# uthree/tinyvc

Hardware: AMD Instinct MI355X
Metric: audio-samples/sec (16 kHz) end-to-end VC (higher is better)
Workload: dtype f32 (fp32 in / out / accumulate; channel contractions as two-term fp16 splits on v_mfma_f32_32x32x16_f16: 22-bit significands, three part-products per fp32 product)

## Files before the change

tinyvc_amd/csrc/conv3s.h:

```cpp
#pragma once
#include <type_traits>
#include "conv_epi.h"
#include "small_kernels.h"
#include "split_fp16.h"
#include "tvc_common.h"

namespace tvc {

constexpr int S_WPE = 3;
constexpr int S_WPE_G = 4;
constexpr int S_WPE_F = 3;
constexpr int TVC_S_KG = 2;
constexpr int S_BPC = 1;
constexpr int S_FB = 2;
constexpr int S_FB_G = 1;
constexpr int S_FB_F = 1;
constexpr int S_FB_FW = 2;
constexpr int S_PF = 2;


template <class E, class = void>
struct wants_res_conv : std::false_type {};
template <class E>
struct wants_res_conv<E, std::void_t<decltype(E::kResConv)>> : std::bool_constant<E::kResConv> {};

template <int MTB_, int WM_, int NWV_, int WN_ = 1, int KG_ = 1, int MAXD_ = 27>
struct SplitTile {
    static constexpr int MTB = MTB_, WM = WM_, NWV = NWV_, WN = WN_;
    static constexpr int KG = KG_;
    static constexpr int MW = MTB / WM, NW = MW * NWV, NTHR = NW * 64;
    static_assert(MTB % WM == 0, "wave rows must tile the workgroup");
    static constexpr int BM = MTB * 32, BN = NWV * WN * 32;
    static constexpr int MAXD = MAXD_, XROW = BN + 2 * MAXD;
    static constexpr int XG_U4 = kParts * 2 * XROW;
    static constexpr int X_U4 = KG * XG_U4;
    static constexpr int X_PER = (KG * 2 * XROW + NTHR - 1) / NTHR;
    static constexpr int a_u4(int taps) { return taps * KG * MTB * kPU4; }
    static constexpr int stage_u4(int taps) { return a_u4(taps) + X_U4; }
    static constexpr int KS_MAX = 2 * 768;
    static constexpr int OS = BN + 4;
    static constexpr int lds_bytes(int taps) {
        const int stage = stage_u4(taps) * 16, out = BM * OS * 4;
        return (stage > out ? stage : out) + 2 * 6 * BM * 4 + KS_MAX * 4 + 64;
    }
    static constexpr int bias_off(int taps) {
        const int stage = stage_u4(taps) * 16, out = BM * OS * 4;
        return (stage > out ? stage : out) / 4;
    }
};

struct ConvSArgs {
    const uint4* A6;
    const float* wsc;
    int MT;
    const float* x;
    long xstride;
    int Cin, len, dil, tiles_per_utt, ntiles;
    int lin = 0;
    float lscale = 0.f;
    int cmax = 0;
    int flatT = 0;
    const float* kscale = nullptr;
    const uint4* sc6 = nullptr;
    const float* fsc = nullptr;
    const float* cond = nullptr;
    int Ccond = 0;
    const float* amax_x = nullptr;
    const float* amax_c = nullptr;
    float* amax_y = nullptr;
    RagDev rag;
};


template <class TL>
struct SlabRegs {
    static constexpr int A_MAX = (3 * TL::KG * TL::MTB * kParts + TL::NW - 1) / TL::NW;
    u32x4 ar[A_MAX];
    float xr[TL::X_PER][8];
    float xr2[TL::X_PER][8];
};
template <class TL>
struct SlabMap {
    unsigned xo[TL::X_PER];
    int xdst[TL::X_PER];
    int xg8[TL::X_PER];
    int xk[TL::X_PER];
    unsigned xo1[TL::X_PER];
    float w0[TL::X_PER], w1[TL::X_PER];
    float xs[TL::X_PER];
};
template <class TL, bool LERP = false>
__device__ __forceinline__ void make_map(SlabMap<TL>& m, int len, int dil, int t0, int fT = 0, unsigned fstride = 0, int kcin = 0, int lin = 0,
                                         float lscale = 0.f, float xs = 1.f, const float* amax = nullptr, int rs_ = 0, const int* __restrict__ c2b = nullptr, int cmult = 1) {
    const int rs = rs_ ? rs_ : len;
    const int xw = TL::BN + 2 * dil;
    int tid0 = threadIdx.x;
    asm volatile("" : "+v"(tid0));
    __builtin_assume(tid0 >= 0 && tid0 < TL::NTHR);
#pragma unroll
    for (int i = 0; i < TL::X_PER; ++i) {
        int idx = tid0 + i * TL::NTHR;
        int gk = idx / xw, c = idx - gk * xw;
        int p = t0 - dil + c;
        p = p < 0 ? 0 : (p > len - 1 ? len - 1 : p);
        const bool live = gk < 2 * TL::KG;
        gk = live ? gk : 2 * TL::KG - 1;
        const int ks = gk >> 1, g = gk & 1;
        m.xdst[i] = live ? ks * TL::XG_U4 + g * TL::XROW + c : -1;
        m.xg8[i] = ks * 16 + 8 * g;
        m.xs[i] = xs;
        if (fT > 0) {
            const int b = p / fT, t = p - b * fT;
            m.xo[i] = (unsigned)b * fstride + (unsigned)(m.xg8[i] * fT + t);
            m.xk[i] = (b - t0 / fT) * kcin;
            m.xs[i] = bfp_load(amax, b).s;
        } else if (LERP) {
            const Lerp lc = lerp_coord(p, lscale, lin);
            m.xo[i] = (unsigned)(m.xg8[i] * lin + lc.i0);
            m.xo1[i] = (unsigned)(m.xg8[i] * lin + lc.i1);
            m.w0[i] = lc.w0;
            m.w1[i] = lc.w1;
            m.xk[i] = 0;
        } else {
            m.xo[i] = (unsigned)(m.xg8[i] * rs + p);
            m.xk[i] = 0;
            if (c2b) m.xs[i] = bfp_load(amax, c2b[p / cmult]).s;
        }
    }
}
template <class TL, int TAPS, bool LERP = false, bool CLAMP = false>
__device__ __forceinline__ void slab_load(SlabRegs<TL>& r, const SlabMap<TL>& m, const uint4* __restrict__ A6, int MT, int mt0,
                                          const float* __restrict__ xb, int Cin, int len, int s, int fT = 0, int cmax = 0, int lin = 0, int rs_ = 0, int tid_ = -1) {
    constexpr int MTB = TL::MTB, NW = TL::NW, X_PER = TL::X_PER, STEPS = TAPS * TL::KG;
    const int cs = LERP ? lin : (fT > 0 ? fT : (rs_ ? rs_ : len));
    constexpr int PIECES = STEPS * MTB * kParts, A_PER = (PIECES + NW - 1) / NW;
    static_assert(A_PER <= SlabRegs<TL>::A_MAX, "weight pieces must fit the staging registers");
    const int tid = tid_ >= 0 ? tid_ : (int)threadIdx.x;
    __builtin_assume(tid >= 0 && tid < TL::NTHR);
    const int lane = tid & 63, wave = __builtin_amdgcn_readfirstlane(tid >> 6);
    __builtin_assume(wave >= 0 && wave < NW);
    const int ci0 = s * 16 * TL::KG;
    {
        const uint4* a_src = A6 + (long)mt0 * kPU4;
#pragma unroll
        for (int i = 0; i < A_PER; ++i) {
            int q = wave + i * NW;
            q = q < PIECES ? q : PIECES - 1;
            const int tap = q / (MTB * kParts), rem = q - tap * (MTB * kParts);
            r.ar[i] = ldg_so4(a_src + (long)s * STEPS * MT * kPU4, 16u * (unsigned)(tap * MT * kPU4 + rem * 64 + lane));
        }
    }
    const float* xc = xb + (long)ci0 * cs;
    if (LERP) {
#pragma unroll
        for (int i = 0; i < X_PER; ++i)
#pragma unroll
            for (int j = 0; j < 8; ++j) {
                r.xr[i][j] = ldg_so(xc + (long)j * cs, 4u * m.xo[i]);
                r.xr2[i][j] = ldg_so(xc + (long)j * cs, 4u * m.xo1[i]);
            }
        return;
    }
    if constexpr (CLAMP) {
#pragma unroll
        for (int i = 0; i < X_PER; ++i)
#pragma unroll
            for (int j = 0; j < 8; ++j) {
                int cj = ci0 + m.xg8[i] + j;
                cj = cj < cmax ? cj : cmax;
                r.xr[i][j] = xb[m.xo[i] + (unsigned)((cj - m.xg8[i]) * cs)];
            }
        return;
    }
#pragma unroll
    for (int i = 0; i < X_PER; ++i)
#pragma unroll
        for (int j = 0; j < 8; ++j) r.xr[i][j] = ldg_so(xc + (long)j * cs, 4u * m.xo[i]);
}
template <class TL, int TAPS, bool LERP = false, bool CLAMP = false>
__device__ __forceinline__ void first_load(SlabRegs<TL>& r, const uint4* __restrict__ A6, int MT, int mt0, const float* __restrict__ xb,
                                           int Cin, int len, int dil, int t0, int fT = 0, unsigned fstride = 0, int cmax = 0, int lin = 0,
                                           float lscale = 0.f, int rs_ = 0) {
    SlabMap<TL> m;
    make_map<TL, LERP>(m, len, dil, t0, fT, fstride, 0, lin, lscale, 1.f, nullptr, rs_);
    int tid = threadIdx.x;
    asm volatile("" : "+v"(tid));
    slab_load<TL, TAPS, LERP, CLAMP>(r, m, A6, MT, mt0, xb, Cin, len, 0, fT, cmax, lin, rs_, tid);
}

struct NoMid { __device__ __forceinline__ void operator()() const {} };
template <class TL, int TAPS, int A_U4, bool LRELU, int FB, bool SCALED = false, bool LERP = false, bool CLAMP = false, bool TWO = false, class Next, class Mid = NoMid>
__device__ __forceinline__ void split_phase(f32x16 (&hi)[TL::WM][TL::WN], f32x16 (&lo)[TL::WM][TL::WN], SlabRegs<TL>& r, const uint4* __restrict__ A6, int MT, int mt0,
                                            const float* __restrict__ xb, int Cin, int len, int dil, int t0, uint4* As, uint4* Xs, Next next, float xs,
                                            const float* Ks = nullptr, int fT = 0, unsigned fstride = 0, int cmax = 0, int lin = 0, float lscale = 0.f,
                                            int mt0b = 0, Mid mid = Mid(), const float* amax = nullptr, int rs_ = 0, const int* __restrict__ c2b = nullptr, int cmult = 1) {
    constexpr int MTB = TL::MTB, WM = TL::WM, WN = TL::WN, NWV = TL::NWV, NW = TL::NW, XROW = TL::XROW, X_PER = TL::X_PER;
    int tid = threadIdx.x;
    asm volatile("" : "+v"(tid));
    __builtin_assume(tid >= 0 && tid < TL::NTHR);
    const int lane = tid & 63, wave = __builtin_amdgcn_readfirstlane(tid >> 6);
    __builtin_assume(wave >= 0 && wave < NW);
    const int l31 = lane & 31, lh = lane >> 5;
    const int wm = wave / NWV, wn = wave - wm * NWV;
    SlabMap<TL> m;
    make_map<TL, LERP>(m, len, dil, t0, fT, fstride, Cin, lin, lscale, xs, amax, rs_, c2b, cmult);
    constexpr int STEPS = TAPS * TL::KG;
    constexpr int PIECES = STEPS * MTB * kParts, A_PER = (PIECES + NW - 1) / NW;
    auto lstore = [&](int sl) __attribute__((always_inline)) {
        uint4* Asb = As;
        uint4* Xsb = Xs;
#pragma unroll
        for (int i = 0; i < A_PER; ++i) {
            const int q = wave + i * NW;
            if (q < PIECES) *reinterpret_cast<u32x4*>(Asb + q * 64 + lane) = r.ar[i];
        }
#pragma unroll
        for (int i = 0; i < X_PER; ++i)
            if (m.xdst[i] >= 0) {
                if (LERP) {
#pragma unroll
                    for (int j = 0; j < 8; ++j) r.xr[i][j] = fmaf(m.w0[i], r.xr[i][j], __fmul_rn(m.w1[i], r.xr2[i][j]));
                }
                if (LRELU) {
#pragma unroll
                    for (int j = 0; j < 8; ++j) r.xr[i][j] = fmaxf(r.xr[i][j], 0.1f * r.xr[i][j]);
                }
                if (SCALED) {
                    const float4 k0 = *reinterpret_cast<const float4*>(Ks + m.xk[i] + sl * 16 * TL::KG + m.xg8[i]);
                    const float4 k1 = *reinterpret_cast<const float4*>(Ks + m.xk[i] + sl * 16 * TL::KG + m.xg8[i] + 4);
                    r.xr[i][0] *= k0.x; r.xr[i][1] *= k0.y; r.xr[i][2] *= k0.z; r.xr[i][3] *= k0.w;
                    r.xr[i][4] *= k1.x; r.xr[i][5] *= k1.y; r.xr[i][6] *= k1.z; r.xr[i][7] *= k1.w;
                }
#pragma unroll
                for (int j = 0; j < 8; ++j) r.xr[i][j] *= m.xs[i];
                uint4 p1, p2;
                split8(r.xr[i], p1, p2);
                Xsb[m.xdst[i]] = p1;
                Xsb[2 * XROW + m.xdst[i]] = p2;
            }
    };

    const int nslab1 = Cin / (16 * TL::KG);
    const int nslab = TWO ? 2 * nslab1 : nslab1;
    const uint4* as0 = As + wm * WM * kPU4 + lane;
    const uint4* xs0 = Xs + lh * XROW + wn * WN * 32 + l31;
    for (int s = 0; s < nslab; ++s) {
        slab_barrier();
        if (TWO && s == nslab1) mid();
        lstore(TWO && s >= nslab1 ? s - nslab1 : s);
        if (s + 1 < nslab) {
            if (TWO) slab_load<TL, TAPS, LERP, CLAMP>(r, m, A6, MT, s + 1 >= nslab1 ? mt0b : mt0, xb, Cin, len, s + 1 >= nslab1 ? s + 1 - nslab1 : s + 1, fT, cmax, lin, rs_, tid);
            else slab_load<TL, TAPS, LERP, CLAMP>(r, m, A6, MT, mt0, xb, Cin, len, s + 1, fT, cmax, lin, rs_, tid);
        } else next();
        slab_barrier();
        const uint4* as = as0;
        const uint4* xs_ = xs0;
        f16x8 af[2][WM][kParts], bf[2][WN][kParts];
        auto frags = [&](int tap, int fb) __attribute__((always_inline)) {
#pragma unroll
            for (int j = 0; j < WN; ++j)
#pragma unroll
                for (int p = 0; p < kParts; ++p)
                    bf[fb][j][p] = __builtin_bit_cast(f16x8, xs_[(tap / TAPS) * TL::XG_U4 + 2 * p * XROW + j * 32 + (tap % TAPS) * dil]);
#pragma unroll
            for (int i = 0; i < WM; ++i)
#pragma unroll
                for (int p = 0; p < kParts; ++p) af[fb][i][p] = __builtin_bit_cast(f16x8, as[(tap * MTB * kParts + i * kParts + p) * 64]);
        };
        if (FB == 2) frags(0, 0);
#pragma unroll
        for (int tap = 0; tap < STEPS; ++tap) {
            const int fb = FB == 2 ? tap & 1 : 0;
            if (FB == 2) {
                if (tap + 1 < STEPS) frags(tap + 1, fb ^ 1);
                __builtin_amdgcn_sched_barrier(0);
            } else {
                frags(tap, 0);
            }
#pragma unroll
            for (int i = 0; i < WM; ++i)
#pragma unroll
                for (int j = 0; j < WN; ++j) lo[i][j] = TVC_MFMA16(af[fb][i][1], bf[fb][j][0], lo[i][j]);
#pragma unroll
            for (int i = 0; i < WM; ++i)
#pragma unroll
                for (int j = 0; j < WN; ++j) hi[i][j] = TVC_MFMA16(af[fb][i][0], bf[fb][j][0], hi[i][j]);
#pragma unroll
            for (int i = 0; i < WM; ++i)
#pragma unroll
                for (int j = 0; j < WN; ++j) lo[i][j] = TVC_MFMA16(af[fb][i][0], bf[fb][j][1], lo[i][j]);
            if (FB == 2) __builtin_amdgcn_sched_barrier(0);
        }
    }
}

template <class TL>
__device__ __forceinline__ void film_load(SlabRegs<TL>& r, const SlabMap<TL>& m, const uint4* __restrict__ F6, int MT, int mt0, int mtoff,
                                          const float* __restrict__ xb, int len, int s, int rs_ = 0) {
    const int rs = rs_ ? rs_ : len;
    constexpr int MTB = TL::MTB, NW = TL::NW, X_PER = TL::X_PER;
    constexpr int KG = TL::KG, GP = 2 * MTB * kParts, PIECES = KG * GP, A_PER = (PIECES + NW - 1) / NW;
    static_assert(A_PER <= SlabRegs<TL>::A_MAX, "FiLM weight pieces must fit the staging registers");
    const int lane = threadIdx.x & 63, wave = threadIdx.x >> 6;
#pragma unroll
    for (int i = 0; i < A_PER; ++i) {
        int q = wave + i * NW;
        q = q < PIECES ? q : PIECES - 1;
        const int kg = q / GP, q2 = q - kg * GP;
        const int grp = q2 / (MTB * kParts), rem = q2 - grp * (MTB * kParts);
        r.ar[i] = ldg_so4(F6 + ((long)s * KG * MT + mt0) * kPU4, 16u * (unsigned)((kg * MT + grp * mtoff) * kPU4 + rem * 64 + lane));
    }
    const float* xc = xb + (long)s * 16 * KG * rs;
#pragma unroll
    for (int i = 0; i < X_PER; ++i)
#pragma unroll
        for (int j = 0; j < 8; ++j) r.xr[i][j] = ldg_so(xc + (long)j * rs, 4u * m.xo[i]);
}
template <class TL>
__device__ __forceinline__ void film_first_load(SlabRegs<TL>& r, const uint4* __restrict__ F6, int MT, int mt0, int mtoff,
                                                const float* __restrict__ xb, int len, int t0, int rs_ = 0) {
    SlabMap<TL> m;
    make_map<TL>(m, len, 0, t0, 0, 0u, 0, 0, 0.f, 1.f, nullptr, rs_);
    film_load<TL>(r, m, F6, MT, mt0, mtoff, xb, len, 0, rs_);
}
template <class TL, class Next>
__device__ __forceinline__ void film_phase(f32x16 (&asc)[TL::WM][TL::WN], f32x16 (&lsc)[TL::WM][TL::WN], f32x16 (&ash)[TL::WM][TL::WN], f32x16 (&lsh)[TL::WM][TL::WN],
                                           SlabRegs<TL>& r, const uint4* __restrict__ F6,
                                           int MT, int mt0, int mtoff, const float* __restrict__ xb, int Cin, int len, int t0, uint4* As, uint4* Xs,
                                           Next next, float xs, int rs_ = 0) {
    constexpr int MTB = TL::MTB, WM = TL::WM, WN = TL::WN, NWV = TL::NWV, NW = TL::NW, XROW = TL::XROW, X_PER = TL::X_PER;
    constexpr int KG = TL::KG, GP = 2 * MTB * kParts, PIECES = KG * GP, A_PER = (PIECES + NW - 1) / NW;
    const int tid = threadIdx.x, lane = tid & 63, wave = tid >> 6;
    const int l31 = lane & 31, lh = lane >> 5;
    const int wm = wave / NWV, wn = wave - wm * NWV;
    SlabMap<TL> m;
    make_map<TL>(m, len, 0, t0, 0, 0u, 0, 0, 0.f, 1.f, nullptr, rs_);
    const int nslab = Cin / (16 * KG);
    const uint4* as0 = As + wm * WM * kPU4 + lane;
    const uint4* xs0 = Xs + lh * XROW + wn * WN * 32 + l31;
    auto lstore = [&]() __attribute__((always_inline)) {
#pragma unroll
        for (int i = 0; i < A_PER; ++i) {
            const int q = wave + i * NW;
            if (q < PIECES) *reinterpret_cast<u32x4*>(As + q * 64 + lane) = r.ar[i];
        }
#pragma unroll
        for (int i = 0; i < X_PER; ++i)
            if (m.xdst[i] >= 0) {
#pragma unroll
                for (int j = 0; j < 8; ++j) r.xr[i][j] *= xs;
                uint4 p1, p2;
                split8(r.xr[i], p1, p2);
                Xs[m.xdst[i]] = p1;
                Xs[2 * XROW + m.xdst[i]] = p2;
            }
    };
    for (int s = 0; s < nslab; ++s) {
        slab_barrier();
        lstore();
        if (s + 1 < nslab) film_load<TL>(r, m, F6, MT, mt0, mtoff, xb, len, s + 1, rs_);
        else next();
        slab_barrier();
        const uint4* as = as0;
        const uint4* xq = xs0;
#pragma unroll
        for (int kg = 0; kg < KG; ++kg) {
            f16x8 fc[WM][kParts], fh[WM][kParts], bf[WN][kParts];
#pragma unroll
            for (int j = 0; j < WN; ++j)
#pragma unroll
                for (int p = 0; p < kParts; ++p) bf[j][p] = __builtin_bit_cast(f16x8, xq[kg * TL::XG_U4 + 2 * p * XROW + j * 32]);
#pragma unroll
            for (int i = 0; i < WM; ++i)
#pragma unroll
                for (int p = 0; p < kParts; ++p) {
                    fc[i][p] = __builtin_bit_cast(f16x8, as[(kg * GP + i * kParts + p) * 64]);
                    fh[i][p] = __builtin_bit_cast(f16x8, as[(kg * GP + MTB * kParts + i * kParts + p) * 64]);
                }
#pragma unroll
            for (int i = 0; i < WM; ++i)
#pragma unroll
                for (int j = 0; j < WN; ++j) {
                    lsc[i][j] = TVC_MFMA16(fc[i][1], bf[j][0], lsc[i][j]);
                    lsh[i][j] = TVC_MFMA16(fh[i][1], bf[j][0], lsh[i][j]);
                    asc[i][j] = TVC_MFMA16(fc[i][0], bf[j][0], asc[i][j]);
                    ash[i][j] = TVC_MFMA16(fh[i][0], bf[j][0], ash[i][j]);
                    lsc[i][j] = TVC_MFMA16(fc[i][0], bf[j][1], lsc[i][j]);
                    lsh[i][j] = TVC_MFMA16(fh[i][0], bf[j][1], lsh[i][j]);
                }
        }
    }
}

template <class TL, bool RES>
__device__ __forceinline__ void tile_store(float* Ot, const f32x16 (&v)[TL::WM][TL::WN], float* __restrict__ y, const float* __restrict__ res,
                                           int b, int M, int len, int mt0, int t0, float& mx, float* __restrict__ y2 = nullptr, int f2 = 0, int rlin = 0, float rscale = 0.f,
                                           int rs_ = 0, int coloff = 0) {
    const int rs = rs_ ? rs_ : len;
    const int rvalid = (rs_ && rlin > 0) ? __builtin_amdgcn_readfirstlane(len / (rs / rlin)) : rlin;
    const int rcol = (rs_ && rlin > 0) ? __builtin_amdgcn_readfirstlane(coloff / (rs / rlin)) : 0;
    constexpr int WM = TL::WM, WN = TL::WN, BM = TL::BM, BN = TL::BN, OS = TL::OS, NTHR = TL::NTHR;
    int tid = threadIdx.x;
    asm volatile("" : "+v"(tid));
    const int lane = tid & 63, wave = tid >> 6;
    const int l31 = lane & 31, lh = lane >> 5;
    const int wm = wave / TL::NWV, wn = wave - wm * TL::NWV;
    auto park = [&]() __attribute__((always_inline)) {
        slab_barrier();
#pragma unroll
        for (int i = 0; i < WM; ++i)
#pragma unroll
            for (int j = 0; j < WN; ++j)
#pragma unroll
                for (int r = 0; r < 16; ++r)
                    Ot[((wm * WM + i) * 32 + 4 * lh + (r & 3) + 8 * (r >> 2)) * OS + (wn * WN + j) * 32 + l31] = v[i][j][r];
        slab_barrier();
    };
    __builtin_amdgcn_sched_barrier(0);
    float* yb = y + ((long)b * M + mt0 * 32) * rs + coloff + t0;
    const float* rb = RES ? (rlin > 0 ? res + ((long)b * M + mt0 * 32) * rlin + rcol : res + ((long)b * M + mt0 * 32) * rs + coloff + t0) : nullptr;
    const int rows = M - mt0 * 32 < BM ? M - mt0 * 32 : BM;
    const bool vec = ((rs | coloff) & 3) == 0;
    const int len2 = f2 > 0 ? rs / f2 : 0;
    float* y2b = y2 ? y2 + ((long)b * M + mt0 * 32) * len2 + (f2 > 0 ? coloff / f2 : 0) : nullptr;
    if constexpr (RES) {
        if (rlin > 0) {
            constexpr int G = BN / 4, RS = NTHR / G;
            static_assert(NTHR % G == 0, "column groups must tile the workgroup");
            const int c = (tid % G) * 4;
            unsigned o0[4], o1[4];
            float lam[4];
#pragma unroll
            for (int u = 0; u < 4; ++u) {
                const int t = t0 + c + u < len ? t0 + c + u : len - 1;
                const Lerp lc = lerp_coord(t, rscale, rvalid);
                o0[u] = 4u * (unsigned)lc.i0;
                o1[u] = 4u * (unsigned)lc.i1;
                lam[u] = lc.w1;
            }
            const bool full = vec && t0 + c + 3 < len;
            constexpr int NR = (BM + RS - 1) / RS, PF = S_PF;
            float x0[PF][4], x1[PF][4];
            const bool live = t0 + c < len;
            auto request = [&](int k0) __attribute__((always_inline)) {
#pragma unroll
                for (int k = 0; k < PF; ++k) {
                    int row = tid / G + (k0 + k) * RS;
                    row = row < rows ? row : rows - 1;
                    const unsigned ro = 4u * (unsigned)(row * rlin);
#pragma unroll
                    for (int u = 0; u < 4; ++u) {
                        x0[k][u] = ldg_so(rb, ro + o0[u]);
                        x1[k][u] = ldg_so(rb, ro + o1[u]);
                    }
                }
            };
            __builtin_amdgcn_sched_barrier(0);
            request(0);
            park();
            if (live) {
#pragma unroll
            for (int k0 = 0; k0 < NR; k0 += PF) {
                float w[PF][4];
#pragma unroll
                for (int k = 0; k < PF; ++k)
#pragma unroll
                    for (int u = 0; u < 4; ++u) w[k][u] = fmaf(1.f - lam[u], x0[k][u], __fmul_rn(lam[u], x1[k][u]));
                if (k0 + PF < NR) request(k0 + PF);
#pragma unroll
                for (int k = 0; k < PF; ++k) {
                    const int row = tid / G + (k0 + k) * RS;
                    if (row >= rows) break;
                    const float4 o = *reinterpret_cast<const float4*>(Ot + row * OS + c);
                    const float e[4] = {o.x + w[k][0], o.y + w[k][1], o.z + w[k][2], o.w + w[k][3]};
                    const int off = row * rs + c;
                    if (full) {
                        *reinterpret_cast<float4*>(yb + off) = make_float4(e[0], e[1], e[2], e[3]);
                        mx = fmaxf(fmaxf(mx, fmaxf(fabsf(e[0]), fabsf(e[1]))), fmaxf(fabsf(e[2]), fabsf(e[3])));
                    } else {
#pragma unroll
                        for (int u = 0; u < 4; ++u)
                            if (t0 + c + u < len) {
                                yb[off + u] = e[u];
                                mx = fmaxf(mx, fabsf(e[u]));
                            }
                    }
                }
            }
            }
            return;
        }
        if (vec && t0 + BN <= len) {
            constexpr int G = BN / 4, RS = NTHR / G, NR = (BM + RS - 1) / RS;
            const int c = (tid % G) * 4;
            float4 q[NR];
            __builtin_amdgcn_sched_barrier(0);
#pragma unroll
            for (int k = 0; k < NR; ++k) {
                int row = tid / G + k * RS;
                row = row < rows ? row : rows - 1;
                q[k] = *reinterpret_cast<const float4*>(rb + row * rs + c);
            }
            park();
#pragma unroll
            for (int k = 0; k < NR; ++k) {
                const int row = tid / G + k * RS;
                if (row >= rows) break;
                float4 w = *reinterpret_cast<const float4*>(Ot + row * OS + c);
                w.x += q[k].x; w.y += q[k].y; w.z += q[k].z; w.w += q[k].w;
                *reinterpret_cast<float4*>(yb + row * rs + c) = w;
                mx = fmaxf(fmaxf(mx, fmaxf(fabsf(w.x), fabsf(w.y))), fmaxf(fabsf(w.z), fabsf(w.w)));
                if (y2b) {
                    const float e[4] = {w.x, w.y, w.z, w.w};
                    if (f2 == 4) {
                        y2b[row * len2 + ((t0 + c) >> 2)] = fmaf(0.5f, e[1], __fmul_rn(0.5f, e[2]));
                    } else {
#pragma unroll
                        for (int u = 0; u < 4; ++u) {
                            const int t = t0 + c + u, qq = t / f2;
                            if (t - qq * f2 == (f2 >> 1)) y2b[row * len2 + qq] = e[u];
                        }
                    }
                }
            }
            return;
        }
    }
    park();
#pragma unroll 2
    for (int idx = tid; idx < BM * (BN / 4); idx += NTHR) {
        const int row = idx / (BN / 4), c = (idx - row * (BN / 4)) * 4;
        if (row >= rows || t0 + c >= len) continue;
        const float4 o = *reinterpret_cast<const float4*>(Ot + row * OS + c);
        const int off = row * rs + c;
        if (RES && rlin > 0) {
            const float e[4] = {o.x, o.y, o.z, o.w};
            float w[4];
#pragma unroll
            for (int u = 0; u < 4; ++u) {
                const int t = t0 + c + u < len ? t0 + c + u : len - 1;
                const Lerp lc = lerp_coord(t, rscale, rvalid);
                w[u] = e[u] + lerp_eval(lc, rb[row * rlin + lc.i0], rb[row * rlin + lc.i1]);
            }
            if (vec && t0 + c + 3 < len) {
                *reinterpret_cast<float4*>(yb + off) = make_float4(w[0], w[1], w[2], w[3]);
                mx = fmaxf(fmaxf(mx, fmaxf(fabsf(w[0]), fabsf(w[1]))), fmaxf(fabsf(w[2]), fabsf(w[3])));
            } else {
#pragma unroll
                for (int u = 0; u < 4; ++u)
                    if (t0 + c + u < len) {
                        yb[off + u] = w[u];
                        mx = fmaxf(mx, fabsf(w[u]));
                    }
            }
        } else if (vec && t0 + c + 3 < len) {
            float4 w = o;
            if (RES) {
                const float4 q = *reinterpret_cast<const float4*>(rb + off);
                w.x += q.x; w.y += q.y; w.z += q.z; w.w += q.w;
            }
            *reinterpret_cast<float4*>(yb + off) = w;
            mx = fmaxf(fmaxf(mx, fmaxf(fabsf(w.x), fabsf(w.y))), fmaxf(fabsf(w.z), fabsf(w.w)));
            if (y2b) {
                const float e[4] = {w.x, w.y, w.z, w.w};
                if (f2 == 4) {
                    y2b[row * len2 + ((t0 + c) >> 2)] = fmaf(0.5f, e[1], __fmul_rn(0.5f, e[2]));
                } else {
#pragma unroll
                    for (int u = 0; u < 4; ++u) {
                        const int t = t0 + c + u, q = t / f2;
                        if (t - q * f2 == (f2 >> 1)) y2b[row * len2 + q] = e[u];
                    }
                }
            }
        } else {
            const float e[4] = {o.x, o.y, o.z, o.w};
#pragma unroll
            for (int u = 0; u < 4; ++u)
                if (t0 + c + u < len) {
                    const float ov = RES ? e[u] + rb[off + u] : e[u];
                    yb[off + u] = ov;
                    mx = fmaxf(mx, fabsf(ov));
                    if (y2b && f2 != 4) {
                        const int t = t0 + c + u, q = t / f2;
                        if (t - q * f2 == (f2 >> 1)) y2b[row * len2 + q] = ov;
                    }
                }
        }
    }
}

template <class TL, int TAPS, bool LRELU, class Epi, bool FILM, bool SCALED = false, bool LERP = false, bool CLAMP = false, bool RAG = false>
__global__ __launch_bounds__(TL::NTHR) __attribute__((amdgpu_waves_per_eu(FILM ? S_WPE_F : (Epi::kIgemm ? (TL::NW <= 8 ? S_WPE_G : 5) : S_WPE)))) void conv3s_kernel(ConvSArgs a, Epi ep) {
    static_assert(!RAG || (!LERP && !SCALED && !(FILM && TL::WN > 1)), "ragged batches: plain / residual-conv / narrow FiLM / GEMM launches only");
    constexpr bool RAGT = RAG && !Epi::kIgemm;
    constexpr bool RAGG = RAG && Epi::kIgemm;
    constexpr int MTB = TL::MTB, WM = TL::WM, WN = TL::WN, A_U4 = TL::a_u4(TAPS);
    extern __shared__ __attribute__((aligned(16))) uint4 smem_s[];
    uint4* As = smem_s;
    uint4* Xs = smem_s + A_U4;

    const int lane = threadIdx.x & 63, wave = threadIdx.x >> 6;
    const int lh = lane >> 5;
    const int wm = wave / TL::NWV;
    const int mblocks = a.MT / MTB;
    int len = a.len;
    const int rs = RAGT ? a.len : 0;
    int coloff = 0;
    const int ntiles = a.ntiles;

    auto coords = [&](int v, int& mt0, int& b, int& t0) __attribute__((always_inline)) {
        const int nt_id = v / mblocks, mb = v - nt_id * mblocks;
        mt0 = mb * MTB;
        if constexpr (RAGT) {
            b = __builtin_amdgcn_readfirstlane(rag_find(a.rag.ts, a.rag.B, __builtin_amdgcn_readfirstlane(nt_id), b));
            t0 = __builtin_amdgcn_readfirstlane((nt_id - a.rag.ts[b]) * TL::BN);
        } else {
            b = nt_id / a.tiles_per_utt;
            t0 = (nt_id - b * a.tiles_per_utt) * TL::BN;
        }
    };
    auto ulen = [&](int b_) __attribute__((always_inline)) { return __builtin_amdgcn_readfirstlane(a.rag.tb[b_] * a.rag.mult); };
    auto uoff = [&](int b_) __attribute__((always_inline)) { return __builtin_amdgcn_readfirstlane(a.rag.pre[b_] * a.rag.mult); };
    int tile, vtiles;
    tile_range(ntiles, tile, vtiles);
    SlabRegs<TL> regs;
    int mt0 = 0, b = 0, t0 = 0;
    if (tile >= vtiles) return;
    coords(tile, mt0, b, t0);
    float mx_run = 0.f;
    int mx_b = b;
    float* const red = reinterpret_cast<float*>(smem_s) + TL::bias_off(TAPS) + 12 * TL::BM + TL::KS_MAX;
    const int fT = (TAPS == 1 && !FILM && !LERP && !RAGT) ? a.flatT : 0;
    const unsigned fstride = (unsigned)a.xstride;
    constexpr bool FILM_FIRST = FILM && TL::WN == 1;
    auto load_first = [&](int mt0_, int b_, int t0_) __attribute__((always_inline)) {
        if constexpr (FILM_FIRST && RAGT) film_first_load<TL>(regs, a.sc6, 2 * a.MT, mt0_, a.MT, a.cond + uoff(b_), ulen(b_), t0_, rs);
        else if constexpr (FILM_FIRST) film_first_load<TL>(regs, a.sc6, 2 * a.MT, mt0_, a.MT, a.cond + (long)b_ * a.Ccond * len, len, t0_);
        else if constexpr (RAGT) first_load<TL, TAPS, LERP, CLAMP>(regs, a.A6, a.MT, mt0_, a.x + uoff(b_), a.Cin, ulen(b_), a.dil, t0_, 0, 0u, a.cmax, 0, 0.f, rs);
        else first_load<TL, TAPS, LERP, CLAMP>(regs, a.A6, a.MT, mt0_, fT ? a.x : a.x + (long)b_ * a.xstride, a.Cin, len, a.dil, t0_, fT, fstride, a.cmax, a.lin, a.lscale);
    };
    if constexpr (RAGT) {
        len = ulen(b);
        coloff = uoff(b);
    }
    load_first(mt0, b, t0);
    for (int tile_no = 0; tile < vtiles; ++tile_no) {
        const int nxt = tile + 1;
        if constexpr (!Epi::kIgemm) {
            if (a.amax_y && b != mx_b) {
                amax_flush_wg(a.amax_y + mx_b, mx_run, red);
                mx_run = 0.f;
                mx_b = b;
            }
        }
        auto load_next_tile = [&]() __attribute__((always_inline)) {
            if (nxt < vtiles) {
                int mt0n, bn = b, t0n;
                coords(nxt, mt0n, bn, t0n);
                load_first(mt0n, bn, t0n);
            }
        };
        const float* xb = RAGT ? a.x + coloff : (fT ? a.x : a.x + (long)b * a.xstride);
        float* Bs = reinterpret_cast<float*>(smem_s) + TL::bias_off(TAPS) + (tile_no & 1) * 6 * TL::BM;
        if constexpr (!Epi::kIgemm) {
            for (int i = threadIdx.x; i < TL::BM; i += TL::NTHR) {
                int m = mt0 * 32 + i;
                m = m < ep.M ? m : ep.M - 1;
                Bs[i] = ep.bias[m];
                Bs[3 * TL::BM + i] = a.wsc[mt0 + (i >> 5)];
                if constexpr (FILM) {
                    Bs[TL::BM + i] = ep.bsc[m];
                    Bs[2 * TL::BM + i] = ep.bsh[m];
                    Bs[4 * TL::BM + i] = a.fsc[mt0 + (i >> 5)];
                    Bs[5 * TL::BM + i] = a.fsc[a.MT + mt0 + (i >> 5)];
                }
            }
        }
        float* Ks = reinterpret_cast<float*>(smem_s) + TL::bias_off(TAPS) + 12 * TL::BM;
        if constexpr (SCALED) {
            const int b0 = fT ? t0 / fT : b;
            const int nrow = fT ? ((t0 + TL::BN - 1 < len ? t0 + TL::BN - 1 : len - 1) / fT - b0 + 1) * a.Cin : a.Cin;
            for (int i = threadIdx.x; i < nrow; i += TL::NTHR) Ks[i] = a.kscale[(long)b0 * a.Cin + i];
        }
        const int rl = wm * WM * 32 + 4 * lh;
        const Bfp sx = (fT || RAGG) ? Bfp{1.f, 1.f} : bfp_load_u(a.amax_x, b);
        f32x16 hi[WM][WN], lo[WM][WN];
        auto clear = [&](f32x16 (&u)[WM][WN]) __attribute__((always_inline)) {
#pragma unroll
            for (int i = 0; i < WM; ++i)
#pragma unroll
                for (int j = 0; j < WN; ++j)
#pragma unroll
                    for (int r = 0; r < 16; ++r) u[i][j][r] = 0.f;
        };
        clear(hi);
        clear(lo);
        auto fold = [&](f32x16 (&h)[WM][WN], const f32x16 (&l)[WM][WN], const float* wtab, float inv) __attribute__((always_inline)) {
#pragma unroll
            for (int i = 0; i < WM; ++i)
#pragma unroll
                for (int q = 0; q < 4; ++q) {
                    const float4 w4 = *reinterpret_cast<const float4*>(wtab + rl + i * 32 + 8 * q);
                    const float wv[4] = {w4.x, w4.y, w4.z, w4.w};
#pragma unroll
                    for (int u = 0; u < 4; ++u) {
                        const float c = wv[u] * inv, cl = c * kLoInv;
#pragma unroll
                        for (int j = 0; j < WN; ++j) h[i][j][4 * q + u] = comb(h[i][j][4 * q + u], l[i][j][4 * q + u], c, cl);
                    }
#pragma unroll
                    for (int j = 0; j < WN; ++j) asm volatile("" : "+v"(h[i][j]) : : "memory");
                }
        };

        if constexpr (FILM && TL::WN > 1) {
            const float* cb = a.cond + (long)b * a.Ccond * len;
            const int mtoff = a.MT;
            const Bfp sc = bfp_load_u(a.amax_c, b);
            split_phase<TL, TAPS, A_U4, LRELU, S_FB_FW, false, LERP, false>(
                hi, lo, regs, a.A6, a.MT, mt0, xb, a.Cin, len, a.dil, t0, As, Xs,
                [&]() __attribute__((always_inline)) { first_load<TL, 1>(regs, a.sc6, 2 * a.MT, mt0, cb, a.Ccond, len, 0, t0); }, sx.s, nullptr, 0, 0u, 0, a.lin, a.lscale);
            fold(hi, lo, Bs + 3 * TL::BM, sx.inv);
            f32x16 fh[WM][WN];
            clear(fh);
            clear(lo);
            split_phase<TL, 1, A_U4, false, S_FB_F, false, false, false, true>(
                fh, lo, regs, a.sc6, 2 * a.MT, mt0, cb, a.Ccond, len, 0, t0, As, Xs, load_next_tile, sc.s, nullptr, 0, 0u, 0, 0, 0.f, mtoff + mt0,
                [&]() __attribute__((always_inline)) {
                    fold(fh, lo, Bs + 4 * TL::BM, sc.inv);
#pragma unroll
                    for (int i = 0; i < WM; ++i)
#pragma unroll
                        for (int r = 0; r < 16; ++r) {
                            const int row = rl + i * 32 + (r & 3) + 8 * (r >> 2);
                            const float bm = Bs[row], bs = Bs[TL::BM + row];
#pragma unroll
                            for (int j = 0; j < WN; ++j) {
                                hi[i][j][r] = __fmul_rn(hi[i][j][r] + bm, fh[i][j][r] + bs);
                                fh[i][j][r] = 0.f;
                                lo[i][j][r] = 0.f;
                            }
                        }
                });
            fold(fh, lo, Bs + 5 * TL::BM, sc.inv);
#pragma unroll
            for (int i = 0; i < WM; ++i)
#pragma unroll
                for (int r = 0; r < 16; ++r) {
                    const float bh = Bs[2 * TL::BM + rl + i * 32 + (r & 3) + 8 * (r >> 2)];
#pragma unroll
                    for (int j = 0; j < WN; ++j) hi[i][j][r] = __fadd_rn(hi[i][j][r], fh[i][j][r] + bh);
                }
            tile_store<TL, true>(reinterpret_cast<float*>(smem_s), hi, ep.y, ep.res, b, ep.M, len, mt0, t0, mx_run, nullptr, 0, ep.res_lin, ep.res_scale);
        } else if constexpr (FILM) {
            const float* cb = RAGT ? a.cond + coloff : a.cond + (long)b * a.Ccond * len;
            const int mtoff = a.MT;
            const Bfp sc = bfp_load_u(a.amax_c, b);
            f32x16 asc[WM][WN], lsc[WM][WN], ash[WM][WN], lsh[WM][WN];
            clear(asc);
            clear(lsc);
            clear(ash);
            clear(lsh);
            film_phase<TL>(asc, lsc, ash, lsh, regs, a.sc6, 2 * a.MT, mt0, mtoff, cb, a.Ccond, len, t0, As, Xs,
                           [&]() __attribute__((always_inline)) { first_load<TL, TAPS, LERP, false>(regs, a.A6, a.MT, mt0, xb, a.Cin, len, a.dil, t0, 0, 0u, 0, a.lin, a.lscale, rs); }, sc.s, rs);
            fold(asc, lsc, Bs + 4 * TL::BM, sc.inv);
            fold(ash, lsh, Bs + 5 * TL::BM, sc.inv);
            split_phase<TL, TAPS, A_U4, LRELU, S_FB_F, false, LERP, false>(hi, lo, regs, a.A6, a.MT, mt0, xb, a.Cin, len, a.dil, t0, As, Xs, load_next_tile, sx.s, nullptr, 0, 0u, 0,
                                                                            a.lin, a.lscale, 0, NoMid(), nullptr, rs);
            fold(hi, lo, Bs + 3 * TL::BM, sx.inv);
            {
#pragma unroll
                for (int i = 0; i < WM; ++i)
#pragma unroll
                    for (int q = 0; q < 4; ++q) {
                        const int row = rl + i * 32 + 8 * q;
                        const float4 m4 = *reinterpret_cast<const float4*>(Bs + row), s4 = *reinterpret_cast<const float4*>(Bs + TL::BM + row),
                                     h4 = *reinterpret_cast<const float4*>(Bs + 2 * TL::BM + row);
                        const float bm[4] = {m4.x, m4.y, m4.z, m4.w}, bs[4] = {s4.x, s4.y, s4.z, s4.w}, bh[4] = {h4.x, h4.y, h4.z, h4.w};
#pragma unroll
                        for (int u = 0; u < 4; ++u)
#pragma unroll
                            for (int j = 0; j < WN; ++j)
                                hi[i][j][4 * q + u] = __fadd_rn(__fmul_rn(hi[i][j][4 * q + u] + bm[u], asc[i][j][4 * q + u] + bs[u]), ash[i][j][4 * q + u] + bh[u]);
#pragma unroll
                        for (int j = 0; j < WN; ++j) asm volatile("" : "+v"(hi[i][j]) : : "memory");
                    }
                tile_store<TL, true>(reinterpret_cast<float*>(smem_s), hi, ep.y, ep.res, RAGT ? 0 : b, ep.M, len, mt0, t0, mx_run, nullptr, 0, ep.res_lin, ep.res_scale, rs, coloff);
            }
        } else {
            float inv = sx.inv;
            if constexpr (wants_res_conv<Epi>::value) {
                const float* cb = RAGT ? a.cond + coloff : a.cond + (long)b * a.Ccond * len;
                const Bfp s2 = bfp_min(sx, bfp_load_u(a.amax_c, b));
                inv = s2.inv;
                split_phase<TL, TAPS, A_U4, LRELU, S_FB, false, false, false>(
                    hi, lo, regs, a.A6, a.MT, mt0, xb, a.Cin, len, a.dil, t0, As, Xs,
                    [&]() __attribute__((always_inline)) { first_load<TL, 1>(regs, a.sc6, a.MT, mt0, cb, a.Ccond, len, 0, t0, 0, 0u, 0, 0, 0.f, rs); }, s2.s, nullptr, 0, 0u, 0, 0, 0.f,
                    0, NoMid(), nullptr, rs);
                split_phase<TL, 1, A_U4, false, S_FB, false, false, false>(hi, lo, regs, a.sc6, a.MT, mt0, cb, a.Ccond, len, 0, t0, As, Xs, load_next_tile, s2.s, nullptr, 0, 0u, 0, 0,
                                                                           0.f, 0, NoMid(), nullptr, rs);
            } else
            split_phase<TL, TAPS, A_U4, LRELU, Epi::kIgemm ? S_FB_G : S_FB, SCALED, LERP, CLAMP>(hi, lo, regs, a.A6, a.MT, mt0, xb, a.Cin, len, a.dil, t0, As, Xs,
                                                                                                  load_next_tile, sx.s, Ks, fT, fstride, a.cmax, a.lin, a.lscale, 0, NoMid(),
                                                                                                  a.amax_x, rs, RAGG ? a.rag.col2b : nullptr, RAGG ? a.rag.mult : 1);
            if constexpr (Epi::kIgemm) {
                const int l31 = lane & 31, wn = wave - wm * TL::NWV;
                const int mtw = __builtin_amdgcn_readfirstlane(mt0 + wm * WM);
#pragma unroll
                for (int i = 0; i < WM; ++i) {
                    const float cw = a.wsc[mtw + i];
#pragma unroll
                    for (int j = 0; j < WN; ++j) {
                        const int col = t0 + (wn * WN + j) * 32 + l31;
                        const int n = b * len + col;
                        if (col < len) {
                            const float c = cw * (RAGG ? bfp_load(a.amax_x, a.rag.col2b[col / a.rag.mult]).inv : (fT ? bfp_load(a.amax_x, col / fT).inv : inv)), cl = c * kLoInv;
#pragma unroll
                            for (int q = 0; q < 4; ++q) {
                                const float v[4] = {comb(hi[i][j][4 * q], lo[i][j][4 * q], c, cl), comb(hi[i][j][4 * q + 1], lo[i][j][4 * q + 1], c, cl),
                                                    comb(hi[i][j][4 * q + 2], lo[i][j][4 * q + 2], c, cl), comb(hi[i][j][4 * q + 3], lo[i][j][4 * q + 3], c, cl)};
                                ep.store(n, (mt0 + wm * WM + i) * 32 + 8 * q + 4 * lh, v);
                            }
                        }
                    }
                }
                tile = nxt;
                if (tile < vtiles) coords(tile, mt0, b, t0);
                continue;
            }
            if constexpr (!Epi::kIgemm) {
                fold(hi, lo, Bs + 3 * TL::BM, inv);
#pragma unroll
                for (int i = 0; i < WM; ++i)
#pragma unroll
                    for (int r = 0; r < 16; ++r) {
                        const float bm = Bs[rl + i * 32 + (r & 3) + 8 * (r >> 2)];
#pragma unroll
                        for (int j = 0; j < WN; ++j) hi[i][j][r] += bm;
                    }
                tile_store<TL, Epi::kRes>(reinterpret_cast<float*>(smem_s), hi, ep.y, ep.res, RAGT ? 0 : b, ep.M, len, mt0, t0, mx_run, ep.y2, ep.f2, 0, 0.f, rs, coloff);
            }
        }
        tile = nxt;
        if (tile < vtiles) {
            coords(tile, mt0, b, t0);
            if constexpr (RAGT) {
                len = ulen(b);
                coloff = uoff(b);
            }
        }
    }
    if constexpr (!Epi::kIgemm) {
        if (a.amax_y) amax_flush_wg(a.amax_y + mx_b, mx_run, red);
    }
}

template <class TL, int TAPS, bool LRELU, class Epi, bool FILM, bool SCALED = false, bool LERP = false, bool CLAMP = false>
inline int conv3s_launch_t(tvc_ctx* ctx, hipStream_t s, const PackedW& w, const float* x, int B, int Cin, int len, int dil, const Epi& ep,
                           const PackedW* wsc, const PackedW* wsh, const float* cond, int Ccond, long xstride = 0, int bpc = S_BPC,
                           const float* kscale = nullptr, bool flat = false, int cmax = 0, int lin = 0, float lscale = 0.f, const BfpSlots& bfp = {}) {
    if (Cin % (16 * TL::KG) != 0 || (FILM && Ccond % (16 * TL::KG) != 0)) return fail(ctx, TVC_ERR_ARG, "conv3s: channel counts must be multiples of the slab depth");
    if (Cin / 16 > w.S6) return fail(ctx, TVC_ERR_ARG, "conv3s: weight image has fewer K16 steps than the launch walks");
    constexpr int lds = TL::lds_bytes(TAPS);
    TVC_CHECK((lds_optin<conv3s_kernel<TL, TAPS, LRELU, Epi, FILM, SCALED, LERP, CLAMP>>(ctx, lds, "conv3s")));
    ConvSArgs a;
    a.A6 = reinterpret_cast<const uint4*>(w.A6);
    a.wsc = w.wscale;
    a.MT = w.MT6;
    a.amax_x = bfp.x;
    a.amax_c = bfp.c;
    a.amax_y = bfp.y;
    if (Epi::kIgemm && bfp.y) return fail(ctx, TVC_ERR_ARG, "conv3s: GEMM launches finish their elements in the epilogue functor and cannot track the output's |max|");
    if (SCALED && (!kscale || Cin > 768)) return fail(ctx, TVC_ERR_ARG, "conv3s: scaled launch needs factors for <= 768 channels");
    a.kscale = kscale;
    a.cmax = cmax;
    if (CLAMP != (cmax > 0)) return fail(ctx, TVC_ERR_ARG, "conv3s: row clamp is a compile-time property of the launch");
    a.lin = lin;
    a.lscale = lscale;
    if (LERP && (lin <= 0 || flat)) return fail(ctx, TVC_ERR_ARG, "conv3s: interpolated input needs its low-rate length");
    a.x = x;
    a.xstride = xstride ? xstride : (long)Cin * (LERP ? lin : len);
    a.Cin = Cin;
    a.len = len;
    a.dil = dil;
    if (flat) {
        if (FILM || TAPS != 1 || dil != 0) return fail(ctx, TVC_ERR_ARG, "conv3s: flat tiles are for plain GEMMs");
        a.flatT = len;
        a.len = B * len;
        B = 1;
    }
    a.tiles_per_utt = (a.len + TL::BN - 1) / TL::BN;
    if (wants_res_conv<Epi>::value) {
        if (FILM || !wsc || wsc->MT6 != w.MT6 || wsc->taps != 1 || Ccond % 16 != 0 || Ccond / 16 > wsc->S6 || !cond)
            return fail(ctx, TVC_ERR_ARG, "conv3s: the residual 1x1 phase needs a matching 1x1 image and its input");
        if (wsc->wjoint != w.A6) return fail(ctx, TVC_ERR_STATE, "conv3s: the residual 1x1's image must be packed with the conv's per-m-tile scales");
        a.sc6 = reinterpret_cast<const uint4*>(wsc->A6);
        a.cond = cond;
        a.Ccond = Ccond;
    }
    if (FILM) {
        if (wsc->MT6 != 2 * w.MT6) return fail(ctx, TVC_ERR_ARG, "conv3s: FiLM image must stack scale and shift rows");
        a.sc6 = reinterpret_cast<const uint4*>(wsc->A6);
        a.fsc = wsc->wscale;
        a.cond = cond;
        a.Ccond = Ccond;
    }
    a.ntiles = (a.MT / TL::MTB) * a.tiles_per_utt * B;
    const int slots = ctx->ncu * bpc;
    if (ctx->rag) {
        if constexpr (!LERP && !SCALED && !(FILM && TL::WN > 1)) {
            if (flat) return fail(ctx, TVC_ERR_STATE, "conv3s: a ragged batch runs as one long utterance");
            int ncol = a.tiles_per_utt;
            TVC_CHECK(rag_tiles(ctx, s, B, a.len, Epi::kIgemm ? 0 : TL::BN, &a.rag, &ncol, "conv3s"));
            TVC_CHECK((lds_optin<conv3s_kernel<TL, TAPS, LRELU, Epi, FILM, SCALED, LERP, CLAMP, true>>(ctx, lds, "conv3s")));
            a.ntiles = (a.MT / TL::MTB) * ncol;
            dim3 g((unsigned)(a.ntiles < slots ? a.ntiles : slots));
            hipLaunchKernelGGL((conv3s_kernel<TL, TAPS, LRELU, Epi, FILM, SCALED, LERP, CLAMP, true>), g, dim3(TL::NTHR), lds, s, a, ep);
            return 0;
        } else {
            return fail(ctx, TVC_ERR_STATE, "conv3s: this launch has no ragged-batch variant");
        }
    }
    dim3 g((unsigned)(a.ntiles < slots ? a.ntiles : slots));
    hipLaunchKernelGGL((conv3s_kernel<TL, TAPS, LRELU, Epi, FILM, SCALED, LERP, CLAMP>), g, dim3(TL::NTHR), lds, s, a, ep);
    return 0;
}

template <bool LRELU, class Epi, bool FILM = false, bool LERP = false>
inline int conv3s_launch(tvc_ctx* ctx, hipStream_t s, const PackedW& w, const float* x, int B, int Cin, int len, int dil, const Epi& ep,
                         const BfpSlots& bfp, const PackedW* wsc = nullptr, const PackedW* wsh = nullptr, const float* cond = nullptr, int Ccond = 0, int lin = 0,
                         float lscale = 0.f) {
    if (w.MT6 % 3 != 0) return fail(ctx, TVC_ERR_ARG, "conv3s: k3 convs need a multiple of 96 output rows");
    if constexpr (FILM) {
        const long mb = w.MT6 / 3;
        const long tiles_w = mb * ((len + 255) / 256) * B;
        const long slots = 256 * S_BPC;
        const bool wide = tiles_w >= slots && !ctx->rag;
        if (wide)
            return conv3s_launch_t<SplitTile<3, 1, 4, 2>, 3, LRELU, Epi, FILM, false, LERP>(ctx, s, w, x, B, Cin, len, dil, ep, wsc, wsh, cond, Ccond, 0, S_BPC, nullptr, false,
                                                                                           0, lin, lscale, bfp);
        if (Cin % 32 == 0 && Ccond % 32 == 0)
            return conv3s_launch_t<SplitTile<3, 1, 4, 1, 2>, 3, LRELU, Epi, FILM, false, LERP>(ctx, s, w, x, B, Cin, len, dil, ep, wsc, wsh, cond, Ccond, 0, S_BPC, nullptr, false, 0,
                                                                                              lin, lscale, bfp);
        return conv3s_launch_t<SplitTile<3, 1, 4, 1>, 3, LRELU, Epi, FILM, false, LERP>(ctx, s, w, x, B, Cin, len, dil, ep, wsc, wsh, cond, Ccond, 0, S_BPC, nullptr, false, 0,
                                                                                       lin, lscale, bfp);
    } else
        return conv3s_launch_t<SplitTile<3, 1, 4, 2>, 3, LRELU, Epi, FILM, false, LERP>(ctx, s, w, x, B, Cin, len, dil, ep, wsc, wsh, cond, Ccond, 0, S_BPC, nullptr, false, 0,
                                                                                       lin, lscale, bfp);
}

template <int MTB, int NWV, int BPC, int KG, class Epi, bool SCALED, bool CLAMP>
inline int gemm_s_launch_k(tvc_ctx* ctx, hipStream_t s, const PackedW& w, const float* x, int B, int Cin, int len, long xstride, const Epi& ep,
                           const float* kscale, int cmax, const float* amax_x) {
    using TL = SplitTile<MTB, (MTB >= 4 ? 2 : 1), NWV, 1, KG, 0>;
    const long xs = xstride ? xstride : (long)Cin * len;
    const bool flat = B > 1 && xs * B < (1L << 30) && (!SCALED || len >= TL::BN);
    return conv3s_launch_t<TL, 1, false, Epi, false, SCALED, false, CLAMP>(ctx, s, w, x, B, Cin, len, 0, ep, nullptr, nullptr, nullptr, 0, xstride, BPC, kscale, flat,
                                                                           cmax, 0, 0.f, BfpSlots{amax_x, nullptr, nullptr});
}
template <int MTB, int NWV, int BPC, class Epi, bool SCALED = false>
inline int gemm_s_launch(tvc_ctx* ctx, hipStream_t s, const PackedW& w, const float* x, int B, int Cin, int len, long xstride, const Epi& ep,
                         const float* amax_x, const float* kscale = nullptr) {
    if (w.MT6 % MTB != 0) return fail(ctx, TVC_ERR_ARG, "gemm_s: row tiles do not divide");
    if (TVC_S_KG >= 2 && Cin % 32 == 0) return gemm_s_launch_k<MTB, NWV, BPC, 2, Epi, SCALED, false>(ctx, s, w, x, B, Cin, len, xstride, ep, kscale, 0, amax_x);
    return gemm_s_launch_k<MTB, NWV, BPC, 1, Epi, SCALED, false>(ctx, s, w, x, B, Cin, len, xstride, ep, kscale, 0, amax_x);
}
template <int MTB, int NWV, int BPC, class Epi>
inline int gemm_s_launch_ragged(tvc_ctx* ctx, hipStream_t s, const PackedW& w, const float* x, int B, int krows, int len, long xstride, const Epi& ep,
                                const float* amax_x) {
    if (w.MT6 % MTB != 0) return fail(ctx, TVC_ERR_ARG, "gemm_s: row tiles do not divide");
    return gemm_s_launch_k<MTB, NWV, BPC, 2, Epi, false, true>(ctx, s, w, x, B, (krows + 31) / 32 * 32, len, xstride, ep, nullptr, krows - 1, amax_x);
}


}
```

tinyvc_amd/csrc/conv_epi.h:

```cpp
#pragma once
#include "gemm_epi.h"

namespace tvc {

template <bool RES, int F2 = 0>
struct C3EpiBias {
    static constexpr bool kRes = RES;
    static constexpr bool kIgemm = false;
    float* y;
    const float* bias;
    const float* res;
    int M, len;
    float* y2 = nullptr;
    int f2 = 0;
    __device__ __forceinline__ void store(int b, int t, int m, const float v[4]) const {
        const int q = F2 > 0 ? t / F2 : 0;
        const bool pick = F2 > 0 && y2 != nullptr && t - q * F2 == (F2 >> 1);
#pragma unroll
        for (int r = 0; r < 4; ++r)
            if (m + r < M) {
                long i = ((long)b * M + m + r) * len + t;
                float o = v[r] + bias[m + r];
                if (RES) o += res[i];
                y[i] = o;
                if (pick) y2[((long)b * M + m + r) * (len / F2) + q] = o;
            }
    }
};

struct C3EpiBiasResConv : C3EpiBias<false, 0> {
    static constexpr bool kResConv = true;
};

struct C3EpiFilmFused {
    static constexpr bool kIgemm = false;
    float* y;
    const float* bias;
    const float* bsc;
    const float* bsh;
    const float* res;
    int M, len;
    int res_lin = 0;
    float res_scale = 0.f;
    __device__ __forceinline__ void store(int b, int t, int m, const float h[4], const float sc[4], const float sh[4]) const {
#pragma unroll
        for (int r = 0; r < 4; ++r)
            if (m + r < M) {
                long i = ((long)b * M + m + r) * len + t;
                float hv = h[r] + bias[m + r];
                y[i] = __fadd_rn(__fadd_rn(__fmul_rn(hv, sc[r] + bsc[m + r]), sh[r] + bsh[m + r]), res[i]);
            }
    }
};

}
```

tinyvc_amd/csrc/conv_s2.h:

```cpp
#pragma once
#include "small_kernels.h"
#include "split_fp16.h"

namespace tvc {

struct ConvS2Args {
    const uint4* A6;
    const float* wsc;
    int MT;
    const float* x;
    int Cin, len, dil, lin;
    float lscale;
    float* y;
    const float* bias;
    int M, tiles_per_utt, ntiles, mblocks;
    const float* amax_x;
    float* amax_y;
    uint4* ypre;
    float pre_w, pre_b;
    RagDev rag;
};
__device__ __forceinline__ float presplit_bound(float pre_w, float pre_b, const float* amax, int b) { return fmaf(pre_w, sload_f32(amax + b), pre_b); }
__device__ __forceinline__ Bfp norm_from_amax(float amax) {
    const unsigned u = __builtin_bit_cast(unsigned, amax);
    Bfp r{1.f, 1.f};
    if (u != 0u && u < 0x7f800000u) {
        int k = 14 - ((int)(u >> 23) - 127);
        k = k > 120 ? 120 : (k < -120 ? -120 : k);
        r.s = __builtin_bit_cast(float, (unsigned)(127 + k) << 23);
        r.inv = __builtin_bit_cast(float, (unsigned)(127 - k) << 23);
    }
    return r;
}

struct CS2 {
    static constexpr int MTB = 3, NWV = 4, WN = 2, NW = MTB * NWV, NTHR = NW * 64, BN = NWV * WN * 32, MAXD = 27, XROW = BN + 2 * MAXD;
    static constexpr int A_PIECES = 3 * MTB * kParts, A_PER = (A_PIECES + NW - 1) / NW;
    static constexpr int A_U4 = A_PIECES * 64, X_U4 = kParts * 2 * XROW, BUF_U4 = A_U4 + X_U4;
    static constexpr int TAB = 2 * 128 * 3;
    static constexpr int lds_bytes = 2 * BUF_U4 * 16 + TAB * 4 + 64;
};

template <bool LERP, bool PRE = false, bool RAG = false>
__global__ __launch_bounds__(CS2::NTHR) __attribute__((amdgpu_waves_per_eu(3))) void conv_s2_kernel(ConvS2Args a) {
    using TL = CS2;
    constexpr int MTB = TL::MTB, NWV = TL::NWV, WN = TL::WN, NW = TL::NW, BN = TL::BN, XROW = TL::XROW, A_PER = TL::A_PER;
    extern __shared__ __attribute__((aligned(16))) uint4 smem_c2[];
    float* Tb = reinterpret_cast<float*>(smem_c2 + 2 * TL::BUF_U4);
    float* red = Tb + TL::TAB;
    const int tid = threadIdx.x, lane = tid & 63;
    const int wave = __builtin_amdgcn_readfirstlane(tid >> 6);
    const int l31 = lane & 31, lh = lane >> 5;
    const int wm = wave / NWV, wn = wave - wm * NWV;
    const int nslab = a.Cin / 16, rs = a.len, dil = a.dil;
    const int cs_ = LERP ? a.lin : rs;
    const int xf = LERP ? rs / a.lin : 1;
    const int xw = BN + 2 * dil, nitems = 2 * xw;

    for (int i = tid; i < a.M; i += TL::NTHR) {
        Tb[i] = a.bias[i];
        Tb[384 + i] = a.wsc[i >> 5];
    }

    int tfirst, tlast;
    tile_range(a.ntiles, tfirst, tlast);
    if (tfirst >= tlast) return;
    auto coords = [&](int v, int& mt0, int& b, int& t0, int& len, int& off) __attribute__((always_inline)) {
        const int nt = v / a.mblocks, mb = v - nt * a.mblocks;
        mt0 = mb * MTB;
        const RagTile rt = rag_tile<RAG>(a.rag, nt, a.tiles_per_utt, rs, b);
        b = rt.b;
        t0 = rt.tin * BN;
        len = rt.len;
        off = rt.off;
    };

    u32x4 ar[A_PER];
    float xr[8], xr2[LERP ? 8 : 1];
    const int item = tid < nitems ? tid : tid - nitems;
    const int ig = item / xw, ic = item - ig * xw;
    const int xdst = ig * XROW + ic;
    unsigned xo = 0, xo1 = 0;
    float lw0 = 0.f, lw1 = 0.f, xsc = 1.f;
    float rw0 = 0.f, rw1 = 0.f, rxs = 1.f;
    int lv = tfirst, ls = 0, lmt0, lb = 0, lt0, llen, loff;
    coords(lv, lmt0, lb, lt0, llen, loff);
    auto tile_offsets = [&]() __attribute__((always_inline)) {
        int p = lt0 - dil + ic;
        p = p < 0 ? 0 : (p > llen - 1 ? llen - 1 : p);
        const int cbase = 8 * ig * cs_ + (RAG ? (LERP ? loff / xf : loff) : 0);
        if (LERP) {
            const Lerp lc = lerp_coord(p, a.lscale, RAG ? llen / xf : a.lin);
            xo = (unsigned)(cbase + lc.i0);
            xo1 = (unsigned)(cbase + lc.i1);
            lw0 = lc.w0;
            lw1 = lc.w1;
        } else {
            xo = (unsigned)(cbase + p);
        }
        xsc = bfp_load_u(a.amax_x, lb).s;
    };
    tile_offsets();
    auto issue_load = [&]() __attribute__((always_inline)) {
        const uint4* abase = a.A6 + ((long)ls * 3 * a.MT + lmt0) * kPU4;
#pragma unroll
        for (int i = 0; i < A_PER; ++i) {
            int q = wave + i * NW;
            q = q < TL::A_PIECES ? q : TL::A_PIECES - 1;
            const int tap = q / (MTB * kParts), rem = q - tap * (MTB * kParts);
            ar[i] = ldg_so4(abase, 16u * (unsigned)(tap * a.MT * kPU4 + rem * 64 + lane));
        }
        const float* xc = a.x + ((RAG ? 0L : (long)lb * a.Cin) + (long)ls * 16) * cs_;
#pragma unroll
        for (int j = 0; j < 8; ++j) {
            xr[j] = ldg_so(xc + (long)j * cs_, 4u * xo);
            if (LERP) xr2[j] = ldg_so(xc + (long)j * cs_, 4u * xo1);
        }
        rw0 = lw0;
        rw1 = lw1;
        rxs = xsc;
    };
    auto advance_load = [&]() __attribute__((always_inline)) {
        if (++ls == nslab) {
            if (lv + 1 < tlast) {
                ++lv;
                ls = 0;
                coords(lv, lmt0, lb, lt0, llen, loff);
                tile_offsets();
            } else {
                ls = nslab - 1;
            }
        }
    };
    auto lstore = [&](int buf) __attribute__((always_inline)) {
        uint4* Ab = smem_c2 + buf * TL::BUF_U4;
        uint4* Xb = Ab + TL::A_U4;
#pragma unroll
        for (int i = 0; i < A_PER; ++i) {
            int q = wave + i * NW;
            q = q < TL::A_PIECES ? q : TL::A_PIECES - 1;
            *reinterpret_cast<u32x4*>(Ab + q * 64 + lane) = ar[i];
        }
        float v[8];
#pragma unroll
        for (int j = 0; j < 8; ++j) {
            const float t = LERP ? fmaf(rw0, xr[j], __fmul_rn(rw1, xr2[j])) : xr[j];
            v[j] = fmaxf(t, 0.1f * t) * rxs;
        }
        uint4 p1, p2;
        split8(v, p1, p2);
        Xb[xdst] = p1;
        Xb[2 * XROW + xdst] = p2;
    };

    f32x16 hi[WN], lo[WN];
#pragma unroll
    for (int j = 0; j < WN; ++j)
#pragma unroll
        for (int r = 0; r < 16; ++r) hi[j][r] = lo[j][r] = 0.f;
    auto multiply = [&](int buf, int tap) __attribute__((always_inline)) {
        const uint4* Ab = smem_c2 + buf * TL::BUF_U4 + ((tap * MTB + wm) * kParts) * 64 + lane;
        const uint4* Xb = smem_c2 + buf * TL::BUF_U4 + TL::A_U4 + lh * XROW + wn * WN * 32 + l31 + tap * dil;
        f16x8 af[kParts], bf[WN][kParts];
#pragma unroll
        for (int j = 0; j < WN; ++j)
#pragma unroll
            for (int p = 0; p < kParts; ++p) bf[j][p] = __builtin_bit_cast(f16x8, Xb[p * 2 * XROW + j * 32]);
#pragma unroll
        for (int p = 0; p < kParts; ++p) af[p] = __builtin_bit_cast(f16x8, Ab[p * 64]);
#pragma unroll
        for (int j = 0; j < WN; ++j) lo[j] = TVC_MFMA16(af[1], bf[j][0], lo[j]);
#pragma unroll
        for (int j = 0; j < WN; ++j) hi[j] = TVC_MFMA16(af[0], bf[j][0], hi[j]);
#pragma unroll
        for (int j = 0; j < WN; ++j) lo[j] = TVC_MFMA16(af[0], bf[j][1], lo[j]);
    };

    int cv = tfirst, cs = 0, cmt0, cb = 0, ct0, len, coff;
    coords(cv, cmt0, cb, ct0, len, coff);
    float mx_run = 0.f;
    int flush_b = -1;

    issue_load();
    advance_load();
    lstore(0);
    issue_load();
    advance_load();
    slab_barrier();
    int buf = 0;
    while (true) {
        multiply(buf, 0);
        lstore(buf ^ 1);
        issue_load();
        multiply(buf, 1);
        multiply(buf, 2);
        advance_load();
        if (++cs == nslab) {
            const Bfp sx = bfp_load_u(a.amax_x, cb);
            const int row0 = (cmt0 + wm) * 32;
            float* yb = RAG ? a.y + (long)row0 * rs + coff : a.y + ((long)cb * a.M + row0) * rs;
            const float ps = PRE ? norm_from_amax(presplit_bound(a.pre_w, a.pre_b, a.amax_x, cb)).s : 1.f;
#pragma unroll
            for (int j = 0; j < WN; ++j) {
                const int t = ct0 + (wn * WN + j) * 32 + l31;
                const bool live = t < len;
                const unsigned off = 4u * (unsigned)(4 * lh * rs + (live ? t : len - 1));
#pragma unroll
                for (int g = 0; g < 4; ++g) {
                    if (row0 + 8 * g < a.M) {
                        const float4 bv = *reinterpret_cast<const float4*>(Tb + row0 + 8 * g + 4 * lh);
                        const float c = Tb[384 + row0] * sx.inv, cl = c * kLoInv;
                        const float e[4] = {comb(hi[j][4 * g], lo[j][4 * g], c, cl) + bv.x, comb(hi[j][4 * g + 1], lo[j][4 * g + 1], c, cl) + bv.y,
                                            comb(hi[j][4 * g + 2], lo[j][4 * g + 2], c, cl) + bv.z, comb(hi[j][4 * g + 3], lo[j][4 * g + 3], c, cl) + bv.w};
                        if (PRE) {
                            float v[4];
#pragma unroll
                            for (int q = 0; q < 4; ++q) v[q] = fmaxf(e[q], 0.1f * e[q]) * ps;
                            unsigned p1[2], p2[2];
                            split2<false>(v[0], v[1], p1[0], p2[0]);
                            split2<false>(v[2], v[3], p1[1], p2[1]);
                            const auto qx = __builtin_amdgcn_permlane32_swap(p1[0], p2[0], false, false);
                            const auto qy = __builtin_amdgcn_permlane32_swap(p1[1], p2[1], false, false);
                            if (live) a.ypre[(((RAG ? 0L : (long)cb * 2) + lh) * (a.M >> 3) + ((row0 >> 3) + g)) * rs + (RAG ? coff : 0) + t] = make_uint4(qx[0], qy[0], qx[1], qy[1]);
                        } else if (live) {
#pragma unroll
                            for (int q = 0; q < 4; ++q) {
                                stg_so(yb + (long)(8 * g + q) * rs, off, e[q]);
                                mx_run = fmaxf(mx_run, fabsf(e[q]));
                            }
                        }
                    }
                }
#pragma unroll
                for (int r = 0; r < 16; ++r) hi[j][r] = lo[j][r] = 0.f;
            }
            cs = 0;
            const int done_b = cb;
            ++cv;
            const bool last = cv >= tlast;
            if (!last) coords(cv, cmt0, cb, ct0, len, coff);
            if (a.amax_y && (last || cb != done_b)) {
                const float m = wave_max(mx_run);
                if (lane == 0) red[wave] = m;
                mx_run = 0.f;
                flush_b = done_b;
            }
            if (last) break;
        }
        slab_barrier();
        if (flush_b >= 0) {
            if (tid == 0) {
                float m = 0.f;
                for (int w = 0; w < NW; ++w) m = fmaxf(m, red[w]);
                if (m > 0.f) atomicMax(reinterpret_cast<unsigned*>(a.amax_y + flush_b), __builtin_bit_cast(unsigned, m));
            }
            flush_b = -1;
        }
        buf ^= 1;
    }
    if (flush_b >= 0) {
        slab_barrier();
        if (tid == 0) {
            float m = 0.f;
            for (int w = 0; w < NW; ++w) m = fmaxf(m, red[w]);
            if (m > 0.f) atomicMax(reinterpret_cast<unsigned*>(a.amax_y + flush_b), __builtin_bit_cast(unsigned, m));
        }
    }
}

template <bool LERP, bool PRE = false>
inline bool conv_s2_try(int* rc, tvc_ctx* ctx, hipStream_t s, const PackedW& w, const float* x, int B, int Cin, int len, int dil, float* y, const BfpSlots& bfp,
                        int lin = 0, float lscale = 0.f, float pre_w = 0.f, float pre_b = 0.f) {
    if (PRE && (!bfp.x || w.M % 8 != 0)) return false;
    if (w.taps != 3 || w.MT6 % 3 != 0 || w.M > 384 || Cin % 16 != 0 || Cin / 16 > w.S6 || dil < 1 || dil > CS2::MAXD || bfp.c) return false;
    if ((long)B * w.M * len >= (1L << 31) / 4 * 4 && (long)w.M * len * 4 >= (1L << 32)) return false;
    if ((long)Cin * (LERP ? lin : len) * 4 >= (1L << 32) || (long)w.M * len * 4 >= (1L << 32)) return false;
    if (LERP != (lin > 0)) return false;
    if ((*rc = lds_optin<conv_s2_kernel<LERP, PRE>, conv_s2_kernel<LERP, PRE, true>>(ctx, CS2::lds_bytes, "conv_s2"))) return true;
    ConvS2Args a;
    a.A6 = reinterpret_cast<const uint4*>(w.A6);
    a.wsc = w.wscale;
    a.MT = w.MT6;
    a.x = x;
    a.Cin = Cin;
    a.len = len;
    a.dil = dil;
    a.lin = lin;
    a.lscale = lscale;
    a.y = y;
    a.bias = w.bias;
    a.M = w.M;
    a.mblocks = w.MT6 / CS2::MTB;
    a.tiles_per_utt = (len + CS2::BN - 1) / CS2::BN;
    a.amax_x = bfp.x;
    a.amax_y = PRE ? nullptr : bfp.y;
    a.ypre = reinterpret_cast<uint4*>(y);
    a.pre_w = pre_w;
    a.pre_b = pre_b;
    int ncol = a.tiles_per_utt * B;
    if ((*rc = rag_tiles(ctx, s, B, len, CS2::BN, &a.rag, &ncol, "conv_s2"))) return true;
    a.ntiles = ncol * a.mblocks;
    const int grid = a.ntiles < ctx->ncu ? a.ntiles : ctx->ncu;
    if (ctx->rag) hipLaunchKernelGGL((conv_s2_kernel<LERP, PRE, true>), dim3(grid), dim3(CS2::NTHR), CS2::lds_bytes, s, a);
    else hipLaunchKernelGGL((conv_s2_kernel<LERP, PRE>), dim3(grid), dim3(CS2::NTHR), CS2::lds_bytes, s, a);
    *rc = launch_check(ctx, "conv_s2");
    return true;
}

}
```

tinyvc_amd/csrc/decoder.hip:

```cpp
#include "conv3s.h"
#include "conv_s2.h"
#include "film_s2.h"
#include "gemm_s2.h"
#include "small_kernels.h"
#include "tvc_common.h"

namespace tvc {


__device__ __forceinline__ float div24k(float x) {
    const float r = 1.0f / 24000.0f;
    const float q0 = __fmul_rn(x, r);
    return fmaf(fmaf(-q0, 24000.0f, x), r, q0);
}

__device__ __forceinline__ double wave_incl_scan(double v, int lane) {
#pragma unroll
    for (int o = 1; o < 64; o <<= 1) {
        double u = __shfl_up(v, o);
        if (lane >= o) v += u;
    }
    return v;
}

static __global__ __launch_bounds__(256) void harm_frame_sum_kernel(const float* __restrict__ f0, double* __restrict__ csum,
                                                                    int T, float scale, RagDev rg) {
    const int b = blockIdx.y, lane = threadIdx.x & 63;
    const int t = 4 * blockIdx.x + (threadIdx.x >> 6);
    const int rs = T;
    long fbase = (long)b * T, cbase = (long)b * kHarm * T;
    if (rg.tb) {
        T = rg.tb[b];
        fbase = cbase = rg.pre[b];
        scale = __fdiv_rn((float)T, (float)(T * kHop));
    }
    if (t >= T) return;
    const float* f = f0 + fbase;
    double acc[kHarm];
#pragma unroll
    for (int m = 0; m < kHarm; ++m) acc[m] = 0.0;
    if (lane < kHop / 8) {
#pragma unroll
        for (int k = 0; k < 8; ++k) {
            Lerp c = lerp_coord(t * kHop + 8 * lane + k, scale, T);
            float fs = lerp_eval(c, f[c.i0], f[c.i1]);
#pragma unroll
            for (int m = 0; m < kHarm; ++m) acc[m] += (double)div24k(__fmul_rn(fs, (float)(m + 1)));
        }
    }
#pragma unroll
    for (int m = 0; m < kHarm; ++m) {
        double v = acc[m];
#pragma unroll
        for (int o = 32; o > 0; o >>= 1) v += __shfl_xor(v, o);
        if (lane == m) csum[cbase + (long)m * rs + t] = v;
    }
}

static __global__ __launch_bounds__(64) void harm_frame_scan_kernel(double* __restrict__ csum, int T, RagDev rg) {
    double* p = csum + ((long)blockIdx.y * kHarm + blockIdx.x) * T;
    if (rg.tb) {
        p = csum + (long)blockIdx.x * T + rg.pre[blockIdx.y];
        T = rg.tb[blockIdx.y];
    }
    const int lane = threadIdx.x;
    double carry = 0.0;
    for (int base = 0; base < T; base += 64) {
        int i = base + lane;
        double v = i < T ? p[i] : 0.0;
        double inc = wave_incl_scan(v, lane);
        if (i < T) p[i] = carry + (inc - v);
        carry += __shfl(inc, 63);
    }
}

static __global__ __launch_bounds__(256) void harm_synth_kernel(const float* __restrict__ f0, const float* __restrict__ amps,
                                                                const double* __restrict__ coff, float* __restrict__ source,
                                                                int T, float scale_size, float scale_amp, RagDev rg) {
    const int b = blockIdx.y, lane = threadIdx.x & 63;
    const int t = 4 * blockIdx.x + (threadIdx.x >> 6);
    const int rs = T;
    const long Ls = (long)T * kHop;
    long fbase = (long)b * T, abase = (long)b * kHarm * T, sbase = (long)b * 16 * Ls;
    if (rg.tb) {
        T = rg.tb[b];
        fbase = abase = rg.pre[b];
        sbase = (long)rg.pre[b] * kHop;
        scale_size = __fdiv_rn((float)T, (float)(T * kHop));
    }
    if (t >= T) return;
    const bool act = lane < kHop / 8;
    const float* f = f0 + fbase;
    const int p0 = t * kHop + 8 * (act ? lane : 0);
    float fs[8], uv[8];
    Lerp ca[8];
#pragma unroll
    for (int e = 0; e < 8; ++e) {
        const Lerp c = lerp_coord(p0 + e, scale_size, T);
        const float a0 = f[c.i0], a1 = f[c.i1];
        fs[e] = lerp_eval(c, a0, a1);
        uv[e] = lerp_eval(c, a0 > 20.f ? 1.f : 0.f, a1 > 20.f ? 1.f : 0.f);
        ca[e] = lerp_coord(p0 + e, scale_amp, T);
    }
    for (int m = 0; m < kHarm; ++m) {
        double d[8], sum = 0.0;
#pragma unroll
        for (int e = 0; e < 8; ++e) {
            d[e] = act ? (double)div24k(__fmul_rn(fs[e], (float)(m + 1))) : 0.0;
            sum += d[e];
        }
        const double inc = wave_incl_scan(sum, lane);
        double run = coff[abase + (long)m * rs + t] + (inc - sum);
        if (act) {
            const float* am = amps + abase + (long)m * rs;
            float o[8];
#pragma unroll
            for (int e = 0; e < 8; ++e) {
                run += d[e];
                const float I = (float)run;
                const float frac = I - floorf(I);
                const float theta = __fmul_rn(6.2831854820251465f, frac);
                const float hsin = __fmul_rn(sincos_small(theta).x, uv[e]);
                const float amp = lerp_eval(ca[e], am[ca[e].i0], am[ca[e].i1]);
                o[e] = __fmul_rn(hsin, amp);
            }
            float4* dst = reinterpret_cast<float4*>(source + sbase + (long)m * Ls + p0);
            dst[0] = make_float4(o[0], o[1], o[2], o[3]);
            dst[1] = make_float4(o[4], o[5], o[6], o[7]);
        }
    }
}

static __global__ __launch_bounds__(256) void noise_ola_kernel(const float* __restrict__ frames, float* __restrict__ source, int B, int T, float* __restrict__ smax, RagDev rg) {
    __shared__ float red[4];
    const long Ls = (long)T * kHop;
    const long b = blockIdx.y;
    long fbase = b * T, sbase = (b * 16 + 15) * Ls;
    if (rg.tb) {
        T = rg.tb[b];
        fbase = rg.pre[b];
        sbase = 15 * Ls + (long)rg.pre[b] * kHop;
    }
    const long L = (long)T * kHop;
    float mx = 0.f;
    for (long i = blockIdx.x * (long)blockDim.x + threadIdx.x; i < L; i += (long)gridDim.x * blockDim.x) {
        int p = (int)i;
        int q = p + kNfft / 2;
        int f_hi = q / kHop;
        if (f_hi > T) f_hi = T;
        int f_lo = (q - (kNfft - 1) + kHop - 1) / kHop;
        if (q - (kNfft - 1) <= 0) f_lo = 0;
        float s = 0.f;
        for (int f = f_lo > 1 ? f_lo : 1; f <= f_hi; ++f)
            s = __fadd_rn(s, frames[(fbase + (f - 1)) * kNfft + (q - f * kHop)]);
        const float v = s / (float)(f_hi - f_lo + 1);
        source[sbase + p] = v;
        mx = fmaxf(mx, fabsf(v));
    }
    amax_flush_wg(smax + b, mx, red);
}

static int run_source_net(tvc_ctx* ctx, hipStream_t s, Ws& ws, const float* content, const float* f0,
                          const float* energy, float* amps, float* kern, int B, int T, const float* cmax, float* xmax_zeroed, hipEvent_t amps_ready = nullptr) {
    const int ncols = B * T;
    float* ef = ws.get<float>((size_t)B * T);
    float* x = ws.get<float>((size_t)B * kSrcCh * T);
    const int NB = ctx->rag ? ctx->rag->B : B;
    float* xmax = xmax_zeroed ? xmax_zeroed : ws.get<float>((size_t)NB);
    if (!ws.dry) {
        hipLaunchKernelGGL(window_max_kernel, dim3(grid_for((long)ncols * 64)), dim3(256), 0, s, energy, ef, (long)B, T, kHop);
        EpiSumCond ep{x, ctx->src_content_in.bias, ef, f0, ctx->src_e_w, ctx->src_e_b, ctx->src_f_w, ctx->src_f_b, kSrcCh, T, ncols};
        int rc = 0;
        if (!gemm_s2_try(&rc, ctx, s, ctx->src_content_in, content, B, kSslDim, T, 0, ep, cmax)) rc = gemm_s_launch<2, 4, 2>(ctx, s, ctx->src_content_in, content, B, kSslDim, T, 0, ep, cmax);
        TVC_CHECK(rc);
    }
    if (!ws.dry && !xmax_zeroed) TVC_HIP(ctx, hipMemsetAsync(xmax, 0, (size_t)NB * sizeof(float), s));
    for (int i = 0; i < 3; ++i) TVC_CHECK(run_convnext(ctx, s, ws, ctx->src_mid[i], x, B, T, i == 2 ? xmax : nullptr));
    if (ws.dry) return 0;
    EpiBias<ACT_ELU1, false> ea{amps, ctx->src_to_amps.bias, nullptr, kHarm, T, ncols, (long)kHarm * T, 0};
    TVC_CHECK((gemm_s_launch<1, 4, 2>(ctx, s, ctx->src_to_amps, x, B, kSrcCh, T, 0, ea, xmax)));
    if (amps_ready) TVC_HIP(ctx, hipEventRecord(amps_ready, s));
    EpiBias<ACT_ELU1, false> ek{kern, ctx->src_to_kernel.bias, nullptr, kBins, T, ncols, (long)kBins * T, 0};
    TVC_CHECK((gemm_s_launch<2, 4, 2>(ctx, s, ctx->src_to_kernel, x, B, kSrcCh, T, 0, ek, xmax)));
    return launch_check(ctx, "source_net");
}

static int run_harm_sums(tvc_ctx* ctx, hipStream_t s, const float* f0, double* csum, int B, int T) {
    const long L = (long)T * kHop;
    const int NB = ctx->rag ? ctx->rag->B : B;
    const int Tg = ctx->rag ? ctx->rag->Tlong : T;
    RagDev rg;
    TVC_CHECK(rag_view(ctx, s, 1, 0, &rg, nullptr));
    const float scale_size = (float)T / (float)L;
    hipLaunchKernelGGL(harm_frame_sum_kernel, dim3((Tg + 3) / 4, NB), dim3(256), 0, s, f0, csum, T, scale_size, rg);
    hipLaunchKernelGGL(harm_frame_scan_kernel, dim3(kHarm, NB), dim3(64), 0, s, csum, T, rg);
    return launch_check(ctx, "harm_sums");
}

int run_dsp(tvc_ctx* ctx, hipStream_t s, Ws& ws, const float* f0, const float* amps, const float* kern, const float* angle, uint64_t seed, float* source, int B, int T,
            float* smax, double* csum, const DspFork* fk) {
    const long L = (long)T * kHop;
    if (!csum) csum = ws.get<double>((size_t)B * kHarm * T);
    float* frames = ws.get<float>((size_t)B * T * kNfft);
    const int NB = ctx->rag ? ctx->rag->B : B;
    const int Tg = ctx->rag ? ctx->rag->Tlong : T;
    float* smax_own = smax ? nullptr : ws.get<float>((size_t)NB);
    if (ws.dry) return 0;
    if (!smax) {
        smax = smax_own;
        TVC_HIP(ctx, hipMemsetAsync(smax, 0, (size_t)NB * sizeof(float), s));
    }
    RagDev rg;
    TVC_CHECK(rag_view(ctx, s, 1, 0, &rg, nullptr));
    const float scale_size = (float)T / (float)L;
    const float scale_amp = (float)(1.0 / (double)kHop);
    hipStream_t sh = s;
    if (fk) {
        sh = fk->side;
        TVC_HIP(ctx, hipStreamWaitEvent(sh, fk->amps_ready, 0));
    } else {
        TVC_CHECK(run_harm_sums(ctx, s, f0, csum, B, T));
    }
    hipLaunchKernelGGL(harm_synth_kernel, dim3((Tg + 3) / 4, NB), dim3(256), 0, sh, f0, amps, csum, source, T, scale_size, scale_amp, rg);
    TVC_CHECK(run_amax_rows(ctx, sh, amps, B, kHarm, T, smax));
    TVC_CHECK(run_noise_ifft(ctx, s, kern, angle, seed, frames, B, T, ctx->rag && angle));
    hipLaunchKernelGGL(noise_ola_kernel, dim3(grid_for((long)Tg * kHop / 4, 256, NB >= 32 ? 16 : 512 / NB), NB), dim3(256), 0, s, frames, source, B, T, smax, rg);
    return launch_check(ctx, "dsp");
}

static int plain_conv(tvc_ctx* ctx, hipStream_t s, const PackedW& w, const float* x, int B, int Cin, int len, int dil, float* y, const BfpSlots& bfp, int lin = 0,
                      float lscale = 0.f) {
    int rc = 0;
    if ((lin > 0 ? conv_s2_try<true>(&rc, ctx, s, w, x, B, Cin, len, dil, y, bfp, lin, lscale) : conv_s2_try<false>(&rc, ctx, s, w, x, B, Cin, len, dil, y, bfp)))
        return rc;
    if (lin > 0)
        return conv3s_launch<true, C3EpiBias<false>, false, true>(ctx, s, w, x, B, Cin, len, dil, C3EpiBias<false>{y, w.bias, nullptr, w.M, len}, bfp, nullptr, nullptr,
                                                                   nullptr, 0, lin, lscale);
    return conv3s_launch<true>(ctx, s, w, x, B, Cin, len, dil, C3EpiBias<false>{y, w.bias, nullptr, w.M, len}, bfp);
}

static int film_conv(tvc_ctx* ctx, hipStream_t s, const PackedW& w, const PackedW& fw, const FilmU& fu, const float* h, const float* cond, int B, int C, int len, int dil,
                     float* out, const float* bsc, const float* bsh, const float* res, int res_lin, float res_scale, const BfpSlots& bfp) {
    int rc = 0;
    if (rag_min_len(ctx, len) >= FS2::BN && film_s2_try(&rc, ctx, s, fu, h, cond, B, C, len, dil, out, res, res_lin, res_scale, bfp)) return rc;
    return conv3s_launch<true, C3EpiFilmFused, true>(ctx, s, w, h, B, C, len, dil, C3EpiFilmFused{out, w.bias, bsc, bsh, res, C, len, res_lin, res_scale}, bfp, &fw, &fw,
                                                     cond, C);
}

static int conv_film_half(tvc_ctx* ctx, hipStream_t s, const PackedW& ca, const PackedW& cb, const PackedW& fw, const FilmU& fu, const float* x, int lin, float lscale,
                          int da, int db, float* h, const float* cond, int B, int C, int len, float* out, const float* bsc, const float* bsh, const float* res,
                          int res_lin, float res_scale, const float* ma_in, float* mh, const float* mcond, float* mout) {
    const bool pre = rag_min_len(ctx, len) >= FS2::BN && fu.img && fu.C == C && fu.hb_w > 0.f && C % 96 == 0 && C <= 384 && ma_in && mcond && res && db >= 1 && db <= FS2::MAXD &&
                     (long)C * len * 4 < (1L << 32) && (res_lin <= 0 || (long)C * res_lin * 4 < (1L << 32));
    if (pre) {
        int rc = 0;
        const BfpSlots in{ma_in, nullptr, nullptr};
        const bool ok = lin > 0 ? conv_s2_try<true, true>(&rc, ctx, s, ca, x, B, C, len, da, h, in, lin, lscale, fu.hb_w, fu.hb_b)
                                : conv_s2_try<false, true>(&rc, ctx, s, ca, x, B, C, len, da, h, in, 0, 0.f, fu.hb_w, fu.hb_b);
        if (ok) {
            TVC_CHECK(rc);
            if (!film_s2_try(&rc, ctx, s, fu, h, cond, B, C, len, db, out, res, res_lin, res_scale, BfpSlots{ma_in, mcond, mout}, true, fu.hb_w, fu.hb_b))
                return fail(ctx, TVC_ERR_STATE, "filter_net: the FiLM conv refused the pre-split operand its producer wrote");
            return rc;
        }
    }
    TVC_CHECK(plain_conv(ctx, s, ca, x, B, C, len, da, h, BfpSlots{ma_in, nullptr, mh}, lin, lscale));
    return film_conv(ctx, s, cb, fw, fu, h, cond, B, C, len, db, out, bsc, bsh, res, res_lin, res_scale, BfpSlots{mh, mcond, mout});
}

static __global__ void g8_to_planar_kernel(const float* __restrict__ x, float* __restrict__ y, long B, long l, int C) {
    const long n = B * C * l;
    for (long i = blockIdx.x * (long)blockDim.x + threadIdx.x; i < n; i += (long)gridDim.x * blockDim.x) {
        const long t = i % l, bc = i / l, c = bc % C, b = bc / C;
        y[i] = x[((b * (C / 8) + c / 8) * l + t) * 8 + (c & 7)];
    }
}

static int filter_input_gemm(tvc_ctx* ctx, hipStream_t s, const float* content, const float* f0, float* x, int B, int T, const float* cmax) {
    EpiSumCond ep{x, ctx->flt_content_in.bias, nullptr, f0, nullptr, nullptr, ctx->flt_f_w, ctx->flt_f_b, 384, T, B * T};
    int rc = 0;
    if (!gemm_s2_try(&rc, ctx, s, ctx->flt_content_in, content, B, kSslDim, T, 0, ep, cmax)) rc = gemm_s_launch<2, 4, 2>(ctx, s, ctx->flt_content_in, content, B, kSslDim, T, 0, ep, cmax);
    return rc;
}

int run_filter(tvc_ctx* ctx, hipStream_t s, Ws& ws, const float* content, const float* f0,
               const float* energy, const float* source, float* wave, int B, int T, const FilterTaps* taps, const float* cmax, const float* smax, float* zeroed_slots, bool x_slot_set,
               float* x_pre, bool x_pre_filled) {
    const long L = (long)T * kHop;
    static const int ch[5] = {384, 192, 96, 48, 24};
    const long len_dn[5] = {L, L / 5, L / 20, L / 80, L / 240};
    float* skip[5];
    for (int i = 0; i < 5; ++i) skip[i] = ws.get<float>((size_t)B * ch[4 - i] * len_dn[i]);
    float* x = x_pre ? x_pre : ws.get<float>((size_t)B * ch[0] * T);
    float* xi_pre[5] = {nullptr, nullptr, nullptr, nullptr, nullptr};
    for (int i = 1; i <= 4; ++i) xi_pre[i] = ws.get<float>((size_t)B * ctx->downs[i - 1].cin * len_dn[i]);
    for (int i = 1; i < 4; ++i)
        if (len_dn[i] % ctx->downs[i].factor != 0 || (ctx->downs[i].factor == 4 && len_dn[i] % 4 != 0))
            return fail(ctx, TVC_ERR_ARG, "filter_net: level lengths must divide by the next Downsample factor");

    enum { S_CONTENT = 0, S_SRC, S_X, S_SKIP0, S_DH1 = S_SKIP0 + 5, S_DH2 = S_DH1 + 4, S_UHA = S_DH2 + 4, S_UX1 = S_UHA + 5, S_UHB = S_UX1 + 5, S_UXU = S_UHB + 5,
           S_LEV = S_UXU + 5, S_COUNT = S_LEV + 5 };
    const int NB = ctx->rag ? ctx->rag->B : B;
    static_assert(S_COUNT == kFilterSlots && S_X == kFilterSlotX, "tvc_common.h kFilterSlots / kFilterSlotX");
    float* slots = zeroed_slots ? zeroed_slots : ws.get<float>((size_t)S_COUNT * NB);
    auto slot = [&](int i) { return slots + (size_t)i * NB; };

    if (!ws.dry) {
        ProfScope ps(ctx, s, ws, "filter.in+down0");
        if (!zeroed_slots) TVC_HIP(ctx, hipMemsetAsync(slots, 0, (size_t)S_COUNT * NB * sizeof(float), s));
        if (!cmax) {
            TVC_CHECK(run_amax_rows(ctx, s, content, B, kSslDim, T, slot(S_CONTENT)));
            cmax = slot(S_CONTENT);
        }
        if (!smax) {
            TVC_CHECK(run_amax_rows(ctx, s, source, B, 16, L, slot(S_SRC)));
            TVC_CHECK(run_amax_rows(ctx, s, energy, B, 1, L, slot(S_SRC)));
            smax = slot(S_SRC);
        }
        if (!x_pre_filled) TVC_CHECK(filter_input_gemm(ctx, s, content, f0, x, B, T, cmax));
        if (!(zeroed_slots && x_slot_set)) TVC_CHECK(run_slot_affine(ctx, s, slot(S_X), cmax, 1, ctx->flt_in_bw, ctx->flt_in_bb, NB));
        TVC_CHECK(run_down0_split(ctx, s, ctx->flt_down0s, source, energy, skip[0], taps ? taps->skips[0] : nullptr, xi_pre[1], B, (int)L, smax, slot(S_SKIP0)));
    }
    for (int i = 1; i <= 4; ++i) {
        const DownW& d = ctx->downs[i - 1];
        const int len = (int)len_dn[i];
        size_t mk = ws.mark();
        float* xi = xi_pre[i];
        float* h1 = d.cin == 24 ? nullptr : ws.get<float>((size_t)B * d.cin * len);
        float* h2 = d.cin == 24 ? nullptr : ws.get<float>((size_t)B * d.cin * len);
        if (!ws.dry) {
            static const char* names[4] = {"filter.down1", "filter.down2", "filter.down3", "filter.down4"};
            ProfScope ps(ctx, s, ws, names[i - 1]);
            float* y2 = i < 4 ? xi_pre[i + 1] : nullptr;
            const int f2 = i < 4 ? ctx->downs[i].factor : 0;
            const float* mxi = slot(S_SKIP0 + i - 1);
            float *mh1 = slot(S_DH1 + i - 1), *mh2 = slot(S_DH2 + i - 1), *mout = slot(S_SKIP0 + i);
            if (d.cin == 24) {
                TVC_CHECK(run_down24_fused(ctx, s, d, xi, skip[i], y2, B, len, mxi, mout));
            } else {
                if (d.cin == 48) {
                    TVC_CHECK(run_conv48_pair(ctx, s, d.c1, d.c2, xi, 0, 0.f, nullptr, nullptr, nullptr, nullptr, h2, B, len, 1, 2, mxi, nullptr, mh2));
                } else {
                    TVC_CHECK(plain_conv(ctx, s, d.c1, xi, B, d.cin, len, 1, h1, BfpSlots{mxi, nullptr, mh1}));
                    TVC_CHECK(plain_conv(ctx, s, d.c2, h1, B, d.cin, len, 2, h2, BfpSlots{mh1, nullptr, mh2}));
                }
                TVC_CHECK((conv3s_launch<true, C3EpiBiasResConv>(ctx, s, d.c3, h2, B, d.cin, len, 4,
                                                                 C3EpiBiasResConv{{skip[i], d.c3res_bias, nullptr, d.cout, len, y2, f2}},
                                                                 BfpSlots{mh2, mxi, mout}, &d.res, nullptr, xi, d.cin)));
            }
        }
        ws.release(mk);
    }
    float* xlev[5];
    {
        long l = T;
        for (int i = 0; i < 5; ++i) {
            l *= ctx->ups[i].factor;
            xlev[i] = ws.get<float>((size_t)B * ctx->ups[i].cout * l);
        }
    }
    long len = T;
    const float* mx_in = slot(S_X);
    for (int i = 0; i < 5; ++i) {
        const UpW& u = ctx->ups[i];
        const int lin = (int)len;
        len *= u.factor;
        const int lo = (int)len, C = u.cin, nc = B * lo;
        const float* cond = skip[4 - i];
        const float* mcond = slot(S_SKIP0 + 4 - i);
        size_t mk = ws.mark();
        float* xu = ws.get<float>((size_t)B * C * lo);
        float* h = ws.get<float>((size_t)B * C * lo);
        float* x1 = ws.get<float>((size_t)B * C * lo);
        if (!ws.dry && C == 24) {
            ProfScope ps(ctx, s, ws, "filter.up4+out");
            TVC_CHECK(run_up24_split(ctx, s, u, x, cond, ctx->down0_bw, ctx->down0_bb, x1, wave, B, lo, mx_in, smax, slot(S_UX1 + i)));
        } else if (!ws.dry) {
            static const char* names[4] = {"filter.up0", "filter.up1", "filter.up2", "filter.up3"};
            ProfScope ps(ctx, s, ws, names[i]);
            const float lscale = (float)(1.0 / (double)u.factor);
            for (int half = 0; half < 2; ++half) {
                const PackedW& ca = half ? u.c3 : u.c1;
                const PackedW& cb = half ? u.c4 : u.c2;
                const PackedW& fw = half ? u.film2 : u.film1;
                const float* bsc = fw.bias;
                const float* bsh = fw.bias + C;
                const int da = half ? 9 : 1, db = half ? 27 : 3;
                float* xout = half ? xu : x1;
                const float* ma_in = half ? slot(S_UX1 + i) : mx_in;
                float* mh = slot((half ? S_UHB : S_UHA) + i);
                float* mout = slot((half ? S_UXU : S_UX1) + i);
                if (C == 48) {
                    if (half == 0) {
                        TVC_CHECK(run_conv48_pair(ctx, s, ca, cb, x, lin, lscale, &fw, bsc, bsh, cond, xout, B, lo, da, db, ma_in, mcond, mout));
                    } else {
                        TVC_CHECK(run_conv48s(ctx, s, ca, x1, nullptr, nullptr, nullptr, nullptr, nullptr, h, B, lo, da, ma_in, nullptr, mh));
                        TVC_CHECK(run_conv48s(ctx, s, cb, h, &fw, bsc, bsh, cond, x1, nullptr, B, lo, db, mh, mcond, slot(S_LEV + i), &u.c5, xlev[i]));
                    }
                } else if (half == 0) {
                    TVC_CHECK(conv_film_half(ctx, s, ca, cb, fw, u.fu1, x, lin, lscale, da, db, h, cond, B, C, lo, xout, bsc, bsh, x, lin, lscale, ma_in, mh, mcond, mout));
                } else {
                    TVC_CHECK(conv_film_half(ctx, s, ca, cb, fw, u.fu2, x1, 0, 0.f, da, db, h, cond, B, C, lo, xout, bsc, bsh, x1, 0, 0.f, ma_in, mh, mcond, mout));
                }
            }
            if (C != 48) {
                EpiBias<ACT_NONE, false> ep{xlev[i], u.c5.bias, nullptr, u.cout, lo, nc, (long)u.cout * lo, 0, slot(S_LEV + i), slot(S_UXU + i), u.c5_bw, u.c5_bb, NB};
                if (u.cout == 48) {
                    EpiBiasG8 eg{xlev[i], u.c5.bias, u.cout, lo, nc, slot(S_LEV + i), slot(S_UXU + i), u.c5_bw, u.c5_bb, NB};
                    TVC_CHECK((gemm_s_launch<2, 4, 2>(ctx, s, u.c5, xu, B, C, lo, 0, eg, slot(S_UXU + i))));
                } else if (u.c5.MT6 % 3 == 0) TVC_CHECK((gemm_s_launch<3, 4, 1>(ctx, s, u.c5, xu, B, C, lo, 0, ep, slot(S_UXU + i))));
                else TVC_CHECK((gemm_s_launch<2, 4, 2>(ctx, s, u.c5, xu, B, C, lo, 0, ep, slot(S_UXU + i))));
            }
        }
        ws.release(mk);
        x = xlev[i];
        mx_in = slot(S_LEV + i);
    }
    if (!ws.dry && taps) {
        for (int i = 1; i < 5; ++i)
            if (taps->skips[i] && i == 1)
                hipLaunchKernelGGL(g8_to_planar_kernel, dim3(grid_for((long)B * 48 * len_dn[1])), dim3(256), 0, s, skip[1], taps->skips[1], (long)B, len_dn[1], 48);
            else if (taps->skips[i])
                TVC_HIP(ctx, hipMemcpyAsync(taps->skips[i], skip[i], (size_t)B * ch[4 - i] * len_dn[i] * sizeof(float), hipMemcpyDeviceToDevice, s));
        long l = T;
        for (int i = 0; i < 4; ++i) {
            l *= ctx->ups[i].factor;
            if (taps->ups[i] && ctx->ups[i].cout <= 48)
                hipLaunchKernelGGL(g8_to_planar_kernel, dim3(grid_for((long)B * ctx->ups[i].cout * l)), dim3(256), 0, s, xlev[i], taps->ups[i], (long)B, l, ctx->ups[i].cout);
            else if (taps->ups[i])
                TVC_HIP(ctx, hipMemcpyAsync(taps->ups[i], xlev[i], (size_t)B * ctx->ups[i].cout * l * sizeof(float), hipMemcpyDeviceToDevice, s));
        }
    }
    return ws.dry ? 0 : launch_check(ctx, "filter_net");
}

int run_decoder(tvc_ctx* ctx, hipStream_t s, Ws& ws, const float* content, const float* f0,
                const float* energy, const float* angle, uint64_t seed, float* wave, float* amps_out,
                float* kernel_out, float* source_out, int B, int T, const float* content_bound, const float* energy_bound,
                int content_bound_stride) {
    const long L = (long)T * kHop;
    float* amps = amps_out ? amps_out : ws.get<float>((size_t)B * kHarm * T);
    float* kern = kernel_out ? kernel_out : ws.get<float>((size_t)B * kBins * T);
    float* source = source_out ? source_out : ws.get<float>((size_t)B * 16 * L);
    const int NB = ctx->rag ? ctx->rag->B : B;
    float* cmax = ws.get<float>((size_t)(3 + kFilterSlots) * NB);
    float* smax = cmax + NB;
    float* xmax = smax + NB;
    float* fslots = xmax + NB;
    float* x0 = ws.get<float>((size_t)B * 384 * T);
    double* csum = ws.get<double>((size_t)B * kHarm * T);
    if (!ws.dry) {
        TVC_CHECK(run_slot_prep(ctx, s, cmax, (3 + kFilterSlots) * NB, content_bound ? cmax : nullptr, content_bound, content_bound_stride, 1.f, 0.f, energy_bound ? smax : nullptr,
                                energy_bound, 1, 1.f, 0.f, content_bound ? fslots + (size_t)kFilterSlotX * NB : nullptr, ctx->flt_in_bw, ctx->flt_in_bb,
                                NB));
        if (!content_bound) TVC_CHECK(run_amax_rows(ctx, s, content, B, kSslDim, T, cmax));
        if (!energy_bound) TVC_CHECK(run_amax_rows(ctx, s, energy, B, 1, L, smax));
    }
    SideFork fk(ctx, s);
    if (wave) TVC_CHECK(fk.fork(ws, ctx->ev_fork2, ctx->ev_join2));
    if (fk.forked()) {
        TVC_CHECK(run_harm_sums(ctx, fk.side, f0, csum, B, T));
        ProfScope ps(ctx, fk.side, ws, "filter_net.input@side");
        TVC_CHECK(filter_input_gemm(ctx, fk.side, content, f0, x0, B, T, cmax));
    }
    size_t mk = ws.mark();
    {
        ProfScope ps(ctx, s, ws, "source_net");
        TVC_CHECK(run_source_net(ctx, s, ws, content, f0, energy, amps, kern, B, T, cmax, xmax, fk.forked() ? ctx->ev_amps : nullptr));
    }
    ws.release(mk);
    if (!wave && !source_out) return 0;
    {
        ProfScope ps(ctx, s, ws, "dsp");
        const DspFork df{fk.side, ctx->ev_amps};
        TVC_CHECK(run_dsp(ctx, s, ws, f0, amps, kern, angle, seed, source, B, T, smax, csum, fk.forked() ? &df : nullptr));
        TVC_CHECK(fk.join());
    }
    ws.release(mk);
    if (!wave) return 0;
    ProfScope ps(ctx, s, ws, "filter_net");
    TVC_CHECK(run_filter(ctx, s, ws, content, f0, energy, source, wave, B, T, nullptr, cmax, smax, fslots, content_bound != nullptr, x0, fk.forked()));
    ws.release(mk);
    return 0;
}

}
```

tinyvc_amd/csrc/film_s2.h:

```cpp
#pragma once
#include "conv_s2.h"
#include "split_fp16.h"

namespace tvc {


struct FilmS2Args {
    const uint4* img;
    const float* tab;
    const float* x;
    const float* cond;
    int C, len, dil;
    float* y;
    const float* res;
    int res_lin;
    float res_scale;
    int tiles_per_utt, ntiles, mblocks;
    const float* amax_x;
    const float* amax_c;
    float* amax_y;
    const uint4* xpre;
    float pre_w, pre_b;
    RagDev rag;
};

template <int NWV_>
struct FS2T {
    static constexpr int MTB = 3, MW = 1, WM = MTB / MW, NWV = NWV_, WN = 1, NW = MW * NWV, NTHR = NW * 64, BN = NWV * WN * 32, MAXD = 27, XROW = BN + 2 * MAXD;
    static constexpr int A_CONV = 3 * MTB * 2, A_PIECES = A_CONV + 2 * MTB * 2, A_PER = (A_PIECES + NW - 1) / NW;
    static constexpr int XS = (2 * XROW + NTHR - 1) / NTHR;
    static constexpr int A_U4 = A_PIECES * 64, X_U4 = 2 * 2 * XROW, C_U4 = 2 * 2 * BN, BUF_U4 = A_U4 + X_U4 + C_U4;
    static constexpr int lds_bytes = 2 * BUF_U4 * 16 + 6 * 384 * 4 + 64;
    static_assert(2 * BN <= NTHR, "one cond item per thread");
};
using FS2 = FS2T<8>;

__device__ __forceinline__ void split8u(const float (&v)[8], uint4& p1, uint4& p2) {
    unsigned o1[4], o2[4];
#pragma unroll
    for (int j = 0; j < 4; ++j) split2<false>(v[2 * j], v[2 * j + 1], o1[j], o2[j]);
    p1 = make_uint4(o1[0], o1[1], o1[2], o1[3]);
    p2 = make_uint4(o2[0], o2[1], o2[2], o2[3]);
}

template <bool XPRE, bool RAG = false, int NWV_ = 8>
__global__ __launch_bounds__(FS2T<NWV_>::NTHR) __attribute__((amdgpu_waves_per_eu(2))) void film_s2_kernel(FilmS2Args a) {
    using TL = FS2T<NWV_>;
    constexpr int MTB = TL::MTB, WM = TL::WM, NWV = TL::NWV, WN = TL::WN, NW = TL::NW, BN = TL::BN, XROW = TL::XROW, A_PER = TL::A_PER, XS = TL::XS;
    extern __shared__ __attribute__((aligned(16))) uint4 smem_fs[];
    float* Tb = reinterpret_cast<float*>(smem_fs + 2 * TL::BUF_U4);
    float* red = Tb + 6 * 384;
    const int tid = threadIdx.x, lane = tid & 63;
    const int wave = __builtin_amdgcn_readfirstlane(tid >> 6);
    const int l31 = lane & 31, lh = lane >> 5;
    const int wm = wave / NWV, wn = wave - wm * NWV;
    const int C = a.C, nslab = C / 16, rs = a.len, dil = a.dil;
    const int rf = a.res_lin > 0 ? rs / a.res_lin : 1;
    const int xw = BN + 2 * dil, nitems = 2 * xw;

    for (int i = tid; i < 6 * C; i += TL::NTHR) {
        const int r = i / C;
        Tb[r * 384 + (i - r * C)] = a.tab[i];
    }

    int tfirst, tlast;
    tile_range(a.ntiles, tfirst, tlast);
    if (tfirst >= tlast) return;
    auto coords = [&](int v, int& mb, int& b, int& t0, int& len, int& off) __attribute__((always_inline)) {
        const int nt = v / a.mblocks;
        mb = v - nt * a.mblocks;
        const RagTile rt = rag_tile<RAG>(a.rag, nt, a.tiles_per_utt, rs, b);
        b = rt.b;
        t0 = rt.tin * BN;
        len = rt.len;
        off = rt.off;
    };

    u32x4 ar[A_PER];
    float xr[XPRE ? 1 : XS][8], cr[8];
    uint4 xq[XPRE ? XS : 1][2];
    auto item_of = [&](int t_, int k, int& g, int& c) __attribute__((always_inline)) {
        int item = t_ + k * TL::NTHR;
        item = item < nitems ? item : item - nitems;
        g = item / xw;
        c = item - g * xw;
    };
    int xdst[XS];
#pragma unroll
    for (int k = 0; k < XS; ++k) {
        int g, c;
        item_of(tid, k, g, c);
        xdst[k] = g * XROW + c;
    }
    const int cg = tid >= BN ? 1 : 0, cc = tid - cg * BN;
    const int cdst = cg * BN + cc;
    unsigned xo[XS], co = 0;
    float xs = 1.f, cs_ = 1.f;
    float rxs = 1.f, rcs = 1.f;
    int lv = tfirst, ls = 0, lmb, lb = 0, lt0, llen, loff;
    coords(lv, lmb, lb, lt0, llen, loff);
    auto tile_offsets = [&]() __attribute__((always_inline)) {
        const int ub = RAG ? loff : 0;
        int tl = tid;
        asm volatile("" : "+v"(tl));
#pragma unroll
        for (int k = 0; k < XS; ++k) {
            int g, c;
            item_of(tl, k, g, c);
            int p = lt0 - dil + c;
            p = p < 0 ? 0 : (p > llen - 1 ? llen - 1 : p);
            xo[k] = (unsigned)((XPRE ? 1 : 8) * g * rs + ub + p);
        }
        int pc = lt0 + cc;
        pc = pc > llen - 1 ? llen - 1 : pc;
        co = (unsigned)(8 * cg * rs + ub + pc);
        xs = XPRE ? 1.f : norm_from_amax(sload_f32(a.amax_x + lb)).s;
        cs_ = norm_from_amax(sload_f32(a.amax_c + lb)).s;
    };
    tile_offsets();
    auto issue_load = [&]() __attribute__((always_inline)) {
        const uint4* abase = a.img + ((long)lmb * nslab + ls) * (TL::A_PIECES * 64);
#pragma unroll
        for (int i = 0; i < A_PER; ++i) {
            int q = wave + i * NW;
            q = q < TL::A_PIECES ? q : TL::A_PIECES - 1;
            ar[i] = ldg_so4(abase, 16u * (unsigned)(q * 64 + lane));
        }
        const long ubase = RAG ? 0L : (long)lb * C;
        const float* xc = a.x + (ubase + (long)ls * 16) * rs;
        const float* cc_ = a.cond + (ubase + (long)ls * 16) * rs;
        if (XPRE) {
            const uint4* xp = a.xpre + ((RAG ? 0L : (long)lb * 2 * (C >> 3)) + 2 * ls) * rs;
#pragma unroll
            for (int k = 0; k < XS; ++k) {
                const unsigned e = xo[k];
                xq[k][0] = __builtin_bit_cast(uint4, ldg_so4(xp, 16u * e));
                xq[k][1] = __builtin_bit_cast(uint4, ldg_so4(xp + (long)(C >> 3) * rs, 16u * e));
            }
        } else {
#pragma unroll
            for (int k = 0; k < XS; ++k)
#pragma unroll
                for (int j = 0; j < 8; ++j) xr[k][j] = ldg_so(xc + (long)j * rs, 4u * xo[k]);
        }
#pragma unroll
        for (int j = 0; j < 8; ++j) cr[j] = ldg_so(cc_ + (long)j * rs, 4u * co);
        rxs = xs;
        rcs = cs_;
    };
    auto advance_load = [&]() __attribute__((always_inline)) {
        if (++ls == nslab) {
            if (lv + 1 < tlast) {
                ++lv;
                ls = 0;
                coords(lv, lmb, lb, lt0, llen, loff);
                tile_offsets();
            } else {
                ls = nslab - 1;
            }
        }
    };
    auto lstore = [&](int buf) __attribute__((always_inline)) {
        uint4* Ab = smem_fs + buf * TL::BUF_U4;
        uint4* Xb = Ab + TL::A_U4;
        uint4* Cb = Xb + TL::X_U4;
#pragma unroll
        for (int i = 0; i < A_PER; ++i) {
            int q = wave + i * NW;
            q = q < TL::A_PIECES ? q : TL::A_PIECES - 1;
            *reinterpret_cast<u32x4*>(Ab + q * 64 + lane) = ar[i];
        }
        float v[8];
        uint4 p1, p2;
#pragma unroll
        for (int k = 0; k < XS; ++k) {
            if (XPRE) {
                p1 = xq[k][0];
                p2 = xq[k][1];
            } else {
#pragma unroll
                for (int j = 0; j < 8; ++j) v[j] = fmaxf(xr[k][j], 0.1f * xr[k][j]) * rxs;
                split8u(v, p1, p2);
            }
            Xb[xdst[k]] = p1;
            Xb[2 * XROW + xdst[k]] = p2;
        }
#pragma unroll
        for (int j = 0; j < 8; ++j) v[j] = cr[j] * rcs;
        split8u(v, p1, p2);
        Cb[cdst] = p1;
        Cb[2 * BN + cdst] = p2;
    };

    f32x16 hi[WM][WN], sc[WM][WN], sh[WM][WN];
#pragma unroll
    for (int i = 0; i < WM; ++i)
#pragma unroll
        for (int j = 0; j < WN; ++j)
#pragma unroll
            for (int r = 0; r < 16; ++r) hi[i][j][r] = sc[i][j][r] = sh[i][j][r] = 0.f;
    auto tap_mul = [&](int buf, int tap) __attribute__((always_inline)) {
        const uint4* Ab = smem_fs + buf * TL::BUF_U4 + ((tap * MTB + wm * WM) * 2) * 64 + lane;
        const uint4* Xb = smem_fs + buf * TL::BUF_U4 + TL::A_U4 + lh * XROW + wn * WN * 32 + l31 + tap * dil;
        f16x8 bf[WN][2];
#pragma unroll
        for (int j = 0; j < WN; ++j)
#pragma unroll
            for (int p = 0; p < 2; ++p) bf[j][p] = __builtin_bit_cast(f16x8, Xb[p * 2 * XROW + j * 32]);
#pragma unroll
        for (int i = 0; i < WM; ++i) {
            f16x8 af[2];
#pragma unroll
            for (int p = 0; p < 2; ++p) af[p] = __builtin_bit_cast(f16x8, Ab[(i * 2 + p) * 64]);
#pragma unroll
            for (int j = 0; j < WN; ++j) hi[i][j] = TVC_MFMA16(af[1], bf[j][0], hi[i][j]);
#pragma unroll
            for (int j = 0; j < WN; ++j) hi[i][j] = TVC_MFMA16(af[0], bf[j][1], hi[i][j]);
#pragma unroll
            for (int j = 0; j < WN; ++j) hi[i][j] = TVC_MFMA16(af[0], bf[j][0], hi[i][j]);
        }
    };
    auto film_mul = [&](int buf) __attribute__((always_inline)) {
        const uint4* Ab = smem_fs + buf * TL::BUF_U4 + (TL::A_CONV + wm * WM * 2) * 64 + lane;
        const uint4* Cb = smem_fs + buf * TL::BUF_U4 + TL::A_U4 + TL::X_U4 + lh * BN + wn * WN * 32 + l31;
        f16x8 bf[WN][2];
#pragma unroll
        for (int j = 0; j < WN; ++j)
#pragma unroll
            for (int p = 0; p < 2; ++p) bf[j][p] = __builtin_bit_cast(f16x8, Cb[p * 2 * BN + j * 32]);
#pragma unroll
        for (int i = 0; i < WM; ++i) {
            f16x8 af[2], ag[2];
#pragma unroll
            for (int p = 0; p < 2; ++p) af[p] = __builtin_bit_cast(f16x8, Ab[(i * 2 + p) * 64]);
#pragma unroll
            for (int p = 0; p < 2; ++p) ag[p] = __builtin_bit_cast(f16x8, Ab[((MTB + i) * 2 + p) * 64]);
#pragma unroll
            for (int j = 0; j < WN; ++j) {
                sc[i][j] = TVC_MFMA16(af[1], bf[j][0], sc[i][j]);
                sh[i][j] = TVC_MFMA16(ag[1], bf[j][0], sh[i][j]);
            }
#pragma unroll
            for (int j = 0; j < WN; ++j) {
                sc[i][j] = TVC_MFMA16(af[0], bf[j][1], sc[i][j]);
                sh[i][j] = TVC_MFMA16(ag[0], bf[j][1], sh[i][j]);
            }
#pragma unroll
            for (int j = 0; j < WN; ++j) {
                sc[i][j] = TVC_MFMA16(af[0], bf[j][0], sc[i][j]);
                sh[i][j] = TVC_MFMA16(ag[0], bf[j][0], sh[i][j]);
            }
        }
    };

    int cv = tfirst, cs = 0, cmb, cb = 0, ct0, len, coff;
    coords(cv, cmb, cb, ct0, len, coff);
    float mx_run = 0.f;
    int flush_b = -1;

    issue_load();
    advance_load();
    lstore(0);
    issue_load();
    advance_load();
    slab_barrier();
    int buf = 0;
    while (true) {
        tap_mul(buf, 0);
        lstore(buf ^ 1);
        issue_load();
        tap_mul(buf, 1);
        tap_mul(buf, 2);
        film_mul(buf);
        advance_load();
        if (++cs == nslab) {
            cs = 0;
            int el = lane;
            asm volatile("" : "+v"(el));
            const int e31 = el & 31, eh = el >> 5;
            const float ix = norm_from_amax(XPRE ? presplit_bound(a.pre_w, a.pre_b, a.amax_x, cb) : sload_f32(a.amax_x + cb)).inv, ic_ = norm_from_amax(sload_f32(a.amax_c + cb)).inv;
#pragma unroll
            for (int i = 0; i < WM; ++i) {
            const int row0 = (cmb * MTB + wm * WM + i) * 32;
            const float kc = Tb[FilmU::TAB_SCALE * 384 + row0] * ix, ks = Tb[FilmU::TAB_SSC * 384 + row0] * ic_, kh = Tb[FilmU::TAB_SSH * 384 + row0] * ic_;
#pragma unroll
            for (int g = 0; g < 4; ++g) {
                const int rr = row0 + 8 * g + 4 * eh;
                const float4 b0 = *reinterpret_cast<const float4*>(Tb + FilmU::TAB_BIAS * 384 + rr);
                const float4 b1 = *reinterpret_cast<const float4*>(Tb + FilmU::TAB_BSC * 384 + rr);
                const float4 b2 = *reinterpret_cast<const float4*>(Tb + FilmU::TAB_BSH * 384 + rr);
                const float bm[4] = {b0.x, b0.y, b0.z, b0.w}, bs[4] = {b1.x, b1.y, b1.z, b1.w}, bh[4] = {b2.x, b2.y, b2.z, b2.w};
#pragma unroll
                for (int q = 0; q < 4; ++q)
#pragma unroll
                    for (int j = 0; j < WN; ++j) {
                        const int r = 4 * g + q;
                        const float h = fmaf(hi[i][j][r], kc, bm[q]), s = fmaf(sc[i][j][r], ks, bs[q]), t = fmaf(sh[i][j][r], kh, bh[q]);
                        hi[i][j][r] = __fadd_rn(__fmul_rn(h, s), t);
                        sc[i][j][r] = 0.f;
                        sh[i][j][r] = 0.f;
                    }
            }
            float* yb = RAG ? a.y + (long)row0 * rs + coff : a.y + ((long)cb * C + row0) * rs;
#pragma unroll
            for (int j = 0; j < WN; ++j) {
                const int t = ct0 + (wn * WN + j) * 32 + e31;
                const bool live = t < len;
                const int tc = live ? t : len - 1;
                const unsigned off = 4u * (unsigned)(4 * eh * rs + tc);
                if (a.res_lin > 0) {
                    const Lerp lc = lerp_coord(tc, a.res_scale, RAG ? len / rf : a.res_lin);
                    const float* rb = RAG ? a.res + (long)row0 * a.res_lin + coff / rf : a.res + ((long)cb * C + row0) * a.res_lin;
                    const unsigned o0 = 4u * (unsigned)(4 * eh * a.res_lin + lc.i0), o1 = 4u * (unsigned)(4 * eh * a.res_lin + lc.i1);
#pragma unroll
                    for (int h8 = 0; h8 < 2; ++h8) {
                        float x0[8], x1[8];
#pragma unroll
                        for (int r = 0; r < 8; ++r) {
                            const float* rr = rb + (long)(16 * h8 + (r & 3) + 8 * (r >> 2)) * a.res_lin;
                            x0[r] = ldg_so(rr, o0);
                            x1[r] = ldg_so(rr, o1);
                        }
#pragma unroll
                        for (int r = 0; r < 8; ++r) hi[i][j][8 * h8 + r] = __fadd_rn(hi[i][j][8 * h8 + r], lerp_eval(lc, x0[r], x1[r]));
                    }
                } else {
                    const float* rb = RAG ? a.res + (long)row0 * rs + coff : a.res + ((long)cb * C + row0) * rs;
                    float rv[16];
#pragma unroll
                    for (int r = 0; r < 16; ++r) rv[r] = ldg_so(rb + (long)((r & 3) + 8 * (r >> 2)) * rs, off);
#pragma unroll
                    for (int r = 0; r < 16; ++r) hi[i][j][r] = __fadd_rn(hi[i][j][r], rv[r]);
                }
#pragma unroll
                for (int r = 0; r < 16; ++r) {
                    const float e = hi[i][j][r];
                    if (live) {
                        stg_so(yb + (long)((r & 3) + 8 * (r >> 2)) * rs, off, e);
                        mx_run = fmaxf(mx_run, fabsf(e));
                    }
                    hi[i][j][r] = 0.f;
                }
            }
            }
            const int done_b = cb;
            ++cv;
            const bool last = cv >= tlast;
            if (!last) coords(cv, cmb, cb, ct0, len, coff);
            if (a.amax_y && (last || cb != done_b)) {
                const float m = wave_max(mx_run);
                if (lane == 0) red[wave] = m;
                mx_run = 0.f;
                flush_b = done_b;
            }
            if (last) break;
        }
        slab_barrier();
        if (flush_b >= 0) {
            if (tid == 0) {
                float m = 0.f;
                for (int w = 0; w < NW; ++w) m = fmaxf(m, red[w]);
                if (m > 0.f) atomicMax(reinterpret_cast<unsigned*>(a.amax_y + flush_b), __builtin_bit_cast(unsigned, m));
            }
            flush_b = -1;
        }
        buf ^= 1;
    }
    if (flush_b >= 0) {
        slab_barrier();
        if (tid == 0) {
            float m = 0.f;
            for (int w = 0; w < NW; ++w) m = fmaxf(m, red[w]);
            if (m > 0.f) atomicMax(reinterpret_cast<unsigned*>(a.amax_y + flush_b), __builtin_bit_cast(unsigned, m));
        }
    }
}

inline bool film_s2_try(int* rc, tvc_ctx* ctx, hipStream_t s, const FilmU& fu, const float* h, const float* cond, int B, int C, int len, int dil, float* out,
                        const float* res, int res_lin, float res_scale, const BfpSlots& bfp, bool pre = false, float pre_w = 0.f, float pre_b = 0.f) {
    if (!fu.img || fu.C != C || C % 96 != 0 || C > 384 || dil < 1 || dil > FS2::MAXD || !bfp.x || !bfp.c || !res) return false;
    if ((long)C * len * 4 >= (1L << 32) || (res_lin > 0 && (long)C * res_lin * 4 >= (1L << 32))) return false;
    if ((*rc = lds_optin<film_s2_kernel<false>, film_s2_kernel<true>, film_s2_kernel<false, true>, film_s2_kernel<true, true>>(ctx, FS2::lds_bytes, "film_s2")) ||
        (*rc = lds_optin<film_s2_kernel<false, false, 7>, film_s2_kernel<true, false, 7>>(ctx, FS2T<7>::lds_bytes, "film_s2")))
        return true;
    FilmS2Args a{};
    a.img = reinterpret_cast<const uint4*>(fu.img);
    a.tab = fu.tab;
    a.x = h;
    a.cond = cond;
    a.C = C;
    a.len = len;
    a.dil = dil;
    a.y = out;
    a.res = res;
    a.res_lin = res_lin;
    a.res_scale = res_scale;
    a.mblocks = C / 96;
    a.tiles_per_utt = (len + FS2::BN - 1) / FS2::BN;
    a.amax_x = bfp.x;
    a.xpre = reinterpret_cast<const uint4*>(h);
    a.pre_w = pre_w;
    a.pre_b = pre_b;
    a.amax_c = bfp.c;
    a.amax_y = bfp.y;
    int ncol = a.tiles_per_utt * B;
    if ((*rc = rag_tiles(ctx, s, B, len, FS2::BN, &a.rag, &ncol, "film_s2"))) return true;
    a.ntiles = ncol * a.mblocks;
    const int grid = a.ntiles < ctx->ncu ? a.ntiles : ctx->ncu;
    if (ctx->rag) {
        if (pre) hipLaunchKernelGGL((film_s2_kernel<true, true>), dim3(grid), dim3(FS2::NTHR), FS2::lds_bytes, s, a);
        else hipLaunchKernelGGL((film_s2_kernel<false, true>), dim3(grid), dim3(FS2::NTHR), FS2::lds_bytes, s, a);
    } else if ((len + 223) / 224 * 224 < (len + 255) / 256 * 256) {
        a.tiles_per_utt = (len + 223) / 224;
        a.ntiles = a.tiles_per_utt * B * a.mblocks;
        const int g7 = a.ntiles < ctx->ncu ? a.ntiles : ctx->ncu;
        if (pre) hipLaunchKernelGGL((film_s2_kernel<true, false, 7>), dim3(g7), dim3(FS2T<7>::NTHR), FS2T<7>::lds_bytes, s, a);
        else hipLaunchKernelGGL((film_s2_kernel<false, false, 7>), dim3(g7), dim3(FS2T<7>::NTHR), FS2T<7>::lds_bytes, s, a);
    } else if (pre) hipLaunchKernelGGL(film_s2_kernel<true>, dim3(grid), dim3(FS2::NTHR), FS2::lds_bytes, s, a);
    else hipLaunchKernelGGL(film_s2_kernel<false>, dim3(grid), dim3(FS2::NTHR), FS2::lds_bytes, s, a);
    *rc = launch_check(ctx, "film_s2");
    return true;
}

}
```

tinyvc_amd/csrc/pack.hip:

```cpp
#include <algorithm>
#include <cmath>

#include "tvc_common.h"

namespace tvc {

size_t ArenaBuilder::put(const float** slot, const float* v, size_t n) {
    const size_t off = (buf.size() + 63) & ~size_t(63);
    buf.resize(off + n, 0.f);
    std::copy(v, v + n, buf.begin() + off);
    fix.push_back({slot, off});
    return off;
}

namespace {

int pad_m(int M) {
    if (M <= 32) return 32;
    if (M <= 64) return 64;
    if (M <= 96) return 96;
    if (M % 96 == 0 && M % 128 != 0) return M;
    return (M + 127) / 128 * 128;
}

uint16_t f16_bits(float f) {
    const _Float16 h = (_Float16)f;
    uint16_t u;
    std::memcpy(&u, &h, 2);
    return u;
}
float f16_value(uint16_t u) {
    _Float16 h;
    std::memcpy(&h, &u, 2);
    return (float)h;
}
void split2(float w, float scale, uint16_t* h1, uint16_t* h2) {
    const float x = w / scale;
    *h1 = f16_bits(x);
    *h2 = f16_bits((x - f16_value(*h1)) * 2048.f);
}
float pow2_scale(float amax) {
    if (!(amax > 0.f) || !std::isfinite(amax)) return 1.f;
    int e;
    std::frexp(amax, &e);
    return std::ldexp(1.f, e - 1);
}
float amax(const float* v, size_t n) {
    float a = 0.f;
    for (size_t i = 0; i < n; ++i) a = std::max(a, std::fabs(v[i]));
    return a;
}
struct RowL1 {
    double w = 0.0, b = 0.0;
};
RowL1 row_l1(const float* w, const float* b, int M, int K) {
    RowL1 r;
    for (int m = 0; m < M; ++m) {
        double sum = 0.0;
        for (int k = 0; k < K; ++k) sum += std::fabs((double)w[(size_t)m * K + k]);
        r.w = std::max(r.w, sum);
        r.b = std::max(r.b, std::fabs((double)b[m]));
    }
    return r;
}

void put_k24(std::vector<float>& img, int piece0, int step_stride, const float* w, int M, int CI, int taps, const float* scale) {
    uint16_t* o = reinterpret_cast<uint16_t*>(img.data());
    for (int s = 0; 2 * s < 3 * taps; ++s)
        for (int mt = 0; 32 * mt < M; ++mt)
            for (int lane = 0; lane < 64; ++lane)
                for (int j = 0; j < 8; ++j) {
                    const int u = 2 * s + (lane >> 5), tap = u / 3, ci = 8 * (u % 3) + j, m = 32 * mt + (lane & 31);
                    const float v = (u < 3 * taps && m < M && ci < CI) ? w[((size_t)m * CI + ci) * taps + tap] : 0.f;
                    const size_t base = ((size_t)(piece0 + s * step_stride + 2 * mt) * 64 + lane) * 8 + j;
                    split2(v, scale[mt], &o[base], &o[base + 512]);
                }
}

struct Packer {
    tvc_ctx* ctx;
    ArenaBuilder& ab;
    std::string missing;
    std::map<const PackedW*, std::vector<float>> host_wscale;

    void note(const std::string& what) {
        if (missing.empty()) missing = what;
    }
    const HostTensor* find(const std::string& key) {
        auto it = ctx->host.find(key);
        if (it != ctx->host.end()) return &it->second;
        note(key);
        return nullptr;
    }
    const float* get(const std::string& key, size_t n) {
        const HostTensor* t = find(key);
        if (t && t->data.size() != n) note(key + " (wrong size)");
        return t && t->data.size() == n ? t->data.data() : nullptr;
    }
    void raw(const std::string& key, const float** slot, size_t n) {
        if (const float* v = get(key, n)) ab.put(slot, v, n);
    }
    void bound(const std::string& name, int M, int K, float* bw, float* bb) {
        const float* w = get(name + ".weight", (size_t)M * K);
        const float* b = get(name + ".bias", M);
        if (!w || !b) return;
        const RowL1 r = row_l1(w, b, M, K);
        *bw = (float)(r.w * 1.0001);
        *bb = (float)(r.b * 1.0001);
    }

    bool stage(const std::vector<std::string>& names, PackedW* pw, int cin, int taps, std::vector<float>* At, std::vector<float>* bias, int* group_rows) {
        int M = 0;
        std::vector<const HostTensor*> ws, bs;
        for (auto& n : names) {
            const HostTensor* w = find(n + ".weight");
            const HostTensor* b = find(n + ".bias");
            if (!w || !b) return false;
            if (w->shape.size() != 3 || w->shape[1] != cin || w->shape[2] != taps ||
                (int64_t)b->data.size() != w->shape[0]) {
                note(n + " (unexpected shape)");
                return false;
            }
            ws.push_back(w);
            bs.push_back(b);
            M += (int)w->shape[0];
        }
        pw->M = M;
        pw->K = cin * taps;
        pw->cin = cin;
        pw->taps = taps;
        pw->Mpad = pad_m(M);
        pw->Kpad = (pw->K + 15) / 16 * 16;
        At->assign((size_t)pw->Kpad * pw->Mpad, 0.f);
        bias->assign(pw->Mpad, 0.f);
        int m0 = 0;
        for (size_t i = 0; i < ws.size(); ++i) {
            int cout = (int)ws[i]->shape[0];
            for (int m = 0; m < cout; ++m) {
                (*bias)[m0 + m] = bs[i]->data[m];
                for (int k = 0; k < pw->K; ++k) (*At)[(size_t)k * pw->Mpad + m0 + m] = ws[i]->data[(size_t)m * pw->K + k];
            }
            m0 += cout;
        }
        bool equal_groups = ws.size() > 1;
        for (auto* w : ws) equal_groups = equal_groups && w->shape[0] == ws[0]->shape[0];
        *group_rows = equal_groups ? (int)ws[0]->shape[0] : 0;
        return true;
    }
    static int image_mt(const PackedW* pw, int group_rows) {
        const int gp = group_rows > 0 ? (group_rows + 31) / 32 * 32 : 0;
        return group_rows > 0 ? (pw->M / group_rows) * gp / 32 : pw->Mpad / 32;
    }
    static int image_row(const PackedW* pw, int group_rows, int m) {
        if (group_rows <= 0) return m < pw->M ? m : pw->M;
        const int gp = (group_rows + 31) / 32 * 32, g = m / gp, mi = m - g * gp;
        return mi < group_rows ? g * group_rows + mi : pw->M;
    }
    std::vector<float> mt_amax(const PackedW* pw, const std::vector<float>& At, int group_rows) {
        const int MT = image_mt(pw, group_rows);
        std::vector<float> amax(MT, 0.f);
        for (int mt = 0; mt < MT; ++mt)
            for (int r = 0; r < 32; ++r) {
                const int m = image_row(pw, group_rows, mt * 32 + r);
                if (m >= pw->M) continue;
                for (int k = 0; k < pw->K; ++k) amax[mt] = std::max(amax[mt], std::fabs(At[(size_t)k * pw->Mpad + m]));
            }
        return amax;
    }
    void conv(const std::vector<std::string>& names, PackedW* pw, int cin, int taps) {
        std::vector<float> At, bias;
        int group_rows = 0;
        if (!stage(names, pw, cin, taps, &At, &bias, &group_rows)) return;
        ab.put(&pw->bias, bias);
        std::vector<float> sc = mt_amax(pw, At, group_rows);
        for (auto& v : sc) v = pow2_scale(v);
        a6(pw, At, group_rows, sc);
    }
    void conv_joint(const std::string& na, PackedW* pa, int cin_a, int taps_a, const std::string& nb, PackedW* pb, int cin_b, int taps_b) {
        std::vector<float> Aa, ba, Ab, bb;
        int ga = 0, gb = 0;
        if (!stage({na}, pa, cin_a, taps_a, &Aa, &ba, &ga) || !stage({nb}, pb, cin_b, taps_b, &Ab, &bb, &gb)) return;
        if (pa->Mpad != pb->Mpad) return note(na + " / " + nb + " (row counts differ)");
        ab.put(&pa->bias, ba);
        ab.put(&pb->bias, bb);
        std::vector<float> sa = mt_amax(pa, Aa, 0), sb = mt_amax(pb, Ab, 0);
        for (size_t i = 0; i < sa.size(); ++i) sa[i] = pow2_scale(std::max(sa[i], sb[i]));
        const size_t off_a = a6(pa, Aa, 0, sa);
        a6(pb, Ab, 0, sa);
        ab.fix.push_back({&pb->wjoint, off_a});
    }
    size_t a6(PackedW* pw, const std::vector<float>& At, int group_rows, const std::vector<float>& scale) {
        const int taps = pw->taps, cin = pw->cin, nslab = ((cin + 15) / 16 + 5) / 6 * 6;
        const int MT = image_mt(pw, group_rows);
        std::vector<float> img((size_t)nslab * taps * MT * 2 * 256, 0.f);
        uint16_t* o = reinterpret_cast<uint16_t*>(img.data());
        for (int s = 0; s < nslab; ++s)
            for (int tap = 0; tap < taps; ++tap)
                for (int mt = 0; mt < MT; ++mt)
                    for (int lane = 0; lane < 64; ++lane)
                        for (int j = 0; j < 8; ++j) {
                            const int ci = s * 16 + 8 * (lane >> 5) + j, m = image_row(pw, group_rows, mt * 32 + (lane & 31));
                            const float w = (ci < cin && m < pw->M) ? At[(size_t)(ci * taps + tap) * pw->Mpad + m] : 0.f;
                            const size_t base = (((size_t)(s * taps + tap) * MT + mt) * 2 * 64 + lane) * 8 + j;
                            split2(w, scale[mt], &o[base], &o[base + 512]);
                        }
        pw->MT6 = MT;
        pw->S6 = nslab;
        const size_t off = ab.put(&pw->A6, img);
        ab.put(&pw->wscale, scale);
        host_wscale[pw] = scale;
        return off;
    }
    void film_u(FilmU* fu, const std::string& conv_name, const std::string& film, int C, const std::string& first_conv) {
        const size_t CC = (size_t)C * C;
        const float* w = get(conv_name + ".weight", 3 * CC);
        const float* b = get(conv_name + ".bias", C);
        const float* wsc = get(film + ".to_scale.weight", CC);
        const float* bsc = get(film + ".to_scale.bias", C);
        const float* wsh = get(film + ".to_shift.weight", CC);
        const float* bsh = get(film + ".to_shift.bias", C);
        if (!w || !b || !wsc || !bsc || !wsh || !bsh) return;
        const int MT = C / 32, nslab = C / 16, mblocks = C / 96;
        auto tile_scale = [&](const float* wt, int per_row, int mt) { return pow2_scale(amax(wt + (size_t)mt * 32 * per_row, (size_t)32 * per_row)) * (1.f / 8192.f); };
        std::vector<float> tab((size_t)6 * C);
        auto row = [&](int r) { return &tab[(size_t)r * C]; };
        float *scale_conv = row(FilmU::TAB_SCALE), *scale_sc = row(FilmU::TAB_SSC), *scale_sh = row(FilmU::TAB_SSH);
        std::copy(b, b + C, row(FilmU::TAB_BIAS));
        std::copy(bsc, bsc + C, row(FilmU::TAB_BSC));
        std::copy(bsh, bsh + C, row(FilmU::TAB_BSH));
        for (int mt = 0; mt < MT; ++mt) {
            std::fill_n(scale_conv + 32 * mt, 32, tile_scale(w, 3 * C, mt));
            std::fill_n(scale_sc + 32 * mt, 32, tile_scale(wsc, C, mt));
            std::fill_n(scale_sh + 32 * mt, 32, tile_scale(wsh, C, mt));
        }
        std::vector<float> img((size_t)mblocks * nslab * 30 * 64 * 4, 0.f);
        uint16_t* o = reinterpret_cast<uint16_t*>(img.data());
        for (int mb = 0; mb < mblocks; ++mb)
            for (int s = 0; s < nslab; ++s)
                for (int q = 0; q < 30; ++q) {
                    const bool conv = q < 18;
                    const int qq = conv ? q : q - 18, grp = qq / 6, mi = (qq % 6) / 2, part = qq % 2, mt = mb * 3 + mi;
                    for (int lane = 0; lane < 64; ++lane)
                        for (int j = 0; j < 8; ++j) {
                            const int m = mt * 32 + (lane & 31), ci = s * 16 + 8 * (lane >> 5) + j;
                            float x;
                            if (conv) x = w[((size_t)m * C + ci) * 3 + grp] / scale_conv[m];
                            else if (grp == 0) x = wsc[(size_t)m * C + ci] / scale_sc[m];
                            else x = wsh[(size_t)m * C + ci] / scale_sh[m];
                            const uint16_t h1 = f16_bits(x);
                            o[((((size_t)mb * nslab + s) * 30 + q) * 64 + lane) * 8 + j] = part == 0 ? h1 : f16_bits(x - f16_value(h1));
                        }
                }
        bound(first_conv, C, 3 * C, &fu->hb_w, &fu->hb_b);
        fu->C = C;
        ab.put(&fu->img, img);
        ab.put(&fu->tab, tab);
    }
    void up24s_half(const float** slot, const std::string& ca, const std::string& cb, const std::string& film, const std::string& c5,
                    const std::string& out7) {
        using L = Up24sBlob;
        constexpr int C = 24;
        const float* wa = get(ca + ".weight", C * C * 3);
        const float* ba = get(ca + ".bias", C);
        const float* wb = get(cb + ".weight", C * C * 3);
        const float* bb = get(cb + ".bias", C);
        const float* wsc = get(film + ".to_scale.weight", C * C);
        const float* bsc = get(film + ".to_scale.bias", C);
        const float* wsh = get(film + ".to_shift.weight", C * C);
        const float* bsh = get(film + ".to_shift.bias", C);
        if (!wa || !ba || !wb || !bb || !wsc || !bsc || !wsh || !bsh) return;
        std::vector<float> img(L::PIECES * 256 + L::FLOATS, 0.f);
        float* fl = img.data() + L::PIECES * 256;
        fl[L::SA] = pow2_scale(amax(wa, C * C * 3));
        fl[L::SB] = pow2_scale(amax(wb, C * C * 3));
        fl[L::SSC] = pow2_scale(amax(wsc, C * C));
        fl[L::SSH] = pow2_scale(amax(wsh, C * C));
        put_k24(img, 0, 2, wa, C, C, 3, &fl[L::SA]);
        put_k24(img, 10, 2, wb, C, C, 3, &fl[L::SB]);
        put_k24(img, 20, 4, wsc, C, C, 1, &fl[L::SSC]);
        put_k24(img, 22, 4, wsh, C, C, 1, &fl[L::SSH]);
        std::copy(ba, ba + C, fl + L::BA);
        std::copy(bb, bb + C, fl + L::BB);
        std::copy(bsc, bsc + C, fl + L::BSC);
        std::copy(bsh, bsh + C, fl + L::BSH);
        const RowL1 r = row_l1(wa, ba, C, C * 3);
        fl[L::L1A] = (float)(r.w * 1.0000002);
        fl[L::BMA] = (float)r.b;
        if (!c5.empty()) {
            const float* w5 = get(c5 + ".weight", C * C);
            const float* b5 = get(c5 + ".bias", C);
            const float* w7 = get(out7 + ".weight", C * 7);
            const float* b7 = get(out7 + ".bias", 1);
            if (!w5 || !b5 || !w7 || !b7) return;
            double bias = b7[0];
            for (int c = 0; c < C; ++c)
                for (int j = 0; j < 7; ++j) {
                    double acc = 0.0;
                    for (int m = 0; m < C; ++m) acc += (double)w7[(size_t)m * 7 + j] * (double)w5[(size_t)m * C + c];
                    fl[L::W75 + c * 7 + j] = (float)acc;
                }
            for (int m = 0; m < C; ++m)
                for (int j = 0; j < 7; ++j) bias += (double)w7[(size_t)m * 7 + j] * (double)b5[m];
            fl[L::B75] = (float)bias;
        }
        ab.put(slot, img);
    }
    void down0s(const float** slot, const std::string& name, float* bound_w, float* bound_b) {
        using L = Down0sBlob;
        constexpr int C = 24, CI = 17;
        const float* w = get(name + ".weight", C * CI * 3);
        const float* b = get(name + ".bias", C);
        if (!w || !b) return;
        std::vector<float> img(L::PIECES * 256 + L::FLOATS, 0.f);
        float* fl = img.data() + L::PIECES * 256;
        fl[L::SCALE] = pow2_scale(amax(w, C * CI * 3));
        put_k24(img, 0, 2, w, C, CI, 3, &fl[L::SCALE]);
        std::copy(b, b + C, fl + L::BIAS);
        const RowL1 r = row_l1(w, b, C, CI * 3);
        fl[L::BW] = *bound_w = (float)(r.w * 1.0001);
        fl[L::BB] = *bound_b = (float)r.b * 1.0001f;
        ab.put(slot, img);
    }
    void conv24s(const float** slot, const std::string& name, int M, const std::string& extra_bias = "", const PackedW* joint = nullptr) {
        constexpr int CI = 24;
        const int MT = (M + 31) / 32;
        const float* w = get(name + ".weight", (size_t)M * CI * 3);
        const float* b = get(name + ".bias", M);
        const float* eb = extra_bias.empty() ? nullptr : get(extra_bias, M);
        if (!w || !b || (!extra_bias.empty() && !eb)) return;
        std::vector<float> img((size_t)K24_PIECES * MT * 256 + Conv24sBlob::FLOATS, 0.f);
        float* fl = img.data() + (size_t)K24_PIECES * MT * 256;
        float* sc = fl + Conv24sBlob::SCALE;
        if (joint) {
            auto it = host_wscale.find(joint);
            if (it == host_wscale.end() || (int)it->second.size() != MT) return note(name + " (its joint image is not packed yet)");
            std::copy(it->second.begin(), it->second.end(), sc);
        } else {
            for (int mt = 0; mt < MT; ++mt) sc[mt] = pow2_scale(amax(w + (size_t)32 * mt * CI * 3, (size_t)(std::min(M, 32 * mt + 32) - 32 * mt) * CI * 3));
        }
        put_k24(img, 0, 2 * MT, w, M, CI, 3, sc);
        for (int m = 0; m < M; ++m) fl[Conv24sBlob::BIAS + m] = b[m] + (eb ? eb[m] : 0.f);
        ab.put(slot, img);
    }
    void convnext(const std::string& p, ConvNeXtW* w, int C, int dil) {
        w->C = C;
        w->dilation = dil;
        raw(p + ".c1.weight", &w->dw_w, (size_t)C * 7);
        raw(p + ".c1.bias", &w->dw_b, C);
        const float* g = get(p + ".norm.gamma", C);
        const float* bt = get(p + ".norm.beta", C);
        if (g) ab.put(&w->ln_g, g, C);
        if (bt) ab.put(&w->ln_b, bt, C);
        if (g && bt) {
            const RowL1 r = row_l1(g, bt, C, 1);
            w->ln_bound = std::sqrt((float)C) * (float)r.w + (float)r.b;
        }
        conv({p + ".c2"}, &w->c2, C, 1);
        raw(p + ".grn.gamma", &w->grn_g, 2 * C);
        raw(p + ".grn.beta", &w->grn_b, 2 * C);
        conv({p + ".c3"}, &w->c3, 2 * C, 1);
        const float* w3 = get(p + ".c3.weight", (size_t)C * 2 * C);
        const float* b3 = get(p + ".c3.bias", C);
        const float* gb = get(p + ".grn.beta", 2 * C);
        if (w3 && b3 && gb) {
            std::vector<float> fb(w->c3.Mpad, 0.f);
            for (int m = 0; m < C; ++m) {
                double acc = b3[m];
                for (int k = 0; k < 2 * C; ++k) acc += (double)w3[(size_t)m * 2 * C + k] * (double)gb[k];
                fb[m] = (float)acc;
            }
            ab.put(&w->c3_bias_grn, fb);
        }
    }
};

}

void pack_constants(tvc_ctx* ctx, ArenaBuilder* ab) {
    const int N = kNfft;
    const double two_pi = 6.283185307179586476925286766559;
    std::vector<float> t960(2 * 960), t1920(2 * 961 + 2), hann(N);
    for (int j = 0; j < 960; ++j) {
        t960[2 * j] = (float)std::cos(two_pi * j / 960.0);
        t960[2 * j + 1] = (float)std::sin(two_pi * j / 960.0);
    }
    for (int k = 0; k <= 960; ++k) {
        t1920[2 * k] = (float)std::cos(two_pi * k / 1920.0);
        t1920[2 * k + 1] = (float)std::sin(two_pi * k / 1920.0);
    }
    for (int n = 0; n < N; ++n) hann[n] = (float)(0.5 - 0.5 * std::cos(two_pi * n / N));
    ab->put(&ctx->fft_tw960, t960);
    ab->put(&ctx->fft_tw1920, t1920);
    ab->put(&ctx->fft_hann, hann);
    ab->put(&ctx->sola_part, std::vector<float>(kSolaPartFloats, 0.f));
}

void pack_checkpoint(tvc_ctx* ctx, ArenaBuilder* ab, std::string* missing_enc, std::string* missing_dec) {
    Packer pk{ctx, *ab};
    if (ctx->pitch_table.size() == (size_t)kPitchClasses)
        ab->put(&ctx->pitch_freq, ctx->pitch_table);
    else
        pk.missing = "pitch table (tvc_set_pitch_table)";

    pk.conv({"ssl_feature_estimator.input_layer", "pitch_estimator.input_layer"}, &ctx->enc_in, kBins, 1);
    pk.raw("ssl_feature_estimator.norm.gamma", &ctx->ssl_ln_g, kSslCh);
    pk.raw("ssl_feature_estimator.norm.beta", &ctx->ssl_ln_b, kSslCh);
    pk.raw("pitch_estimator.norm.gamma", &ctx->pit_ln_g, kPitchCh);
    pk.raw("pitch_estimator.norm.beta", &ctx->pit_ln_b, kPitchCh);
    static const int ssl_dil[6] = {1, 3, 9, 1, 1, 1};
    for (int i = 0; i < 6; ++i)
        pk.convnext("ssl_feature_estimator.mid_layers." + std::to_string(i), &ctx->ssl_mid[i], kSslCh, ssl_dil[i]);
    for (int i = 0; i < 4; ++i)
        pk.convnext("pitch_estimator.mid_layers." + std::to_string(i), &ctx->pit_mid[i], kPitchCh, 1);
    pk.conv({"ssl_feature_estimator.output_layer"}, &ctx->ssl_out, kSslCh, 1);
    pk.conv({"pitch_estimator.output_layer"}, &ctx->pit_out, kPitchCh, 1);
    *missing_enc = pk.missing;
    pk.missing.clear();

    pk.conv({"source_net.content_in"}, &ctx->src_content_in, kSslDim, 1);
    pk.raw("source_net.energy_in.weight", &ctx->src_e_w, kSrcCh);
    pk.raw("source_net.energy_in.bias", &ctx->src_e_b, kSrcCh);
    pk.raw("source_net.f0_in.weight", &ctx->src_f_w, kSrcCh);
    pk.raw("source_net.f0_in.bias", &ctx->src_f_b, kSrcCh);
    for (int i = 0; i < 3; ++i)
        pk.convnext("source_net.mid_layers." + std::to_string(i), &ctx->src_mid[i], kSrcCh, 1);
    pk.conv({"source_net.to_amps"}, &ctx->src_to_amps, kSrcCh, 1);
    pk.conv({"source_net.to_kernel"}, &ctx->src_to_kernel, kSrcCh, 1);

    static const int ch[5] = {384, 192, 96, 48, 24};
    static const int fac[5] = {2, 3, 4, 4, 5};
    pk.conv({"filter_net.content_in"}, &ctx->flt_content_in, kSslDim, 1);
    pk.raw("filter_net.f0_in.weight", &ctx->flt_f_w, ch[0]);
    pk.raw("filter_net.f0_in.bias", &ctx->flt_f_b, ch[0]);
    pk.bound("filter_net.content_in", ch[0], kSslDim, &ctx->flt_in_bw, &ctx->flt_in_bb);
    {
        const float* fw = pk.get("filter_net.f0_in.weight", ch[0]);
        const float* fb = pk.get("filter_net.f0_in.bias", ch[0]);
        if (fw && fb) {
            const RowL1 r = row_l1(fw, fb, ch[0], 1);
            ctx->flt_in_bb += (float)((r.w * 89.0 + r.b) * 1.0001);
        }
    }
    pk.down0s(&ctx->flt_down0s, "filter_net.downs.0", &ctx->down0_bw, &ctx->down0_bb);
    for (int i = 1; i <= 4; ++i) {
        DownW& d = ctx->downs[i - 1];
        d.cin = ch[5 - i];
        d.cout = ch[4 - i];
        d.factor = fac[5 - i];
        std::string p = "filter_net.downs." + std::to_string(i);
        pk.conv_joint(p + ".c3", &d.c3, d.cin, 3, p + ".down_res", &d.res, d.cin, 1);
        if (d.cin == 24) {
            pk.conv24s(&d.s24c1, p + ".c1", 24);
            pk.conv24s(&d.s24c2, p + ".c2", 24);
            pk.conv24s(&d.s24c3r, p + ".c3", 48, p + ".down_res.bias", &d.c3);
            pk.bound(p + ".c1", 24, 72, &d.b1_w, &d.b1_b);
            pk.bound(p + ".c2", 24, 72, &d.b2_w, &d.b2_b);
            continue;
        }
        pk.conv({p + ".c1"}, &d.c1, d.cin, 3);
        pk.conv({p + ".c2"}, &d.c2, d.cin, 3);
        const float* b3 = pk.get(p + ".c3.bias", d.cout);
        const float* br = pk.get(p + ".down_res.bias", d.cout);
        if (b3 && br) {
            std::vector<float> sum(d.c3.Mpad, 0.f);
            for (int m = 0; m < d.cout; ++m) sum[m] = b3[m] + br[m];
            ab->put(&d.c3res_bias, sum);
        }
    }
    for (int i = 0; i < 5; ++i) {
        UpW& u = ctx->ups[i];
        u.cin = ch[i];
        u.cout = i < 4 ? ch[i + 1] : ch[4];
        u.factor = fac[i];
        std::string p = "filter_net.ups." + std::to_string(i);
        if (u.cin == 24) {
            pk.up24s_half(&u.s24a, p + ".c1", p + ".c2", p + ".film1", "", "");
            pk.up24s_half(&u.s24b, p + ".c3", p + ".c4", p + ".film2", p + ".c5", "filter_net.output_layer");
            continue;
        }
        pk.conv({p + ".c1"}, &u.c1, u.cin, 3);
        pk.conv({p + ".c2"}, &u.c2, u.cin, 3);
        pk.conv({p + ".c3"}, &u.c3, u.cin, 3);
        pk.conv({p + ".c4"}, &u.c4, u.cin, 3);
        pk.conv({p + ".c5"}, &u.c5, u.cin, 1);
        pk.bound(p + ".c5", u.cout, u.cin, &u.c5_bw, &u.c5_bb);
        pk.conv({p + ".film1.to_scale", p + ".film1.to_shift"}, &u.film1, u.cin, 1);
        pk.conv({p + ".film2.to_scale", p + ".film2.to_shift"}, &u.film2, u.cin, 1);
        if (u.cin >= 96) {
            pk.film_u(&u.fu1, p + ".c2", p + ".film1", u.cin, p + ".c1");
            pk.film_u(&u.fu2, p + ".c4", p + ".film2", u.cin, p + ".c3");
        }
    }
    *missing_dec = pk.missing;
}

}
```

tinyvc_amd/csrc/split_fp16.h:

```cpp
#pragma once
#include "tvc_common.h"

namespace tvc {

typedef _Float16 f16x8 __attribute__((ext_vector_type(8)));
typedef _Float16 f16x2v __attribute__((ext_vector_type(2)));
typedef float f32x2 __attribute__((ext_vector_type(2)));
typedef float f32x16 __attribute__((ext_vector_type(16)));
typedef unsigned u32x4 __attribute__((ext_vector_type(4)));

constexpr int kParts = 2;
constexpr int kPU4 = kParts * 64;
constexpr float kLoScale = 2048.f;
constexpr float kLoInv = 1.f / 2048.f;

struct Bfp {
    float s, inv;
};
__device__ __forceinline__ Bfp bfp_from_amax(float amax) {
    const unsigned u = __builtin_bit_cast(unsigned, amax);
    int e = (int)(u >> 23) - 127;
    Bfp r{1.f, 1.f};
    if (u != 0u && u < 0x7f800000u && (e >= 15 || e < -10)) {
        e = e > 100 ? 100 : (e < -100 ? -100 : e);
        r.s = __builtin_bit_cast(float, (unsigned)(127 - e) << 23);
        r.inv = __builtin_bit_cast(float, (unsigned)(127 + e) << 23);
    }
    return r;
}
__device__ __forceinline__ Bfp bfp_load(const float* amax, int b) { return amax ? bfp_from_amax(amax[b]) : Bfp{1.f, 1.f}; }
__device__ __forceinline__ float sload_f32(const float* p) {
    float v;
    asm volatile("s_load_dword %0, %1, 0x0\n\ts_waitcnt lgkmcnt(0)" : "=s"(v) : "s"(p) : "memory");
    return v;
}
__device__ __forceinline__ Bfp bfp_load_u(const float* amax, int b) { return amax ? bfp_from_amax(sload_f32(amax + b)) : Bfp{1.f, 1.f}; }
__device__ __forceinline__ Bfp bfp_min(const Bfp& a, const Bfp& b) { return a.s < b.s ? a : b; }
__device__ __forceinline__ float wave_max(float mx) {
#pragma unroll
    for (int o = 32; o > 0; o >>= 1) mx = fmaxf(mx, __shfl_xor(mx, o));
    return mx;
}
__device__ __forceinline__ void amax_flush_wg(float* slot, float mx, float* red) {
    mx = wave_max(mx);
    int tid = threadIdx.x;
    asm volatile("" : "+v"(tid));
    if ((tid & 63) == 0) red[tid >> 6] = mx;
    asm volatile("s_waitcnt lgkmcnt(0)\n\ts_barrier" ::: "memory");
    if (tid == 0) {
        float m = 0.f;
        for (int w = 0; w < (int)(blockDim.x >> 6); ++w) m = fmaxf(m, red[w]);
        if (m > 0.f) atomicMax(reinterpret_cast<unsigned*>(slot), __builtin_bit_cast(unsigned, m));
    }
}
__device__ __forceinline__ void tile_range(int ntiles, int& first, int& last) {
    first = (int)((long)ntiles * blockIdx.x / gridDim.x);
    last = (int)((long)ntiles * (blockIdx.x + 1) / gridDim.x);
}

typedef const __attribute__((address_space(1))) float* gcf32;
typedef __attribute__((address_space(1))) float* gf32;
__device__ __forceinline__ float ldg_so(const float* base, unsigned byte_off) {
    gcf32 p = (gcf32)base;
    asm("" : "+s"(p));
    return *reinterpret_cast<gcf32>(reinterpret_cast<const __attribute__((address_space(1))) char*>(p) + byte_off);
}
__device__ __forceinline__ void stg_so(float* base, unsigned byte_off, float v) {
    gf32 p = (gf32)base;
    asm("" : "+s"(p));
    *reinterpret_cast<gf32>(reinterpret_cast<__attribute__((address_space(1))) char*>(p) + byte_off) = v;
}
__device__ __forceinline__ void stg_so4(float* base, unsigned byte_off, const float (&v)[4]) {
    typedef float f32x4g __attribute__((ext_vector_type(4)));
    typedef __attribute__((address_space(1))) f32x4g* gf4;
    gf32 p = (gf32)base;
    asm("" : "+s"(p));
    *reinterpret_cast<gf4>(reinterpret_cast<__attribute__((address_space(1))) char*>(p) + byte_off) = f32x4g{v[0], v[1], v[2], v[3]};
}
__device__ __forceinline__ u32x4 ldg_so4(const uint4* base, unsigned byte_off) {
    typedef const __attribute__((address_space(1))) u32x4* gcu4;
    gcu4 p = (gcu4)base;
    asm("" : "+s"(p));
    return *reinterpret_cast<gcu4>(reinterpret_cast<const __attribute__((address_space(1))) char*>(p) + byte_off);
}

template <bool SCALED = true>
__device__ __forceinline__ void split2(float v0, float v1, unsigned& p1, unsigned& p2) {
    const f32x2 a = {v0, v1};
    p1 = __builtin_bit_cast(unsigned, __builtin_convertvector(a, f16x2v));
    const f32x2 b = SCALED ? a * kLoScale : a;
    const float ns = SCALED ? -kLoScale : -1.f;
    unsigned r;
    asm("v_fma_mixlo_f16 %0, %1, %2, %3 op_sel_hi:[1,0,0]" : "=v"(r) : "v"(p1), "s"(ns), "v"(b[0]));
    asm("v_fma_mixhi_f16 %0, %1, %2, %3 op_sel:[1,0,0] op_sel_hi:[1,0,0]" : "+v"(r) : "v"(p1), "s"(ns), "v"(b[1]));
    p2 = r;
}
__device__ __forceinline__ void split8(const float (&v)[8], uint4& p1, uint4& p2) {
    unsigned o1[4], o2[4];
#pragma unroll
    for (int j = 0; j < 4; ++j) split2(v[2 * j], v[2 * j + 1], o1[j], o2[j]);
    p1 = make_uint4(o1[0], o1[1], o1[2], o1[3]);
    p2 = make_uint4(o2[0], o2[1], o2[2], o2[3]);
}
#define TVC_MFMA16(a, b, c) __builtin_amdgcn_mfma_f32_32x32x16_f16(a, b, c, 0, 0, 0)
__device__ __forceinline__ float comb(float hi, float lo, float c, float clo) { return fmaf(lo, clo, hi * c); }

__device__ __forceinline__ void slab_barrier() { asm volatile("s_waitcnt lgkmcnt(0)\n\ts_barrier" ::: "memory"); }

struct BfpSlots {
    const float* x = nullptr;
    const float* c = nullptr;
    float* y = nullptr;
};

static __global__ __launch_bounds__(256) void amax_rows_kernel(const float* __restrict__ x, long n, float* __restrict__ slot) {
    __shared__ float red[4];
    const int b = blockIdx.y;
    const float* p = x + (long)b * n;
    float mx = 0.f;
    if ((n & 3) == 0) {
        for (long i = blockIdx.x * 256L + threadIdx.x; i < (n >> 2); i += (long)gridDim.x * 256) {
            const float4 v = reinterpret_cast<const float4*>(p)[i];
            mx = fmaxf(fmaxf(mx, fmaxf(fabsf(v.x), fabsf(v.y))), fmaxf(fabsf(v.z), fabsf(v.w)));
        }
    } else {
        for (long i = blockIdx.x * 256L + threadIdx.x; i < n; i += (long)gridDim.x * 256) mx = fmaxf(mx, fabsf(p[i]));
    }
    amax_flush_wg(slot + b, mx, red);
}
static __global__ __launch_bounds__(256) void amax_rag_kernel(const float* __restrict__ x, int C, int rs, RagDev rg, float* __restrict__ slot) {
    __shared__ float red[4];
    const int b = blockIdx.y;
    const int n = rg.tb[b] * rg.mult;
    const float* p = x + (long)rg.pre[b] * rg.mult;
    float mx = 0.f;
    for (int c = blockIdx.x; c < C; c += gridDim.x) {
        const float* r = p + (long)c * rs;
        for (int i = threadIdx.x; i < n; i += 256) mx = fmaxf(mx, fabsf(r[i]));
    }
    amax_flush_wg(slot + b, mx, red);
}
inline int run_amax_rows(tvc_ctx* ctx, hipStream_t s, const float* x, int B, int C, long len, float* slot) {
    if (ctx->rag) {
        RagDev rg;
        TVC_CHECK(rag_tiles(ctx, s, B, len, 0, &rg, nullptr, "amax_rows"));
        const int gx = C < 8 ? C : (ctx->rag->B >= 64 ? 8 : 16);
        hipLaunchKernelGGL(amax_rag_kernel, dim3((unsigned)gx, (unsigned)ctx->rag->B), dim3(256), 0, s, x, C, (int)len, rg, slot);
        return launch_check(ctx, "amax_rows (ragged)");
    }
    const long n = (long)C * len;
    if ((reinterpret_cast<uintptr_t>(x) & 15) != 0) return fail(ctx, TVC_ERR_ARG, "amax_rows: the tensor must be 16-byte aligned");
    long gx = (n / 4 + 255) / 256 / 8;
    const long cap = B >= 64 ? 8 : 512 / (B > 0 ? B : 1);
    if (gx > cap) gx = cap;
    if (gx < 1) gx = 1;
    hipLaunchKernelGGL(amax_rows_kernel, dim3((unsigned)gx, (unsigned)B), dim3(256), 0, s, x, n, slot);
    return launch_check(ctx, "amax_rows");
}

}
```

tinyvc_amd/csrc/tvc_common.h:

```cpp
#pragma once
#include <hip/hip_runtime.h>

#include <atomic>
#include <cstdarg>
#include <cstdint>
#include <cstdio>
#include <cstring>
#include <map>
#include <string>
#include <vector>

#include "../../include/tinyvc_hip.h"
#include "ragged.h"

namespace tvc {

constexpr int kSampleRate = 24000;
constexpr int kNfft = 1920;
constexpr int kHop = 480;
constexpr int kBins = 961;
constexpr int kSslDim = 768;
constexpr int kSslCh = 384;
constexpr int kPitchCh = 128;
constexpr int kPitchClasses = 512;
constexpr int kSrcCh = 128;
constexpr int kHarm = 15;
constexpr int kSolaCross = 1920, kSolaSearch = 1920, kSolaDelay = 3840;
constexpr int kSolaGroups = 8, kSolaPartFloats = 16384;

struct PackedW {
    const float* bias = nullptr;
    const float* A6 = nullptr;
    const float* wscale = nullptr;
    const float* wjoint = nullptr;
    int M = 0, K = 0, Mpad = 0, Kpad = 0, cin = 0, taps = 1, MT6 = 0, S6 = 0;
};

struct ConvNeXtW {
    const float* dw_w = nullptr;
    const float* dw_b = nullptr;
    const float* ln_g = nullptr;
    const float* ln_b = nullptr;
    PackedW c2, c3;
    const float* grn_g = nullptr;
    const float* grn_b = nullptr;
    const float* c3_bias_grn = nullptr;
    float ln_bound = 0.f;
    int C = 0, dilation = 1;
};

constexpr int K24_PIECES = 10;
struct Up24sBlob {
    static constexpr int PIECES = 28;
    static constexpr int BA = 0, BB = 32, BSC = 64, BSH = 96;
    static constexpr int W75 = 128, B75 = 296;
    static constexpr int SA = 297, SB = 298, SSC = 299, SSH = 300;
    static constexpr int L1A = 301, BMA = 302;
    static constexpr int FLOATS = 304;
};
struct Down0sBlob {
    static constexpr int PIECES = K24_PIECES;
    static constexpr int BIAS = 0;
    static constexpr int BW = 29, BB = 30;
    static constexpr int SCALE = 31;
    static constexpr int FLOATS = 32;
};
struct Conv24sBlob {
    static constexpr int BIAS = 0;
    static constexpr int SCALE = 62;
    static constexpr int FLOATS = 64;
};

struct DownW {
    PackedW res, c1, c2, c3;
    const float* c3res_bias = nullptr;
    const float* s24c1 = nullptr;
    const float* s24c2 = nullptr;
    const float* s24c3r = nullptr;
    float b1_w = 0.f, b1_b = 0.f, b2_w = 0.f, b2_b = 0.f;
    int cin = 0, cout = 0, factor = 1;
};
struct FilmU {
    static constexpr int TAB_BIAS = 0, TAB_SCALE = 1, TAB_BSC = 2, TAB_BSH = 3, TAB_SSC = 4, TAB_SSH = 5;
    const float* img = nullptr;
    const float* tab = nullptr;
    int C = 0;
    float hb_w = 0.f, hb_b = 0.f;
};
struct UpW {
    PackedW c1, c2, c3, c4, c5, film1, film2;
    FilmU fu1, fu2;
    const float* s24a = nullptr;
    const float* s24b = nullptr;
    float c5_bw = 0.f, c5_bb = 0.f;
    int cin = 0, cout = 0, factor = 1;
};

struct HostTensor {
    std::vector<float> data;
    std::vector<int64_t> shape;
};

struct ArenaBuilder {
    std::vector<float> buf;
    std::vector<std::pair<const float**, size_t>> fix;
    size_t put(const float** slot, const float* v, size_t n);
    size_t put(const float** slot, const std::vector<float>& v) { return put(slot, v.data(), v.size()); }
    void resolve(const float* arena) const {
        for (auto& f : fix) *f.first = arena + f.second;
    }
};

}

struct tvc_prof_region {
    std::string name;
    hipEvent_t a = nullptr, b = nullptr;
};

struct tvc_ctx {
    int device = 0;
    int ncu = 0;
    int profiling = 0;
    std::vector<tvc_prof_region> regions;
    std::vector<hipEvent_t> event_pool;
    hipStream_t side = nullptr;
    hipEvent_t ev_fork = nullptr, ev_join = nullptr;
    hipEvent_t ev_fork2 = nullptr, ev_join2 = nullptr, ev_amps = nullptr;
    tvc::RagHost* rag = nullptr;
    int rag_batch_frames = 0;
    bool enc_ready = false, dec_ready = false;
    char enc_missing[160] = {0}, dec_missing[160] = {0};
    std::map<std::string, tvc::HostTensor> host;
    std::vector<float> pitch_table;
    float* arena = nullptr;
    float* const_arena = nullptr;
    size_t arena_floats = 0;
    char err[512] = {0};

    const float* fft_tw960 = nullptr;
    const float* fft_tw1920 = nullptr;
    const float* fft_hann = nullptr;
    const float* pitch_freq = nullptr;
    const float* sola_part = nullptr;

    tvc::PackedW enc_in;
    const float* ssl_ln_g = nullptr;
    const float* ssl_ln_b = nullptr;
    const float* pit_ln_g = nullptr;
    const float* pit_ln_b = nullptr;
    tvc::ConvNeXtW ssl_mid[6], pit_mid[4], src_mid[3];
    tvc::PackedW ssl_out, pit_out;
    tvc::PackedW src_content_in, src_to_amps, src_to_kernel;
    const float* src_e_w = nullptr;
    const float* src_e_b = nullptr;
    const float* src_f_w = nullptr;
    const float* src_f_b = nullptr;
    tvc::PackedW flt_content_in;
    const float* flt_down0s = nullptr;
    float down0_bw = 0.f, down0_bb = 0.f;
    float flt_in_bw = 0.f, flt_in_bb = 0.f;
    const float* flt_f_w = nullptr;
    const float* flt_f_b = nullptr;
    tvc::DownW downs[4];
    tvc::UpW ups[5];
};

namespace tvc {

inline int fail(tvc_ctx* ctx, int code, const char* fmt, ...) {
    if (ctx) {
        va_list ap;
        va_start(ap, fmt);
        vsnprintf(ctx->err, sizeof(ctx->err), fmt, ap);
        va_end(ap);
    }
    return code;
}

#define TVC_HIP(ctx, call)                                                                       \
    do {                                                                                         \
        hipError_t e_ = (call);                                                                  \
        if (e_ != hipSuccess)                                                                    \
            return tvc::fail(ctx, TVC_ERR_HIP, "%s failed: %s (%s:%d)", #call, hipGetErrorString(e_), \
                             __FILE__, __LINE__);                                                \
    } while (0)

#define TVC_CHECK(expr)        \
    do {                       \
        int rc_ = (expr);      \
        if (rc_ != 0) return rc_; \
    } while (0)

struct Ws {
    char* base;
    size_t cap, off = 0, peak = 0;
    bool dry;
    Ws(void* p, size_t c, bool d) : base((char*)p), cap(c), dry(d) {}
    template <class T>
    T* get(size_t n) {
        size_t bytes = (n * sizeof(T) + 255) & ~size_t(255);
        size_t o = off;
        off += bytes;
        if (off > peak) peak = off;
        if (dry) return (T*)(uintptr_t)256;
        return (T*)(base + o);
    }
    size_t mark() const { return off; }
    void release(size_t m) { off = m; }
};

struct ProfScope {
    tvc_ctx* ctx;
    hipStream_t s;
    int idx = -1;
    ProfScope(tvc_ctx* c, hipStream_t st, const Ws& ws, const char* name) : ctx(c), s(st) {
        if (!c || !c->profiling || ws.dry) return;
        if (c->profiling == 2 && std::strncmp(name, "filter_net", 10) != 0) return;
        tvc_prof_region r;
        r.name = name;
        auto take = [&](hipEvent_t* e) {
            if (!c->event_pool.empty()) {
                *e = c->event_pool.back();
                c->event_pool.pop_back();
                return true;
            }
            return hipEventCreate(e) == hipSuccess;
        };
        if (!take(&r.a) || !take(&r.b)) return;
        (void)hipEventRecord(r.a, s);
        c->regions.push_back(r);
        idx = (int)c->regions.size() - 1;
    }
    ~ProfScope() {
        if (idx >= 0) (void)hipEventRecord(ctx->regions[idx].b, s);
    }
};

struct SideFork {
    tvc_ctx* ctx;
    hipStream_t s, side;
    hipEvent_t ev_join = nullptr;
    bool ended = false;
    SideFork(tvc_ctx* c, hipStream_t st) : ctx(c), s(st), side(st) {}
    bool forked() const { return ev_join != nullptr; }
    int fork(const Ws& ws, hipEvent_t ev_fork, hipEvent_t join) {
        hipStreamCaptureStatus cap = hipStreamCaptureStatusNone;
        if (ws.dry || !ctx->side || !ev_fork || !join || hipStreamIsCapturing(s, &cap) != hipSuccess || cap != hipStreamCaptureStatusNone) return 0;
        TVC_HIP(ctx, hipEventRecord(ev_fork, s));
        TVC_HIP(ctx, hipStreamWaitEvent(ctx->side, ev_fork, 0));
        side = ctx->side;
        ev_join = join;
        return 0;
    }
    int end() {
        if (forked() && !ended) TVC_HIP(ctx, hipEventRecord(ev_join, side));
        ended = true;
        return 0;
    }
    hipError_t record_and_wait() {
        hipEvent_t e = ev_join;
        ev_join = nullptr;
        const hipError_t r = e && !ended ? hipEventRecord(e, side) : hipSuccess;
        return e && r == hipSuccess ? hipStreamWaitEvent(s, e, 0) : r;
    }
    int join() { TVC_HIP(ctx, record_and_wait()); return 0; }
    ~SideFork() { (void)record_and_wait(); }
};

inline int launch_check(tvc_ctx* ctx, const char* what) {
    hipError_t e = hipGetLastError();
    if (e != hipSuccess) return fail(ctx, TVC_ERR_HIP, "launch %s: %s", what, hipGetErrorString(e));
    return 0;
}

template <auto... K>
int lds_optin(tvc_ctx* ctx, int bytes, const char* what) {
    static std::atomic<bool> ready_dev[64];
    std::atomic<bool>& ready = ready_dev[ctx->device & 63];
    if (ready.load(std::memory_order_acquire)) return 0;
    for (const void* k : {(const void*)K...}) {
        const hipError_t e = hipFuncSetAttribute(k, hipFuncAttributeMaxDynamicSharedMemorySize, bytes);
        if (e != hipSuccess) return fail(ctx, TVC_ERR_HIP, "%s setup: %s", what, hipGetErrorString(e));
    }
    ready.store(true, std::memory_order_release);
    return 0;
}

void pack_constants(tvc_ctx*, ArenaBuilder*);
void pack_checkpoint(tvc_ctx*, ArenaBuilder*, std::string* missing_enc, std::string* missing_dec);

int run_stft(tvc_ctx*, hipStream_t, Ws&, const float* wav, float* spec, int B, int64_t L);
int run_stft_fft(tvc_ctx*, hipStream_t, const float* wav, float* spec, int B, int64_t L);
int run_noise_ifft(tvc_ctx*, hipStream_t, const float* kern, const float* angle, uint64_t seed, float* frames, int B, int T, bool angle_padded = false);
int run_energy(tvc_ctx*, hipStream_t, Ws&, const float* wav, float* energy, int B, int64_t L, float* emax = nullptr, float* spec_bound = nullptr,
               float* zero = nullptr, int nz = 0);
const float* knn_index_amax(const float* prepared);
int run_knn_amax_rows(tvc_ctx*, hipStream_t, const std::vector<const float*>& blobs, float* out);
int run_slot_affine(tvc_ctx*, hipStream_t, float* out, const float* in, int in_stride, float a, float c, int n);
int run_slot_prep(tvc_ctx*, hipStream_t, float* zero, int nz, float* o1, const float* in1, int s1, float a1, float c1, float* o2, const float* in2, int s2, float a2,
                  float c2, float* o3, float a3, float c3, int n);
constexpr int kBlobMagic = 0x54564B4E, kBlobVersion = 2;
constexpr int kFilterSlotX = 2;
constexpr int kFilterSlots = 41;
int run_encoder(tvc_ctx*, hipStream_t, Ws&, const float* spec, float* ssl, float* f0,
                float* logits, int B, int T, const float* spec_bound = nullptr, float* zeroed_slots = nullptr,
                float* f0_shifted = nullptr, float shift = 0.f,
                const float* shifts = nullptr);
int run_pitch_decode(tvc_ctx*, hipStream_t, const float* logits, float* f0, int B, int T);
int run_knn(tvc_ctx*, hipStream_t, Ws&, const float* src, const float* prepared, int64_t N,
            float* out, int64_t* idx_out, int B, int T);
struct KnnSegIn {
    const float* blob;
    int64_t N;
    int col0, ncols;
};
int run_knn_segs(tvc_ctx*, hipStream_t, Ws&, const float* src, const KnnSegIn* in, int nin, float* out, int64_t* idx_out, int B, int T);
int run_knn_topk(tvc_ctx*, hipStream_t, Ws&, const float* src, const float* prepared, int64_t N,
                 float* sims_out, int64_t* idx_out, int B, int T);
int run_knn_general(tvc_ctx*, hipStream_t, Ws&, const float* src, const float* index, int64_t N, int k, int metric, float* out, int64_t* idx_out,
                    float* val_out, int B, int T);
int run_knn_slots(tvc_ctx*, hipStream_t, const float* prepared, int64_t N, const int64_t* idx, float* slots, int64_t nslots);
int run_knn_finish(tvc_ctx*, hipStream_t, const float* slots, float* out, int B, int T);
int run_shift(tvc_ctx*, hipStream_t, const float* f0, float* out, int64_t n, float semitones);
int run_uniform_to_angle(tvc_ctx*, hipStream_t, float* u, int64_t n);
int run_decoder(tvc_ctx*, hipStream_t, Ws&, const float* content, const float* f0,
                const float* energy, const float* angle, uint64_t seed, float* wave, float* amps_out,
                float* kernel_out, float* source_out, int B, int T, const float* content_bound = nullptr, const float* energy_bound = nullptr,
                int content_bound_stride = 0);
struct FilterTaps {
    float* skips[5] = {nullptr, nullptr, nullptr, nullptr, nullptr};
    float* ups[4] = {nullptr, nullptr, nullptr, nullptr};
};
int run_filter(tvc_ctx*, hipStream_t, Ws&, const float* content, const float* f0, const float* energy,
               const float* source, float* wave, int B, int T, const FilterTaps* taps = nullptr, const float* cmax = nullptr, const float* smax = nullptr,
               float* zeroed_slots = nullptr, bool x_slot_set = false, float* x_pre = nullptr, bool x_pre_filled = false);
struct DspFork {
    hipStream_t side;
    hipEvent_t amps_ready;
};
int run_dsp(tvc_ctx*, hipStream_t, Ws&, const float* f0, const float* amps, const float* kern, const float* angle, uint64_t seed, float* source, int B, int T,
            float* smax = nullptr, double* csum = nullptr, const DspFork* fk = nullptr);
int run_sola(tvc_ctx*, hipStream_t, const float* y, float* sola_buf, const float* fade_in, float* out, int32_t* shift_out,
             int S, int64_t Ly, int block, int use_pv);
int run_stream_push(tvc_ctx* ctx, hipStream_t s, float* buf, const float* blocks, int S, int n, int m);
int64_t resample_out_len(int64_t n, int orig_freq, int new_freq);
int run_resample(tvc_ctx*, hipStream_t, const float* x, float* y, int rows, int64_t n, int orig_freq, int new_freq);
int run_pcm16_to_f32(tvc_ctx*, hipStream_t, const int16_t* pcm, float* y, int64_t n, float gain_db);
int run_f32_to_pcm16(tvc_ctx*, hipStream_t, const float* x, int16_t* pcm, int64_t n, float gain_db);
void frontdoor_release(tvc_ctx*);
int run_prepare_index(tvc_ctx*, hipStream_t, const float* index, float* prepared, int64_t N);
int run_prepare_index_f16(tvc_ctx*, hipStream_t, const void* rows_f16, float* prepared, int64_t N);

int run_up24_split(tvc_ctx*, hipStream_t, const UpW& u, const float* x, const float* cond_planes, float cbw, float cbb, float* x1, float* out, int B, int len,
                   const float* amax_x, const float* amax_c, float* amax_x1);
int run_down0_split(tvc_ctx*, hipStream_t, const float* blob, const float* source, const float* energy, float* planes, float* out_fp32, float* y2, int B, int len,
                    const float* amax_x, float* amax_y);
int run_down24_fused(tvc_ctx*, hipStream_t, const DownW& d, const float* xi, float* out, float* y2, int B, int len, const float* amax_xi, float* amax_out);
int run_conv48s(tvc_ctx*, hipStream_t, const PackedW& w, const float* x, const PackedW* film, const float* bsc, const float* bsh, const float* cond,
                const float* res, float* out, int B, int len, int dil, const float* amax_x, const float* amax_c, float* amax_y,
                const PackedW* c5 = nullptr, float* out5 = nullptr);

int run_conv48_pair(tvc_ctx*, hipStream_t, const PackedW& wa, const PackedW& wb, const float* x, int lin, float lscale, const PackedW* film, const float* bsc,
                    const float* bsh, const float* cond, float* out, int B, int len, int da, int db, const float* amax_x, const float* amax_c,
                    float* amax_y);

int run_convnext(tvc_ctx*, hipStream_t, Ws&, const ConvNeXtW& w, float* x, int B, int T, float* amax_out = nullptr);

}
```

Measured before the change: 696.9 million.

## Pre-split downsample skip outputs into fp16 pairs for FiLM consumers

The downsampling block's final residual conv now writes its skip tensor straight into the two-term fp16 split layout, scaled by an a-priori bound computed from weight row L1 norms and the input amaxes. The FiLM conv in the matching upsampling stage then loads those pre-split operands directly instead of re-reading fp32 and splitting per tile. It also skips the fp32 skip write and the tap copy when a tap buffer already receives it. This cuts memory traffic and split ALU work in the FiLM loads, but relies on a conservative bound instead of the measured amax, which may cost some precision, and it adds more kernel template variants.

```diff
diff --git a/tinyvc_amd/csrc/conv3s.h b/tinyvc_amd/csrc/conv3s.h
--- a/tinyvc_amd/csrc/conv3s.h
+++ b/tinyvc_amd/csrc/conv3s.h
@@ -395,7 +395,7 @@
 template <class TL, bool RES>
 __device__ __forceinline__ void tile_store(float* Ot, const f32x16 (&v)[TL::WM][TL::WN], float* __restrict__ y, const float* __restrict__ res,
                                            int b, int M, int len, int mt0, int t0, float& mx, float* __restrict__ y2 = nullptr, int f2 = 0, int rlin = 0, float rscale = 0.f,
-                                           int rs_ = 0, int coloff = 0) {
+                                           int rs_ = 0, int coloff = 0, uint4* __restrict__ ypre = nullptr, float ps = 1.f) {
     const int rs = rs_ ? rs_ : len;
     const int rvalid = (rs_ && rlin > 0) ? __builtin_amdgcn_readfirstlane(len / (rs / rlin)) : rlin;
     const int rcol = (rs_ && rlin > 0) ? __builtin_amdgcn_readfirstlane(coloff / (rs / rlin)) : 0;
@@ -527,6 +527,22 @@
         }
     }
     park();
+    if (!RES && ypre) {
+        const int M8 = M >> 3;
+        uint4* pb = ypre + ((long)b * 2 * M8 + mt0 * 4) * rs + coloff + t0;
+        for (int idx = tid; idx < (BM / 8) * BN; idx += NTHR) {
+            const int g = idx / BN, c = idx - g * BN;
+            if (8 * g >= rows || t0 + c >= len) continue;
+            float v[8];
+#pragma unroll
+            for (int j = 0; j < 8; ++j) v[j] = Ot[(8 * g + j) * OS + c] * ps;
+            uint4 p1, p2;
+            split8u(v, p1, p2);
+            pb[(long)g * rs + c] = p1;
+            pb[(long)(M8 + g) * rs + c] = p2;
+        }
+    }
+    const bool wy = y != nullptr;
 #pragma unroll 2
     for (int idx = tid; idx < BM * (BN / 4); idx += NTHR) {
         const int row = idx / (BN / 4), c = (idx - row * (BN / 4)) * 4;
@@ -559,7 +575,7 @@
                 const float4 q = *reinterpret_cast<const float4*>(rb + off);
                 w.x += q.x; w.y += q.y; w.z += q.z; w.w += q.w;
             }
-            *reinterpret_cast<float4*>(yb + off) = w;
+            if (wy) *reinterpret_cast<float4*>(yb + off) = w;
             mx = fmaxf(fmaxf(mx, fmaxf(fabsf(w.x), fabsf(w.y))), fmaxf(fabsf(w.z), fabsf(w.w)));
             if (y2b) {
                 const float e[4] = {w.x, w.y, w.z, w.w};
@@ -579,7 +595,7 @@
             for (int u = 0; u < 4; ++u)
                 if (t0 + c + u < len) {
                     const float ov = RES ? e[u] + rb[off + u] : e[u];
-                    yb[off + u] = ov;
+                    if (wy) yb[off + u] = ov;
                     mx = fmaxf(mx, fabsf(ov));
                     if (y2b && f2 != 4) {
                         const int t = t0 + c + u, q = t / f2;
@@ -839,7 +855,13 @@
 #pragma unroll
                         for (int j = 0; j < WN; ++j) hi[i][j][r] += bm;
                     }
-                tile_store<TL, Epi::kRes>(reinterpret_cast<float*>(smem_s), hi, ep.y, ep.res, RAGT ? 0 : b, ep.M, len, mt0, t0, mx_run, ep.y2, ep.f2, 0, 0.f, rs, coloff);
+                if constexpr (wants_res_conv<Epi>::value) {
+                    const float ps = ep.ypre ? norm_from_amax(skip_bound(ep.kb, b)).s : 1.f;
+                    tile_store<TL, Epi::kRes>(reinterpret_cast<float*>(smem_s), hi, ep.y, ep.res, RAGT ? 0 : b, ep.M, len, mt0, t0, mx_run, ep.y2, ep.f2, 0, 0.f, rs, coloff,
+                                              ep.ypre, ps);
+                } else {
+                    tile_store<TL, Epi::kRes>(reinterpret_cast<float*>(smem_s), hi, ep.y, ep.res, RAGT ? 0 : b, ep.M, len, mt0, t0, mx_run, ep.y2, ep.f2, 0, 0.f, rs, coloff);
+                }
             }
         }
         tile = nxt;
diff --git a/tinyvc_amd/csrc/conv_epi.h b/tinyvc_amd/csrc/conv_epi.h
--- a/tinyvc_amd/csrc/conv_epi.h
+++ b/tinyvc_amd/csrc/conv_epi.h
@@ -1,5 +1,6 @@
 #pragma once
 #include "gemm_epi.h"
+#include "split_fp16.h"
 
 namespace tvc {
 
@@ -30,6 +31,8 @@
 
 struct C3EpiBiasResConv : C3EpiBias<false, 0> {
     static constexpr bool kResConv = true;
+    uint4* ypre = nullptr;
+    SkipBound kb;
 };
 
 struct C3EpiFilmFused {
diff --git a/tinyvc_amd/csrc/conv_s2.h b/tinyvc_amd/csrc/conv_s2.h
--- a/tinyvc_amd/csrc/conv_s2.h
+++ b/tinyvc_amd/csrc/conv_s2.h
@@ -20,18 +20,6 @@
     float pre_w, pre_b;
     RagDev rag;
 };
-__device__ __forceinline__ float presplit_bound(float pre_w, float pre_b, const float* amax, int b) { return fmaf(pre_w, sload_f32(amax + b), pre_b); }
-__device__ __forceinline__ Bfp norm_from_amax(float amax) {
-    const unsigned u = __builtin_bit_cast(unsigned, amax);
-    Bfp r{1.f, 1.f};
-    if (u != 0u && u < 0x7f800000u) {
-        int k = 14 - ((int)(u >> 23) - 127);
-        k = k > 120 ? 120 : (k < -120 ? -120 : k);
-        r.s = __builtin_bit_cast(float, (unsigned)(127 + k) << 23);
-        r.inv = __builtin_bit_cast(float, (unsigned)(127 - k) << 23);
-    }
-    return r;
-}
 
 struct CS2 {
     static constexpr int MTB = 3, NWV = 4, WN = 2, NW = MTB * NWV, NTHR = NW * 64, BN = NWV * WN * 32, MAXD = 27, XROW = BN + 2 * MAXD;
@@ -269,13 +257,18 @@
 }
 
 template <bool LERP, bool PRE = false>
+inline bool conv_s2_fits(const PackedW& w, int B, int Cin, int len, int dil, int lin) {
+    if (PRE && w.M % 8 != 0) return false;
+    if (w.taps != 3 || w.MT6 % 3 != 0 || w.M > 384 || Cin % 16 != 0 || Cin / 16 > w.S6 || dil < 1 || dil > CS2::MAXD) return false;
+    if ((long)B * w.M * len >= (1L << 31) / 4 * 4 && (long)w.M * len * 4 >= (1L << 32)) return false;
+    if ((long)Cin * (LERP ? lin : len) * 4 >= (1L << 32) || (long)w.M * len * 4 >= (1L << 32)) return false;
+    return LERP == (lin > 0);
+}
+
+template <bool LERP, bool PRE = false>
 inline bool conv_s2_try(int* rc, tvc_ctx* ctx, hipStream_t s, const PackedW& w, const float* x, int B, int Cin, int len, int dil, float* y, const BfpSlots& bfp,
                         int lin = 0, float lscale = 0.f, float pre_w = 0.f, float pre_b = 0.f) {
-    if (PRE && (!bfp.x || w.M % 8 != 0)) return false;
-    if (w.taps != 3 || w.MT6 % 3 != 0 || w.M > 384 || Cin % 16 != 0 || Cin / 16 > w.S6 || dil < 1 || dil > CS2::MAXD || bfp.c) return false;
-    if ((long)B * w.M * len >= (1L << 31) / 4 * 4 && (long)w.M * len * 4 >= (1L << 32)) return false;
-    if ((long)Cin * (LERP ? lin : len) * 4 >= (1L << 32) || (long)w.M * len * 4 >= (1L << 32)) return false;
-    if (LERP != (lin > 0)) return false;
+    if ((PRE && !bfp.x) || bfp.c || !conv_s2_fits<LERP, PRE>(w, B, Cin, len, dil, lin)) return false;
     if ((*rc = lds_optin<conv_s2_kernel<LERP, PRE>, conv_s2_kernel<LERP, PRE, true>>(ctx, CS2::lds_bytes, "conv_s2"))) return true;
     ConvS2Args a;
     a.A6 = reinterpret_cast<const uint4*>(w.A6);
diff --git a/tinyvc_amd/csrc/decoder.hip b/tinyvc_amd/csrc/decoder.hip
--- a/tinyvc_amd/csrc/decoder.hip
+++ b/tinyvc_amd/csrc/decoder.hip
@@ -247,11 +247,15 @@
                                                      cond, C);
 }
 
+static bool half_presplit(tvc_ctx* ctx, const PackedW& ca, const FilmU& fu, int B, int C, int len, int lin, int da, int db) {
+    return rag_min_len(ctx, len) >= FS2::BN && fu.img && fu.C == C && fu.hb_w > 0.f && C % 96 == 0 && C <= 384 && db >= 1 && db <= FS2::MAXD &&
+           (long)C * len * 4 < (1L << 32) && (lin <= 0 || (long)C * lin * 4 < (1L << 32)) &&
+           (lin > 0 ? conv_s2_fits<true, true>(ca, B, C, len, da, lin) : conv_s2_fits<false, true>(ca, B, C, len, da, 0));
+}
 static int conv_film_half(tvc_ctx* ctx, hipStream_t s, const PackedW& ca, const PackedW& cb, const PackedW& fw, const FilmU& fu, const float* x, int lin, float lscale,
                           int da, int db, float* h, const float* cond, int B, int C, int len, float* out, const float* bsc, const float* bsh, const float* res,
-                          int res_lin, float res_scale, const float* ma_in, float* mh, const float* mcond, float* mout) {
-    const bool pre = rag_min_len(ctx, len) >= FS2::BN && fu.img && fu.C == C && fu.hb_w > 0.f && C % 96 == 0 && C <= 384 && ma_in && mcond && res && db >= 1 && db <= FS2::MAXD &&
-                     (long)C * len * 4 < (1L << 32) && (res_lin <= 0 || (long)C * res_lin * 4 < (1L << 32));
+                          int res_lin, float res_scale, const float* ma_in, float* mh, const float* mcond, float* mout, const SkipBound* ckb) {
+    const bool pre = ma_in && mcond && res && res_lin == lin && half_presplit(ctx, ca, fu, B, C, len, lin, da, db);
     if (pre) {
         int rc = 0;
         const BfpSlots in{ma_in, nullptr, nullptr};
@@ -259,11 +263,12 @@
                                 : conv_s2_try<false, true>(&rc, ctx, s, ca, x, B, C, len, da, h, in, 0, 0.f, fu.hb_w, fu.hb_b);
         if (ok) {
             TVC_CHECK(rc);
-            if (!film_s2_try(&rc, ctx, s, fu, h, cond, B, C, len, db, out, res, res_lin, res_scale, BfpSlots{ma_in, mcond, mout}, true, fu.hb_w, fu.hb_b))
+            if (!film_s2_try(&rc, ctx, s, fu, h, cond, B, C, len, db, out, res, res_lin, res_scale, BfpSlots{ma_in, mcond, mout}, true, fu.hb_w, fu.hb_b, ckb))
                 return fail(ctx, TVC_ERR_STATE, "filter_net: the FiLM conv refused the pre-split operand its producer wrote");
             return rc;
         }
     }
+    if (ckb) return fail(ctx, TVC_ERR_STATE, "filter_net: a pre-split skip reached a half outside film_s2's pre-split path");
     TVC_CHECK(plain_conv(ctx, s, ca, x, B, C, len, da, h, BfpSlots{ma_in, nullptr, mh}, lin, lscale));
     return film_conv(ctx, s, cb, fw, fu, h, cond, B, C, len, db, out, bsc, bsh, res, res_lin, res_scale, BfpSlots{mh, mcond, mout});
 }
@@ -320,6 +325,21 @@
         if (!x_pre_filled) TVC_CHECK(filter_input_gemm(ctx, s, content, f0, x, B, T, cmax));
         if (!(zeroed_slots && x_slot_set)) TVC_CHECK(run_slot_affine(ctx, s, slot(S_X), cmax, 1, ctx->flt_in_bw, ctx->flt_in_bb, NB));
         TVC_CHECK(run_down0_split(ctx, s, ctx->flt_down0s, source, energy, skip[0], taps ? taps->skips[0] : nullptr, xi_pre[1], B, (int)L, smax, slot(S_SKIP0)));
+    }
+    bool cpre[5] = {false, false, false, false, false};
+    SkipBound kb[5];
+    {
+        long l = T;
+        for (int u = 0; u < 5; ++u) {
+            const UpW& up = ctx->ups[u];
+            const int lin = (int)l, i = 4 - u;
+            l *= up.factor;
+            if (i < 2 || l != len_dn[i]) continue;
+            const DownW& d = ctx->downs[i - 1];
+            kb[i] = SkipBound{slot(S_DH2 + i - 1), slot(S_SKIP0 + i - 1), d.sk_wh, d.sk_wx, d.sk_b};
+            cpre[i] = d.sk_wh > 0.f && d.cout == up.cin && half_presplit(ctx, up.c1, up.fu1, B, up.cin, (int)l, lin, 1, 3) &&
+                      half_presplit(ctx, up.c3, up.fu2, B, up.cin, (int)l, 0, 9, 27);
+        }
     }
     for (int i = 1; i <= 4; ++i) {
         const DownW& d = ctx->downs[i - 1];
@@ -344,9 +364,13 @@
                     TVC_CHECK(plain_conv(ctx, s, d.c1, xi, B, d.cin, len, 1, h1, BfpSlots{mxi, nullptr, mh1}));
                     TVC_CHECK(plain_conv(ctx, s, d.c2, h1, B, d.cin, len, 2, h2, BfpSlots{mh1, nullptr, mh2}));
                 }
-                TVC_CHECK((conv3s_launch<true, C3EpiBiasResConv>(ctx, s, d.c3, h2, B, d.cin, len, 4,
-                                                                 C3EpiBiasResConv{{skip[i], d.c3res_bias, nullptr, d.cout, len, y2, f2}},
-                                                                 BfpSlots{mh2, mxi, mout}, &d.res, nullptr, xi, d.cin)));
+                C3EpiBiasResConv ep{{skip[i], d.c3res_bias, nullptr, d.cout, len, y2, f2}};
+                if (cpre[i]) {
+                    ep.y = taps ? taps->skips[i] : nullptr;
+                    ep.ypre = reinterpret_cast<uint4*>(skip[i]);
+                    ep.kb = kb[i];
+                }
+                TVC_CHECK((conv3s_launch<true, C3EpiBiasResConv>(ctx, s, d.c3, h2, B, d.cin, len, 4, ep, BfpSlots{mh2, mxi, mout}, &d.res, nullptr, xi, d.cin)));
             }
         }
         ws.release(mk);
@@ -368,6 +392,7 @@
         const int lo = (int)len, C = u.cin, nc = B * lo;
         const float* cond = skip[4 - i];
         const float* mcond = slot(S_SKIP0 + 4 - i);
+        const SkipBound* ckb = cpre[4 - i] ? &kb[4 - i] : nullptr;
         size_t mk = ws.mark();
         float* xu = ws.get<float>((size_t)B * C * lo);
         float* h = ws.get<float>((size_t)B * C * lo);
@@ -398,9 +423,9 @@
                         TVC_CHECK(run_conv48s(ctx, s, cb, h, &fw, bsc, bsh, cond, x1, nullptr, B, lo, db, mh, mcond, slot(S_LEV + i), &u.c5, xlev[i]));
                     }
                 } else if (half == 0) {
-                    TVC_CHECK(conv_film_half(ctx, s, ca, cb, fw, u.fu1, x, lin, lscale, da, db, h, cond, B, C, lo, xout, bsc, bsh, x, lin, lscale, ma_in, mh, mcond, mout));
+                    TVC_CHECK(conv_film_half(ctx, s, ca, cb, fw, u.fu1, x, lin, lscale, da, db, h, cond, B, C, lo, xout, bsc, bsh, x, lin, lscale, ma_in, mh, mcond, mout, ckb));
                 } else {
-                    TVC_CHECK(conv_film_half(ctx, s, ca, cb, fw, u.fu2, x1, 0, 0.f, da, db, h, cond, B, C, lo, xout, bsc, bsh, x1, 0, 0.f, ma_in, mh, mcond, mout));
+                    TVC_CHECK(conv_film_half(ctx, s, ca, cb, fw, u.fu2, x1, 0, 0.f, da, db, h, cond, B, C, lo, xout, bsc, bsh, x1, 0, 0.f, ma_in, mh, mcond, mout, ckb));
                 }
             }
             if (C != 48) {
@@ -420,7 +445,7 @@
         for (int i = 1; i < 5; ++i)
             if (taps->skips[i] && i == 1)
                 hipLaunchKernelGGL(g8_to_planar_kernel, dim3(grid_for((long)B * 48 * len_dn[1])), dim3(256), 0, s, skip[1], taps->skips[1], (long)B, len_dn[1], 48);
-            else if (taps->skips[i])
+            else if (taps->skips[i] && !cpre[i])
                 TVC_HIP(ctx, hipMemcpyAsync(taps->skips[i], skip[i], (size_t)B * ch[4 - i] * len_dn[i] * sizeof(float), hipMemcpyDeviceToDevice, s));
         long l = T;
         for (int i = 0; i < 4; ++i) {
diff --git a/tinyvc_amd/csrc/film_s2.h b/tinyvc_amd/csrc/film_s2.h
--- a/tinyvc_amd/csrc/film_s2.h
+++ b/tinyvc_amd/csrc/film_s2.h
@@ -21,6 +21,7 @@
     float* amax_y;
     const uint4* xpre;
     float pre_w, pre_b;
+    SkipBound kb;
     RagDev rag;
 };
 
@@ -35,16 +36,9 @@
 };
 using FS2 = FS2T<8>;
 
-__device__ __forceinline__ void split8u(const float (&v)[8], uint4& p1, uint4& p2) {
-    unsigned o1[4], o2[4];
-#pragma unroll
-    for (int j = 0; j < 4; ++j) split2<false>(v[2 * j], v[2 * j + 1], o1[j], o2[j]);
-    p1 = make_uint4(o1[0], o1[1], o1[2], o1[3]);
-    p2 = make_uint4(o2[0], o2[1], o2[2], o2[3]);
-}
-
-template <bool XPRE, bool RAG = false, int NWV_ = 8>
+template <bool XPRE, bool RAG = false, int NWV_ = 8, bool CPRE = false>
 __global__ __launch_bounds__(FS2T<NWV_>::NTHR) __attribute__((amdgpu_waves_per_eu(2))) void film_s2_kernel(FilmS2Args a) {
+    static_assert(!CPRE || XPRE, "a pre-split cond comes with a pre-split h (decoder.hip half_presplit)");
     using TL = FS2T<NWV_>;
     constexpr int MTB = TL::MTB, WM = TL::WM, NWV = TL::NWV, WN = TL::WN, NW = TL::NW, BN = TL::BN, XROW = TL::XROW, A_PER = TL::A_PER, XS = TL::XS;
     extern __shared__ __attribute__((aligned(16))) uint4 smem_fs[];
@@ -77,8 +71,8 @@
     };
 
     u32x4 ar[A_PER];
-    float xr[XPRE ? 1 : XS][8], cr[8];
-    uint4 xq[XPRE ? XS : 1][2];
+    float xr[XPRE ? 1 : XS][8], cr[CPRE ? 1 : 8];
+    uint4 xq[XPRE ? XS : 1][2], cq[CPRE ? 2 : 1];
     auto item_of = [&](int t_, int k, int& g, int& c) __attribute__((always_inline)) {
         int item = t_ + k * TL::NTHR;
         item = item < nitems ? item : item - nitems;
@@ -113,9 +107,9 @@
         }
         int pc = lt0 + cc;
         pc = pc > llen - 1 ? llen - 1 : pc;
-        co = (unsigned)(8 * cg * rs + ub + pc);
+        co = (unsigned)((CPRE ? 1 : 8) * cg * rs + ub + pc);
         xs = XPRE ? 1.f : norm_from_amax(sload_f32(a.amax_x + lb)).s;
-        cs_ = norm_from_amax(sload_f32(a.amax_c + lb)).s;
+        cs_ = CPRE ? 1.f : norm_from_amax(sload_f32(a.amax_c + lb)).s;
     };
     tile_offsets();
     auto issue_load = [&]() __attribute__((always_inline)) {
@@ -143,8 +137,14 @@
 #pragma unroll
                 for (int j = 0; j < 8; ++j) xr[k][j] = ldg_so(xc + (long)j * rs, 4u * xo[k]);
         }
-#pragma unroll
-        for (int j = 0; j < 8; ++j) cr[j] = ldg_so(cc_ + (long)j * rs, 4u * co);
+        if (CPRE) {
+            const uint4* cp = reinterpret_cast<const uint4*>(a.cond) + ((RAG ? 0L : (long)lb * 2 * (C >> 3)) + 2 * ls) * rs;
+            cq[0] = __builtin_bit_cast(uint4, ldg_so4(cp, 16u * co));
+            cq[1] = __builtin_bit_cast(uint4, ldg_so4(cp + (long)(C >> 3) * rs, 16u * co));
+        } else {
+#pragma unroll
+            for (int j = 0; j < 8; ++j) cr[j] = ldg_so(cc_ + (long)j * rs, 4u * co);
+        }
         rxs = xs;
         rcs = cs_;
     };
@@ -185,9 +185,14 @@
             Xb[xdst[k]] = p1;
             Xb[2 * XROW + xdst[k]] = p2;
         }
-#pragma unroll
-        for (int j = 0; j < 8; ++j) v[j] = cr[j] * rcs;
-        split8u(v, p1, p2);
+        if (CPRE) {
+            p1 = cq[0];
+            p2 = cq[1];
+        } else {
+#pragma unroll
+            for (int j = 0; j < 8; ++j) v[j] = cr[j] * rcs;
+            split8u(v, p1, p2);
+        }
         Cb[cdst] = p1;
         Cb[2 * BN + cdst] = p2;
     };
@@ -278,7 +283,8 @@
             int el = lane;
             asm volatile("" : "+v"(el));
             const int e31 = el & 31, eh = el >> 5;
-            const float ix = norm_from_amax(XPRE ? presplit_bound(a.pre_w, a.pre_b, a.amax_x, cb) : sload_f32(a.amax_x + cb)).inv, ic_ = norm_from_amax(sload_f32(a.amax_c + cb)).inv;
+            const float ix = norm_from_amax(XPRE ? presplit_bound(a.pre_w, a.pre_b, a.amax_x, cb) : sload_f32(a.amax_x + cb)).inv,
+                        ic_ = norm_from_amax(CPRE ? skip_bound(a.kb, cb) : sload_f32(a.amax_c + cb)).inv;
 #pragma unroll
             for (int i = 0; i < WM; ++i) {
             const int row0 = (cmb * MTB + wm * WM + i) * 32;
@@ -377,11 +383,17 @@
 }
 
 inline bool film_s2_try(int* rc, tvc_ctx* ctx, hipStream_t s, const FilmU& fu, const float* h, const float* cond, int B, int C, int len, int dil, float* out,
-                        const float* res, int res_lin, float res_scale, const BfpSlots& bfp, bool pre = false, float pre_w = 0.f, float pre_b = 0.f) {
+                        const float* res, int res_lin, float res_scale, const BfpSlots& bfp, bool pre = false, float pre_w = 0.f, float pre_b = 0.f,
+                        const SkipBound* ckb = nullptr) {
     if (!fu.img || fu.C != C || C % 96 != 0 || C > 384 || dil < 1 || dil > FS2::MAXD || !bfp.x || !bfp.c || !res) return false;
     if ((long)C * len * 4 >= (1L << 32) || (res_lin > 0 && (long)C * res_lin * 4 >= (1L << 32))) return false;
-    if ((*rc = lds_optin<film_s2_kernel<false>, film_s2_kernel<true>, film_s2_kernel<false, true>, film_s2_kernel<true, true>>(ctx, FS2::lds_bytes, "film_s2")) ||
-        (*rc = lds_optin<film_s2_kernel<false, false, 7>, film_s2_kernel<true, false, 7>>(ctx, FS2T<7>::lds_bytes, "film_s2")))
+    if (ckb && !pre) {
+        *rc = fail(ctx, TVC_ERR_STATE, "film_s2: a pre-split cond needs a pre-split h");
+        return true;
+    }
+    if ((*rc = lds_optin<film_s2_kernel<false>, film_s2_kernel<true>, film_s2_kernel<false, true>, film_s2_kernel<true, true>, film_s2_kernel<true, false, 8, true>,
+                         film_s2_kernel<true, true, 8, true>>(ctx, FS2::lds_bytes, "film_s2")) ||
+        (*rc = lds_optin<film_s2_kernel<false, false, 7>, film_s2_kernel<true, false, 7>, film_s2_kernel<true, false, 7, true>>(ctx, FS2T<7>::lds_bytes, "film_s2")))
         return true;
     FilmS2Args a{};
     a.img = reinterpret_cast<const uint4*>(fu.img);
@@ -403,20 +415,24 @@
     a.pre_b = pre_b;
     a.amax_c = bfp.c;
     a.amax_y = bfp.y;
+    if (ckb) a.kb = *ckb;
     int ncol = a.tiles_per_utt * B;
     if ((*rc = rag_tiles(ctx, s, B, len, FS2::BN, &a.rag, &ncol, "film_s2"))) return true;
     a.ntiles = ncol * a.mblocks;
     const int grid = a.ntiles < ctx->ncu ? a.ntiles : ctx->ncu;
     if (ctx->rag) {
-        if (pre) hipLaunchKernelGGL((film_s2_kernel<true, true>), dim3(grid), dim3(FS2::NTHR), FS2::lds_bytes, s, a);
+        if (ckb) hipLaunchKernelGGL((film_s2_kernel<true, true, 8, true>), dim3(grid), dim3(FS2::NTHR), FS2::lds_bytes, s, a);
+        else if (pre) hipLaunchKernelGGL((film_s2_kernel<true, true>), dim3(grid), dim3(FS2::NTHR), FS2::lds_bytes, s, a);
         else hipLaunchKernelGGL((film_s2_kernel<false, true>), dim3(grid), dim3(FS2::NTHR), FS2::lds_bytes, s, a);
     } else if ((len + 223) / 224 * 224 < (len + 255) / 256 * 256) {
         a.tiles_per_utt = (len + 223) / 224;
         a.ntiles = a.tiles_per_utt * B * a.mblocks;
         const int g7 = a.ntiles < ctx->ncu ? a.ntiles : ctx->ncu;
-        if (pre) hipLaunchKernelGGL((film_s2_kernel<true, false, 7>), dim3(g7), dim3(FS2T<7>::NTHR), FS2T<7>::lds_bytes, s, a);
+        if (ckb) hipLaunchKernelGGL((film_s2_kernel<true, false, 7, true>), dim3(g7), dim3(FS2T<7>::NTHR), FS2T<7>::lds_bytes, s, a);
+        else if (pre) hipLaunchKernelGGL((film_s2_kernel<true, false, 7>), dim3(g7), dim3(FS2T<7>::NTHR), FS2T<7>::lds_bytes, s, a);
         else hipLaunchKernelGGL((film_s2_kernel<false, false, 7>), dim3(g7), dim3(FS2T<7>::NTHR), FS2T<7>::lds_bytes, s, a);
-    } else if (pre) hipLaunchKernelGGL(film_s2_kernel<true>, dim3(grid), dim3(FS2::NTHR), FS2::lds_bytes, s, a);
+    } else if (ckb) hipLaunchKernelGGL((film_s2_kernel<true, false, 8, true>), dim3(grid), dim3(FS2::NTHR), FS2::lds_bytes, s, a);
+    else if (pre) hipLaunchKernelGGL(film_s2_kernel<true>, dim3(grid), dim3(FS2::NTHR), FS2::lds_bytes, s, a);
     else hipLaunchKernelGGL(film_s2_kernel<false>, dim3(grid), dim3(FS2::NTHR), FS2::lds_bytes, s, a);
     *rc = launch_check(ctx, "film_s2");
     return true;
diff --git a/tinyvc_amd/csrc/pack.hip b/tinyvc_amd/csrc/pack.hip
--- a/tinyvc_amd/csrc/pack.hip
+++ b/tinyvc_amd/csrc/pack.hip
@@ -465,6 +465,14 @@
             std::vector<float> sum(d.c3.Mpad, 0.f);
             for (int m = 0; m < d.cout; ++m) sum[m] = b3[m] + br[m];
             ab->put(&d.c3res_bias, sum);
+            const float* w3 = pk.get(p + ".c3.weight", (size_t)d.cout * d.cin * 3);
+            const float* wr = pk.get(p + ".down_res.weight", (size_t)d.cout * d.cin);
+            if (w3 && wr) {
+                const RowL1 r3 = row_l1(w3, b3, d.cout, d.cin * 3), rr = row_l1(wr, br, d.cout, d.cin);
+                d.sk_wh = (float)(r3.w * 1.0001);
+                d.sk_wx = (float)(rr.w * 1.0001);
+                d.sk_b = (float)((r3.b + rr.b) * 1.0001);
+            }
         }
     }
     for (int i = 0; i < 5; ++i) {
diff --git a/tinyvc_amd/csrc/split_fp16.h b/tinyvc_amd/csrc/split_fp16.h
--- a/tinyvc_amd/csrc/split_fp16.h
+++ b/tinyvc_amd/csrc/split_fp16.h
@@ -36,6 +36,24 @@
 }
 __device__ __forceinline__ Bfp bfp_load_u(const float* amax, int b) { return amax ? bfp_from_amax(sload_f32(amax + b)) : Bfp{1.f, 1.f}; }
 __device__ __forceinline__ Bfp bfp_min(const Bfp& a, const Bfp& b) { return a.s < b.s ? a : b; }
+__device__ __forceinline__ Bfp norm_from_amax(float amax) {
+    const unsigned u = __builtin_bit_cast(unsigned, amax);
+    Bfp r{1.f, 1.f};
+    if (u != 0u && u < 0x7f800000u) {
+        int k = 14 - ((int)(u >> 23) - 127);
+        k = k > 120 ? 120 : (k < -120 ? -120 : k);
+        r.s = __builtin_bit_cast(float, (unsigned)(127 + k) << 23);
+        r.inv = __builtin_bit_cast(float, (unsigned)(127 - k) << 23);
+    }
+    return r;
+}
+__device__ __forceinline__ float presplit_bound(float pre_w, float pre_b, const float* amax, int b) { return fmaf(pre_w, sload_f32(amax + b), pre_b); }
+struct SkipBound {
+    const float* h = nullptr;
+    const float* x = nullptr;
+    float wh = 0.f, wx = 0.f, bb = 0.f;
+};
+__device__ __forceinline__ float skip_bound(const SkipBound& k, int b) { return fmaf(k.wh, sload_f32(k.h + b), fmaf(k.wx, sload_f32(k.x + b), k.bb)); }
 __device__ __forceinline__ float wave_max(float mx) {
 #pragma unroll
     for (int o = 32; o > 0; o >>= 1) mx = fmaxf(mx, __shfl_xor(mx, o));
@@ -102,6 +120,13 @@
     p1 = make_uint4(o1[0], o1[1], o1[2], o1[3]);
     p2 = make_uint4(o2[0], o2[1], o2[2], o2[3]);
 }
+__device__ __forceinline__ void split8u(const float (&v)[8], uint4& p1, uint4& p2) {
+    unsigned o1[4], o2[4];
+#pragma unroll
+    for (int j = 0; j < 4; ++j) split2<false>(v[2 * j], v[2 * j + 1], o1[j], o2[j]);
+    p1 = make_uint4(o1[0], o1[1], o1[2], o1[3]);
+    p2 = make_uint4(o2[0], o2[1], o2[2], o2[3]);
+}
 #define TVC_MFMA16(a, b, c) __builtin_amdgcn_mfma_f32_32x32x16_f16(a, b, c, 0, 0, 0)
 __device__ __forceinline__ float comb(float hi, float lo, float c, float clo) { return fmaf(lo, clo, hi * c); }
 
diff --git a/tinyvc_amd/csrc/tvc_common.h b/tinyvc_amd/csrc/tvc_common.h
--- a/tinyvc_amd/csrc/tvc_common.h
+++ b/tinyvc_amd/csrc/tvc_common.h
@@ -78,6 +78,7 @@
     const float* s24c2 = nullptr;
     const float* s24c3r = nullptr;
     float b1_w = 0.f, b1_b = 0.f, b2_w = 0.f, b2_b = 0.f;
+    float sk_wh = 0.f, sk_wx = 0.f, sk_b = 0.f;
     int cin = 0, cout = 0, factor = 1;
 };
 struct FilmU {
```

After: 693.5 million, median of 2. About the same (-0.5%).
